# ashispati/ar-vae

Hardware: AMD Instinct MI355X
Metric: training images/sec (dSprites beta-VAE+AR, per-GPU batch 512) (higher is better)
Workload: dtype f32 (conv MFMAs: scaled 2-term fp16 split, 3 products, fp32-accurate)

## Files before the change

ar-vae_amd/csrc/conv32.hip:

```cpp
#include <mutex>
#include "diag.h"
#include "common.h"
#include "conv32_common.h"
#include "reduce.h"
#include "midprep.h"
#include "prep32.h"
#include "regloss.h"
#include "down32p.h"
#include "wgrad32r.h"

#include <type_traits>

namespace arvae {

template <int LO, int STRIDE, int PX = 128>
struct PatchLoader {
    using T = Tile<LO, PX>;
    static constexpr int SZ = STRIDE * LO;
    static constexpr int PR = STRIDE * T::TR + 2, PC = STRIDE * T::TC + 2;
    static constexpr int SLOTS = T::TI * PR * PC * 8;
    static constexpr int ITERS = (SLOTS + 255) / 256;
    float4 r[ITERS];
    unsigned rel[ITERS];
    __amdgpu_buffer_rsrc_t rs_v;
// ... 808 lines not shown
    reg_loss_block(reg, b % reg_bx, b / reg_bx, reg_lds, reg_lds + REG_CHUNK);
}


constexpr int WG32_SLAB = SLAB_C32_FLOATS;


template <int LO, int BIAS>
__device__ __forceinline__ void wgrad32x_body(const float *__restrict__ lo, const float *__restrict__ hi, float *__restrict__ slab, int n_img,
                                              int n_tiles, const unsigned *amax_lo, const unsigned *amax_hi, const int BID, const int NBLK) {
    constexpr int PX = 64, KB = PX / 16;
    using PL = PatchLoader<LO, 2, PX>;
    constexpr int WG_PSB_L = WGRAD_PSB_L, WG_PSB_H = WGRAD_PSB_H;
    constexpr int PC = PL::PC, PR = PL::PR, PLANE = PL::PLANE_DW / PSB * WG_PSB_H, LPLANE = PX * WG_PSB_L;
    extern __shared__ __attribute__((aligned(16))) float lds[];
    unsigned *ldsw = reinterpret_cast<unsigned *>(lds);
    unsigned *lo_w = ldsw + 2 * PLANE;
    const int lane = threadIdx.x & 63, wave = __builtin_amdgcn_readfirstlane(threadIdx.x >> 6);
    const int half = lane >> 5, rc = lane & 31;

    int loff[KB][2], hoff[KB][2];
    {
        const int g16 = lane >> 4, q = (lane & 15) >> 2, pp = lane & 3;
#pragma unroll
        for (int b = 0; b < KB; ++b)
#pragma unroll
            for (int i = 0; i < 2; ++i) {
                const int P = 16 * b + 8 * (g16 >> 1) + 4 * i + q;
                int img, r, c;
                tile_pixel<LO, PX>(P, img, r, c);
                loff[b][i] = P * WG_PSB_L + 8 * (g16 & 1) + 2 * pp;
                hoff[b][i] = ((img * PR + 2 * r + wave) * PC + 2 * c) * WG_PSB_H + 8 * (g16 & 1) + 2 * pp;
            }
    }

    f32x16 acc[4];
#pragma unroll
    for (int kx = 0; kx < 4; ++kx)
#pragma unroll
        for (int i = 0; i < 16; ++i) acc[kx][i] = 0.f;
    float4 bias4 = make_float4(0.f, 0.f, 0.f, 0.f);

    const AmaxLoad al_l = amax_issue(amax_lo), al_h = amax_issue(amax_hi);
    PL pl;
    pl.init(hi, n_img);
    const int64_t lo_bytes = (int64_t)n_img * LO * LO * PIXB;
    const __amdgpu_buffer_rsrc_t rs_lo = make_rsrc(lo, lo_bytes);
    float4 lr[2];
    unsigned lo_base = 0;
    auto set_lo = [&](int i0, int rr0, bool ok) {
        lo_base = ok ? (unsigned)(((i0 * LO + rr0) * LO) * PIXB) + threadIdx.x * 16 : OOB;
    };
    int img0, r0;
    tile_origin<LO, PX>(BID, img0, r0);
    pl.set_tile(img0, r0, BID < n_tiles);
    set_lo(img0, r0, BID < n_tiles);
    pl.issue_all();
#pragma unroll
    for (int it = 0; it < 2; ++it) lr[it] = buf_load4(rs_lo, lo_base + it * 4096);
    const Pow2 sc_lo = amax_scale(al_l), sc_hi = amax_scale(al_h);

    for (int tile = BID; tile < n_tiles; tile += NBLK) {
        __syncthreads();
        pl.template commit_split2<BIAS == 2, WG_PSB_H>(ldsw, sc_hi.s, &bias4);
#pragma unroll
        for (int it = 0; it < 2; ++it) {
            const int idx = threadIdx.x + it * 256, pix = idx >> 3, q = idx & 7;
            uint2 hv, lv;
            split_pair_h2(lr[it].x, lr[it].y, sc_lo.s, hv.x, lv.x);
            split_pair_h2(lr[it].z, lr[it].w, sc_lo.s, hv.y, lv.y);
            *reinterpret_cast<uint2 *>(lo_w + pix * WG_PSB_L + q * 2) = hv;
            *reinterpret_cast<uint2 *>(lo_w + LPLANE + pix * WG_PSB_L + q * 2) = lv;
            if (BIAS == 1) { bias4.x += lr[it].x; bias4.y += lr[it].y; bias4.z += lr[it].z; bias4.w += lr[it].w; }
        }
        __syncthreads();
        {
            int ni, nr;
            tile_origin<LO, PX>(tile + NBLK, ni, nr);
            pl.set_tile(ni, nr, tile + NBLK < n_tiles);
            set_lo(ni, nr, tile + NBLK < n_tiles);
        }
        static_for<0, KB>([&](auto bc) __attribute__((always_inline)) {
            constexpr int b = decltype(bc)::value;
            f16x8 b2[2];
#pragma unroll
            for (int t = 0; t < 2; ++t) b2[t] = lds_tr_f16x8(lo_w + t * LPLANE + loff[b][0], lo_w + t * LPLANE + loff[b][1]);
            pl.template issue_step<KB, b>();
            if constexpr (b < 2) lr[b] = buf_load4(rs_lo, lo_base + b * 4096);
#pragma unroll
            for (int kx = 0; kx < 4; ++kx) {
                f16x8 a2[2];
#pragma unroll
                for (int t = 0; t < 2; ++t)
                    a2[t] = lds_tr_f16x8(ldsw + t * PLANE + hoff[b][0] + kx * WG_PSB_H, ldsw + t * PLANE + hoff[b][1] + kx * WG_PSB_H);
                MFMA_H(acc[kx], a2[1], b2[0]);
                MFMA_H(acc[kx], a2[0], b2[1]);
                MFMA_H(acc[kx], a2[0], b2[0]);
            }
        });
    }

    float *out = slab + (int64_t)BID * WG32_SLAB;
    const float inv = sc_lo.inv * sc_hi.inv;
#pragma unroll
    for (int kx = 0; kx < 4; ++kx)
#pragma unroll
        for (int g = 0; g < 4; ++g)
            *reinterpret_cast<float4 *>(out + ((wave * 4 + kx) * C32 + rc) * C32 + 8 * g + 4 * half) =
                make_float4(acc[kx][4 * g] * inv, acc[kx][4 * g + 1] * inv, acc[kx][4 * g + 2] * inv, acc[kx][4 * g + 3] * inv);
    if (BIAS != 0) {
        __syncthreads();
        *reinterpret_cast<float4 *>(lds + threadIdx.x * 4) = bias4;
        __syncthreads();
        if (threadIdx.x < C32) {
            const int q = threadIdx.x >> 2, e = threadIdx.x & 3;
            float tot = 0.f;
            for (int j = 0; j < 32; ++j) tot += lds[(j * 8 + q) * 4 + e];
            out[16 * C32 * C32 + threadIdx.x] = tot;
        }
    }
}
template <int LO, int BIAS>
__global__ __launch_bounds__(256, 1) void wgrad32x_kernel(const float *__restrict__ lo, const float *__restrict__ hi,
                                                          float *__restrict__ slab, int n_img, int n_tiles, const unsigned *amax_lo,
                                                          const unsigned *amax_hi) {
    wgrad32x_body<LO, BIAS>(lo, hi, slab, n_img, n_tiles, amax_lo, amax_hi, blockIdx.x, gridDim.x);
}

template <int MODE, int BIAS>
__global__ __launch_bounds__(256, 1) void pair4_down_kernel(const float *__restrict__ g_hi, Ep32 ep,
                                                           const float *__restrict__ w_lo, const float *__restrict__ w_hi,
                                                           float *__restrict__ slab, int n_img, int tiles_a, int tiles_b, int grid_a,
                                                           const unsigned *amax_lo, const unsigned *amax_hi) {
    if ((int)blockIdx.x < grid_a) down32s_body<4, MODE>(g_hi, ep, n_img, tiles_a, blockIdx.x, grid_a);
    else wgrad32x_body<4, BIAS>(w_lo, w_hi, slab, n_img, tiles_b, amax_lo, amax_hi, blockIdx.x - grid_a, gridDim.x - grid_a);
}
template <int MODE, int BIAS>
__global__ __launch_bounds__(256, 1) void pair4_up_kernel(const float *__restrict__ g_lo, Ep32 ep,
                                                         const float *__restrict__ w_lo, const float *__restrict__ w_hi,
                                                         float *__restrict__ slab, int n_img, int tiles_a, int tiles_b, int grid_a,
                                                         const unsigned *amax_lo, const unsigned *amax_hi) {
    if ((int)blockIdx.x < grid_a) up32x_body<4, MODE, 32>(g_lo, ep, n_img, tiles_a, blockIdx.x, grid_a);
    else wgrad32x_body<4, BIAS>(w_lo, w_hi, slab, n_img, tiles_b, amax_lo, amax_hi, blockIdx.x - grid_a, gridDim.x - grid_a);
}


template <int LO, int MODE, int BIAS>
__global__ __launch_bounds__(512) __attribute__((amdgpu_waves_per_eu(2, 2))) void pair_down_wgrad_kernel(
    const float *__restrict__ g_hi, Ep32 ep, int n_img, int tiles_a, int grid_a, const float *__restrict__ w_lo, const float *__restrict__ w_hi,
    float *__restrict__ slab, int total_steps, int steps_per_wg, const unsigned *amax_lo, const unsigned *amax_hi) {
    if ((int)blockIdx.x < grid_a) down32p_body<LO, MODE>(g_hi, ep, n_img, tiles_a, blockIdx.x, grid_a);
    else wgrad32r_body<LO, BIAS>(w_lo, w_hi, slab, n_img, total_steps, steps_per_wg, amax_lo, amax_hi, blockIdx.x - grid_a);
}
template <int MODE, int BIAS, bool C1W = false>
__global__ __launch_bounds__(512) __attribute__((amdgpu_waves_per_eu(2, 2))) void pair_up16_wgrad_kernel(
    const float *__restrict__ g_lo, Ep32 ep, int n_img, int tiles_a, int grid_a, const float *__restrict__ w_lo, const float *__restrict__ w_hi,
    float *__restrict__ slab, int total_steps, int steps_per_wg, const unsigned *amax_lo, const unsigned *amax_hi, C1Wgrad c1) {
    if ((int)blockIdx.x < grid_a) up32p_body<MODE, C1W>(g_lo, ep, n_img, tiles_a, blockIdx.x, grid_a, c1);
    else wgrad32r_body<16, BIAS>(w_lo, w_hi, slab, n_img, total_steps, steps_per_wg, amax_lo, amax_hi, blockIdx.x - grid_a);
}
template <int MODE, int BIAS>
__global__ __launch_bounds__(512) __attribute__((amdgpu_waves_per_eu(2, 2))) void pair_up8_wgrad_kernel(
    const float *__restrict__ g_lo, Ep32 ep, int n_img, int tiles_a, int grid_a, const float *__restrict__ w_lo, const float *__restrict__ w_hi,
    float *__restrict__ slab, int total_steps, int steps_per_wg, const unsigned *amax_lo, const unsigned *amax_hi) {
    if ((int)blockIdx.x < grid_a) {
        if (threadIdx.x >= 256) return;
        up32x_body<8, MODE, 32>(g_lo, ep, n_img, tiles_a, blockIdx.x, grid_a);
    } else wgrad32r_body<8, BIAS>(w_lo, w_hi, slab, n_img, total_steps, steps_per_wg, amax_lo, amax_hi, blockIdx.x - grid_a);
}

static int cu_count() { return device_cu_count(); }

template <int LO, int PX = 128> static constexpr int tiles_for(int n) {
    using T = Tile<LO, PX>;
    return T::TI == 1 ? n * (LO / T::TR) : (n + T::TI - 1) / T::TI;
}
static int grid_for_tiles(int tiles) {
    const int cap = cu_count() < AMAX_N / 4 ? cu_count() : AMAX_N / 4;
    return tiles < cap ? tiles : cap;
}

bool conv32_fits(const arvae_link_t *l) {
    return l->chi == 32 && l->clo == 32 && l->kh == 4 && l->kw == 4 && l->stride == 2 && l->pad == 1 &&
           l->hh == l->hw && l->lh == l->lw && (l->lh == 16 || l->lh == 8 || l->lh == 4) && l->hi_perm_c == 0 &&
           l->lo_perm_c == 0 && (int64_t)l->n * l->hh * l->hw * PIXB < (1ll << 31) - (1ll << 20);
}

template <class K> static void allow_lds(K kernel, int bytes) {
    (void)hipFuncSetAttribute((const void *)kernel, hipFuncAttributeMaxDynamicSharedMemorySize, bytes);
}

template <int A, int B> struct MaxOf { static constexpr int value = A > B ? A : B; };

constexpr int LDS_DOWN_S = (PatchLoader<4, 2, 32>::BUF2_DW + 4 * 16 * 64) * 4;
static int down_small_grid(int tiles) {
    int g = tiles < 2 * cu_count() ? tiles : 2 * cu_count();
    return g < AMAX_N ? g : AMAX_N;
}

template <int MODE> static void launch_down_small(const Operand &hi, const Ep32 &ep, int n, hipStream_t s) {
    const int tiles = tiles_for<4, 32>(n);
    static std::once_flag attr;
    std::call_once(attr, [&] { allow_lds(down32s_kernel<4, MODE>, LDS_DOWN_S); });
    ARVAE_LAUNCH((down32s_kernel<4, MODE>), dim3(down_small_grid(tiles)), dim3(256), LDS_DOWN_S, s, hi.v, ep, n, tiles);
}
template <int LO, int MODE, int PX>
static void launch_up_px(const Operand &lo, const Ep32 &ep, int n, hipStream_t s) {
    const int tiles = tiles_for<LO, PX>(n), grid = grid_for_tiles(tiles);
    if constexpr (LO == 16 && PX == 128 && MODE != EP_GATE_F) {
        constexpr int LDSP = (2 * 2 * PatchLoader<16, 1, 128>::PLANE_DW) * 4 + 4 * 4 * 4 * 64 * 16;
        static std::once_flag attrp;
        std::call_once(attrp, [&] { allow_lds(up32p_kernel<MODE>, LDSP); });
        ARVAE_LAUNCH((up32p_kernel<MODE>), dim3(grid), dim3(512), LDSP, s, lo.v, ep, n, tiles);
    } else {
        constexpr int LDSX = 2 * PatchLoader<LO, 1, PX>::PLANE_DW * 4;
        static std::once_flag attrx;
        std::call_once(attrx, [&] { allow_lds(up32x_kernel<LO, MODE, PX>, LDSX); });
        ARVAE_LAUNCH((up32x_kernel<LO, MODE, PX>), dim3(grid), dim3(256), LDSX, s, lo.v, ep, n, tiles);
    }
}
template <int LO, int MODE>
static void launch_up_v(const Operand &lo, const Ep32 &ep, int n, hipStream_t s) {
    if (LO == 4 && 2 * tiles_for<LO, 128>(n) <= cu_count()) launch_up_px<4, MODE, 32>(lo, ep, n, s);
    else if (LO == 8 && tiles_for<LO, 128>(n) <= cu_count()) launch_up_px<8, MODE, 32>(lo, ep, n, s);
    else launch_up_px<LO, MODE, 128>(lo, ep, n, s);
}

static int ep_mode(const Ep32 &ep, int relu) {
    return ep.gate_bits != nullptr ? EP_GATE_B : ep.gate != nullptr ? EP_GATE_F : relu ? EP_RELU : EP_PLAIN;
}

template <int LO, int MODE> static void launch_down_p(const float *hi, const Ep32 &ep, int n, hipStream_t s) {
    constexpr int LDS = DownK<LO>::LDS_DW * 4;
    static std::once_flag attr;
    std::call_once(attr, [&] { allow_lds(down32p_kernel<LO, MODE>, LDS); });
    const int tiles = n * DownK<LO>::TILES_PER_IMG;
    ARVAE_LAUNCH((down32p_kernel<LO, MODE>), dim3(grid_for_tiles(tiles)), dim3(512), LDS, s, hi, ep, n, tiles);
}
template <int LO> static void launch_down_p_mode(const float *hi, const Ep32 &ep, int mode, int n, hipStream_t s) {
    switch (mode) {
        case EP_GATE_B: launch_down_p<LO, EP_GATE_B>(hi, ep, n, s); break;
        case EP_GATE_F: launch_down_p<LO, EP_GATE_F>(hi, ep, n, s); break;
        case EP_RELU: launch_down_p<LO, EP_RELU>(hi, ep, n, s); break;
        default: launch_down_p<LO, EP_PLAIN>(hi, ep, n, s); break;
    }
}
static void conv32_down_ksplit(const arvae_link_t *l, const float *hi, const Ep32 &ep, int mode, hipStream_t s) {
    if (l->lh == 16) launch_down_p_mode<16>(hi, ep, mode, l->n, s);
    else launch_down_p_mode<8>(hi, ep, mode, l->n, s);
}

int conv32_down(const arvae_link_t *l, const Operand &hi, const float *bias, int relu, const float *gate, const uint16_t *gate_bits,
                uint16_t *bits_out, float *out, hipStream_t s, const float *wprep, const unsigned *amax_in, unsigned *amax_out) {
    ARVAE_REQUIRE(wprep != nullptr && amax_in != nullptr, "conv32_down: prepared weights and the input's maxima are needed");
    Ep32 ep{bias, gate, gate_bits, bits_out, out, reinterpret_cast<const uint4 *>(wprep), amax_in, amax_out};
    const int mode = ep_mode(ep, relu);
    if (l->lh != 4) {
        conv32_down_ksplit(l, hi.v, ep, mode, s);
        return check_launch(l->lh == 16 ? "down32_kernel<16>" : "down32_kernel<8>");
    }
    switch (mode) {
        case EP_GATE_B: launch_down_small<EP_GATE_B>(hi, ep, l->n, s); break;
        case EP_GATE_F: launch_down_small<EP_GATE_F>(hi, ep, l->n, s); break;
        case EP_RELU: launch_down_small<EP_RELU>(hi, ep, l->n, s); break;
        default: launch_down_small<EP_PLAIN>(hi, ep, l->n, s); break;
    }
    return check_launch("down32_kernel<4>");
}

template <int MODE>
__global__ __launch_bounds__(512) __attribute__((amdgpu_waves_per_eu(2, 2))) void chain_down_kernel(const float *__restrict__ hi, Ep32 ep_a, Ep32 ep_b,
                                                                                                    int n_img, int tiles_a, int tiles_b) {
    extern __shared__ __attribute__((aligned(16))) unsigned chain_lds[];
    constexpr int BODY_DW = MaxOf<DownK<16>::LDS_DW, DownK<8>::LDS_DW>::value;
    float *chain_max = reinterpret_cast<float *>(chain_lds + BODY_DW);
    down32p_body<16, MODE, 1>(hi, ep_a, n_img, tiles_a, blockIdx.x, gridDim.x, chain_max);
    __syncthreads();
    down32p_body<8, MODE, 2>(ep_a.out, ep_b, n_img, tiles_b, blockIdx.x, gridDim.x, chain_max);
}
static int chain_grid(const arvae_link_t *a, const arvae_link_t *b) {
    if (a->n != b->n || a->n < 1) return 0;
    const int tiles_a = a->n * DownK<16>::TILES_PER_IMG, tiles_b = b->n * DownK<8>::TILES_PER_IMG;
    const int grid = grid_for_tiles(tiles_a);
    const int run_a = (tiles_a + grid - 1) / grid, run_b = (tiles_b + grid - 1) / grid;
    return (run_a * DownK<8>::TILES_PER_IMG == run_b * DownK<16>::TILES_PER_IMG) ? grid : 0;
}
bool conv32_down_chain_fits(const arvae_link_t *a, const arvae_link_t *b) {
    static const bool off = diag_env("ARVAE_NO_DOWN_CHAIN") != nullptr;
    return !off && conv32_fits(a) && conv32_fits(b) && a->lh == 16 && b->lh == 8 && b->hh == a->lh && chain_grid(a, b) > 0;
}
int conv32_down_chain(const arvae_link_t *a, const arvae_link_t *b, const float *hi, const unsigned *amax_in, const float *bias_a,
                      uint16_t *bits_a, float *out_a, const float *wprep_a, unsigned *amax_a, const float *bias_b, uint16_t *bits_b,
                      float *out_b, const float *wprep_b, unsigned *amax_b, hipStream_t s) {
    ARVAE_REQUIRE(conv32_down_chain_fits(a, b), "conv32_down_chain: these two layers do not chain");
    ARVAE_REQUIRE(hi && amax_in && out_a && out_b && wprep_a && wprep_b, "conv32_down_chain: null pointer");
    Ep32 ep_a{bias_a, nullptr, nullptr, bits_a, out_a, reinterpret_cast<const uint4 *>(wprep_a), amax_in, amax_a};
    Ep32 ep_b{bias_b, nullptr, nullptr, bits_b, out_b, reinterpret_cast<const uint4 *>(wprep_b), nullptr, amax_b};
    constexpr int LDS = (MaxOf<DownK<16>::LDS_DW, DownK<8>::LDS_DW>::value + 4) * 4;
    static std::once_flag attr;
    std::call_once(attr, [&] { allow_lds(chain_down_kernel<EP_RELU>, LDS); });
    ARVAE_LAUNCH((chain_down_kernel<EP_RELU>), dim3(chain_grid(a, b)), dim3(512), LDS, s, hi, ep_a, ep_b, a->n, a->n * DownK<16>::TILES_PER_IMG,
                 b->n * DownK<8>::TILES_PER_IMG);
    return check_launch("chain(down32<16> + down32<8>)");
}

template <int LO> static int launch_up(const arvae_link_t *l, const Operand &lo, const Ep32 &ep, int relu, hipStream_t s) {
// ... 110 lines not shown
static int conv32_wgrad_stream(const arvae_link_t *l, const Operand &lo, const Operand &hi, float *slab, int bias_mode, const unsigned *amax_lo,
                               const unsigned *amax_hi, hipStream_t s) {
    return l->lh == 16 ? launch_stream<16>(l, lo.v, hi.v, slab, bias_mode, amax_lo, amax_hi, s)
                       : launch_stream<8>(l, lo.v, hi.v, slab, bias_mode, amax_lo, amax_hi, s);
}

int conv32_wgrad_groups(const arvae_link_t *l) {
    if (conv32_wgrad_stream_fits(l)) return conv32_wgrad_stream_groups(l);
    return grid_for_tiles(tiles_for<4, 64>(l->n));
}

int64_t conv32_wgrad_ws_floats(const arvae_link_t *l) {
    return (int64_t)conv32_wgrad_groups(l) * WG32_SLAB;
}

constexpr int LDS_WGRAD_X4 = 2 * (PatchLoader<4, 2, 64>::PLANE_DW / PSB * WGRAD_PSB_H + 64 * WGRAD_PSB_L) * 4;
static int launch_wgrad_x4(const arvae_link_t *l, const Operand &lo, const Operand &hi, float *slab, int bias_mode, int grid,
                           const unsigned *amax_lo, const unsigned *amax_hi, hipStream_t s) {
    const int tiles = tiles_for<4, 64>(l->n);
    static std::once_flag attr;
    std::call_once(attr, [&] {
        allow_lds(wgrad32x_kernel<4, 0>, LDS_WGRAD_X4);
        allow_lds(wgrad32x_kernel<4, 1>, LDS_WGRAD_X4);
        allow_lds(wgrad32x_kernel<4, 2>, LDS_WGRAD_X4);
    });
    if (bias_mode == 1)
        ARVAE_LAUNCH((wgrad32x_kernel<4, 1>), dim3(grid), dim3(256), LDS_WGRAD_X4, s, lo.v, hi.v, slab, l->n, tiles, amax_lo, amax_hi);
    else if (bias_mode == 2)
        ARVAE_LAUNCH((wgrad32x_kernel<4, 2>), dim3(grid), dim3(256), LDS_WGRAD_X4, s, lo.v, hi.v, slab, l->n, tiles, amax_lo, amax_hi);
    else
        ARVAE_LAUNCH((wgrad32x_kernel<4, 0>), dim3(grid), dim3(256), LDS_WGRAD_X4, s, lo.v, hi.v, slab, l->n, tiles, amax_lo, amax_hi);
    return check_launch("wgrad32_kernel<4>");
}

int conv32_wgrad_partial(const arvae_link_t *l, const Operand &lo, const Operand &hi, float *dwt, float *dbias, int bias_mode,
                         float *slab, hipStream_t s, SlabJob *job, const unsigned *amax_lo, const unsigned *amax_hi) {
    ARVAE_REQUIRE(amax_lo != nullptr && amax_hi != nullptr, "conv32_wgrad: the operands' maxima are needed");
    const int grid = conv32_wgrad_groups(l);
    const int rc = conv32_wgrad_stream_fits(l) ? conv32_wgrad_stream(l, lo, hi, slab, bias_mode, amax_lo, amax_hi, s)
                                               : launch_wgrad_x4(l, lo, hi, slab, bias_mode, grid, amax_lo, amax_hi, s);
    *job = SlabJob{slab, dwt, bias_mode ? dbias : nullptr, grid, SLAB_C32, bias_mode};
    return rc;
}

constexpr int PAIR_SPLIT_C1_PERCENT = 62;
constexpr int PAIR_SPLIT_PERCENT = 50;
bool conv32_pair_fits(const arvae_link_t *l, bool up, const float *gate, const uint16_t *gate_bits, int bias_mode) {
    static const bool off4 = diag_env("ARVAE_NO_PAIR4") != nullptr;
    static const bool off = diag_env("ARVAE_NO_PAIR32") != nullptr;
    if ((gate == nullptr && gate_bits == nullptr) || bias_mode != (up ? 2 : 1)) return false;
    if (l->lh == 4) {
        const int wg_tiles = tiles_for<4, 64>(l->n), dg_tiles = tiles_for<4, 32>(l->n);
        return !off4 && wg_tiles >= 8 && wg_tiles + (dg_tiles + 1) / 2 <= cu_count() && conv32_wgrad_groups(l) == wg_tiles;
    }
    if (off || gate_bits == nullptr || !conv32_wgrad_stream_fits(l)) return false;
    if (l->n * (l->lh * l->lh / 32) < 4 * cu_count()) return false;
    if (!up && l->lh == 8 && tiles_for<8, 128>(l->n) > cu_count()) return false;
    return true;
}

template <int LO> static int launch_pair_big(const arvae_link_t *l, bool up, const float *g, const float *x_in, const Ep32 &ep, float *slab,
                                             const unsigned *amax_g, const unsigned *amax_x, hipStream_t s, int *grid_b_out,
                                             const C1Wgrad *c1 = nullptr, int *grid_a_out = nullptr) {
    const int cus = cu_count() < AMAX_N / 4 ? cu_count() : AMAX_N / 4;
    int grid_a = cus * (c1 != nullptr ? PAIR_SPLIT_C1_PERCENT : PAIR_SPLIT_PERCENT) / 100;
    if (grid_a < 1) grid_a = 1;
    const int tiles_a = up ? l->n * DownK<LO>::TILES_PER_IMG : (LO == 16 ? tiles_for<16, 128>(l->n) : tiles_for<8, 32>(l->n));
    {
        const int run = (tiles_a + grid_a - 1) / grid_a;
        grid_a = (tiles_a + run - 1) / run;
    }
    if (grid_a_out != nullptr) *grid_a_out = grid_a;
    ARVAE_REQUIRE(c1 == nullptr || grid_a <= 256, "pair_up16_wgrad: %d workgroups of the Up half exceed the first layer's 256 weight-gradient slabs", grid_a);
    int total, spw, grid_b;
    stream_geometry(l, cus - grid_a, total, spw, grid_b);
    *grid_b_out = grid_b;
    constexpr int LDS_W = RowStream<LO>::LDS_DW * 4;
    const dim3 grid(grid_a + grid_b);
    if (up) {
        constexpr int LDS = MaxOf<LDS_W, DownK<LO>::LDS_DW * 4>::value;
        static std::once_flag attr;
        std::call_once(attr, [&] { allow_lds(pair_down_wgrad_kernel<LO, EP_GATE_B, 2>, LDS); });
        ARVAE_LAUNCH((pair_down_wgrad_kernel<LO, EP_GATE_B, 2>), grid, dim3(512), LDS, s, g, ep, l->n, tiles_a, grid_a, x_in, g, slab, total, spw,
                     amax_x, amax_g);
        return check_launch(LO == 16 ? "pair(down32<16> + wgrad32<16>)" : "pair(down32<8> + wgrad32<8>)");
    }
    if constexpr (LO == 16) {
        constexpr int LDS_U = (2 * 2 * PatchLoader<16, 1, 128>::PLANE_DW) * 4 + 4 * 4 * 4 * 64 * 16;
        constexpr int LDS = MaxOf<LDS_W, LDS_U>::value;
        static std::once_flag attr;
        if (c1 != nullptr) {
            constexpr int LDS_C = MaxOf<LDS_W, LDS_U + 4 * C1W_WAVE_DW * 4>::value;
            static std::once_flag attr_c;
            std::call_once(attr_c, [&] { allow_lds(pair_up16_wgrad_kernel<EP_GATE_B, 1, true>, LDS_C); });
            ARVAE_LAUNCH((pair_up16_wgrad_kernel<EP_GATE_B, 1, true>), grid, dim3(512), LDS_C, s, g, ep, l->n, tiles_a, grid_a, g, x_in,
                         slab, total, spw, amax_g, amax_x, *c1);
            return check_launch("pair(up32<16> + wgrad32<16> + wgrad_c1)");
        }
        std::call_once(attr, [&] { allow_lds(pair_up16_wgrad_kernel<EP_GATE_B, 1>, LDS); });
        ARVAE_LAUNCH((pair_up16_wgrad_kernel<EP_GATE_B, 1>), grid, dim3(512), LDS, s, g, ep, l->n, tiles_a, grid_a, g, x_in, slab,
                     total, spw, amax_g, amax_x, C1Wgrad{nullptr, nullptr});
        return check_launch("pair(up32<16> + wgrad32<16>)");
    } else {
        constexpr int LDS = MaxOf<LDS_W, 2 * PatchLoader<8, 1, 32>::PLANE_DW * 4>::value;
        static std::once_flag attr;
        std::call_once(attr, [&] { allow_lds(pair_up8_wgrad_kernel<EP_GATE_B, 1>, LDS); });
        ARVAE_LAUNCH((pair_up8_wgrad_kernel<EP_GATE_B, 1>), grid, dim3(512), LDS, s, g, ep, l->n, tiles_a, grid_a, g, x_in, slab, total,
                     spw, amax_g, amax_x);
        return check_launch("pair(up32<8> + wgrad32<8>)");
    }
}

bool conv32_pair_c1_fits(const arvae_link_t *l, bool up, const uint16_t *gate_bits) {
    return !up && l->lh == 16 && gate_bits != nullptr;
}
int conv32_pair(const arvae_link_t *l, bool up, const float *g, const float *x_in, const float *gate, const uint16_t *gate_bits,
                float *d_in, const float *wprep, float *dwt, float *dbias, float *slab, hipStream_t s, SlabJob *job,
                const unsigned *amax_g, const unsigned *amax_x, unsigned *amax_out, const float *c1_img, float *c1_slab, SlabJob *c1_job) {
    ARVAE_REQUIRE(wprep != nullptr && amax_g != nullptr && amax_x != nullptr, "conv32_pair: prepared weights and the operands' maxima are needed");
    Ep32 ep{nullptr, gate_bits ? nullptr : gate, gate_bits, nullptr, d_in, reinterpret_cast<const uint4 *>(wprep), amax_g, amax_out};
    if (l->lh != 4) {
        int grid_b = 0, grid_a = 0;
        C1Wgrad c1{c1_img, c1_slab};
        const bool fuse = c1_img != nullptr && c1_slab != nullptr && c1_job != nullptr && conv32_pair_c1_fits(l, up, gate_bits);
        ARVAE_REQUIRE(fuse || c1_img == nullptr, "conv32_pair: this layer cannot carry the first layer's weight gradient");
        const int rc = l->lh == 16 ? launch_pair_big<16>(l, up, g, x_in, ep, slab, amax_g, amax_x, s, &grid_b, fuse ? &c1 : nullptr, &grid_a)
                                   : launch_pair_big<8>(l, up, g, x_in, ep, slab, amax_g, amax_x, s, &grid_b);
        *job = SlabJob{slab, dwt, dbias, grid_b, SLAB_C32, up ? 2 : 1};
        if (fuse) *c1_job = SlabJob{c1_slab, nullptr, nullptr, grid_a, SLAB_C1, 1};
        return rc;
    }
    constexpr int LDS_U = 2 * PatchLoader<4, 1, 32>::PLANE_DW * 4;
    constexpr int LDS = MaxOf<LDS_WGRAD_X4, MaxOf<LDS_DOWN_S, LDS_U>::value>::value;
    const int wg_tiles = tiles_for<4, 64>(l->n), dg_tiles = tiles_for<4, 32>(l->n), grid_a = (dg_tiles + 1) / 2;
    static std::once_flag attr;
    std::call_once(attr, [&] {
        allow_lds(pair4_down_kernel<EP_GATE_F, 2>, LDS);
        allow_lds(pair4_down_kernel<EP_GATE_B, 2>, LDS);
        allow_lds(pair4_up_kernel<EP_GATE_F, 1>, LDS);
        allow_lds(pair4_up_kernel<EP_GATE_B, 1>, LDS);
    });
    const dim3 grid(grid_a + wg_tiles);
    if (up) {
        if (gate_bits) ARVAE_LAUNCH((pair4_down_kernel<EP_GATE_B, 2>), grid, dim3(256), LDS, s, g, ep, x_in, g, slab, l->n, dg_tiles, wg_tiles, grid_a, amax_x, amax_g);
        else ARVAE_LAUNCH((pair4_down_kernel<EP_GATE_F, 2>), grid, dim3(256), LDS, s, g, ep, x_in, g, slab, l->n, dg_tiles, wg_tiles, grid_a, amax_x, amax_g);
    } else {
        if (gate_bits) ARVAE_LAUNCH((pair4_up_kernel<EP_GATE_B, 1>), grid, dim3(256), LDS, s, g, ep, g, x_in, slab, l->n, dg_tiles, wg_tiles, grid_a, amax_g, amax_x);
        else ARVAE_LAUNCH((pair4_up_kernel<EP_GATE_F, 1>), grid, dim3(256), LDS, s, g, ep, g, x_in, slab, l->n, dg_tiles, wg_tiles, grid_a, amax_g, amax_x);
    }
    *job = SlabJob{slab, dwt, dbias, wg_tiles, SLAB_C32, up ? 2 : 1};
    return check_launch(up ? "pair4(down32 + wgrad32)" : "pair4(up32 + wgrad32)");
}

int conv32_wgrad(const arvae_link_t *l, const Operand &lo, const Operand &hi, float *dwt, float *dbias, int bias_mode,
                 float *slab, hipStream_t s, const unsigned *amax_lo, const unsigned *amax_hi) {
    SlabJob job;
    if (int rc = conv32_wgrad_partial(l, lo, hi, dwt, dbias, bias_mode, slab, s, &job, amax_lo, amax_hi)) return rc;
    return slab_reduce(job, s);
}

}

#ifdef ARVAE_STAMPS
extern "C" int arvae_debug_stamps(unsigned long long *out, int count) {
    return (int)hipMemcpyFromSymbol(out, HIP_SYMBOL(arvae::g_stamps), sizeof(unsigned long long) * count);
}
#endif
#ifdef D32K_STAMPS
extern "C" int arvae_debug_d32k_stamps(unsigned long long *out, int count) {
    return (int)hipMemcpyFromSymbol(out, HIP_SYMBOL(arvae::g_d32k_stamps), sizeof(unsigned long long) * count);
}
#endif
#ifdef WGR_STAMPS
extern "C" int arvae_debug_wgr_stamps(unsigned long long *out, int count) {
    return (int)hipMemcpyFromSymbol(out, HIP_SYMBOL(arvae::g_wgr_stamps), sizeof(unsigned long long) * count);
}
#endif
```

ar-vae_amd/csrc/conv_c1.hip:

```cpp
#include <mutex>
#include "diag.h"
#include "common.h"
#include "reduce.h"
#include "prep32.h"
#include "wgrad_c1s.h"
#include "vae_finish.h"

namespace arvae {

constexpr int PS1 = 36;

struct Ep1 {
    const float *bias;
    const float *gate;
    const uint16_t *gate_bits;
    uint16_t *bits_out;
    float *out;
    int relu;
    unsigned *amax_out = nullptr;
};

template <int GATE, int WAVES>
__device__ __forceinline__ void down_c1s_body(Operand img, const float *__restrict__ wt, Ep1 ep, int n_rows, const int BID,
                                              const int NBLK, float *stage) {
// ... 55 lines not shown
                bits |= (o[j] > 0.f ? 1u : 0u) << (4 * g + j);
            }
            const float4 ov = make_float4(o[0], o[1], o[2], o[3]);
            amax_run = fmaxf(amax_run, amax4(ov));
            *reinterpret_cast<float4 *>(tile + rc * PS1 + 8 * g + 4 * half) = ov;
        }
        if (ep.bits_out != nullptr) ep.bits_out[pix * 2 + half] = (uint16_t)bits;
        __builtin_amdgcn_fence(__ATOMIC_RELEASE, "wavefront");
        __builtin_amdgcn_wave_barrier();
        float4 *dst = reinterpret_cast<float4 *>(ep.out + (int64_t)row * LO1 * CC);
#pragma unroll
        for (int i = 0; i < 4; ++i)
            dst[64 * i + lane] = *reinterpret_cast<const float4 *>(tile + (8 * i + (lane >> 3)) * PS1 + 4 * (lane & 7));
        __builtin_amdgcn_fence(__ATOMIC_RELEASE, "wavefront");
        __builtin_amdgcn_wave_barrier();
        v[0] = vn[0]; v[1] = vn[1];
    }
    if (ep.amax_out != nullptr) {
        __shared__ float wmax[WAVES];
        amax_run = wave_max(amax_run);
        if (lane == 0) wmax[threadIdx.x >> 6] = amax_run;
        __syncthreads();
        if (threadIdx.x < 64) {
            float m = 0.f;
#pragma unroll
            for (int w = 0; w < WAVES; ++w) m = fmaxf(m, wmax[w]);
            amax_publish(ep.amax_out, BID, NBLK, m);
        }
    }
}
template <int GATE>
__global__ __launch_bounds__(256) void down_c1s_kernel(Operand img, const float *__restrict__ wt, Ep1 ep, int n_rows) {
    __shared__ __attribute__((aligned(16))) float stage[4 * LO1 * PS1];
    down_c1s_body<GATE, 4>(img, wt, ep, n_rows, blockIdx.x, gridDim.x, stage);
}

__global__ __launch_bounds__(256) void down_c1s_prep_kernel(Operand img, const float *__restrict__ wt, Ep1 ep, int n_rows, PrepArgs prep,
                                                             MidPrepArgs mid, int conv_blocks, int prep_blocks) {
    __shared__ __attribute__((aligned(16))) float stage[4 * LO1 * PS1];
    if ((int)blockIdx.x < prep_blocks) {
        prep_all_block(prep, mid, conv_blocks, blockIdx.x);
        return;
    }
    down_c1s_body<0, 4>(img, wt, ep, n_rows, blockIdx.x - prep_blocks, gridDim.x - prep_blocks, stage);
}


typedef int i32x4 __attribute__((ext_vector_type(4)));
constexpr int TRU = 16;
constexpr int UG_PER_WAVE = (TRU + 2) * 2 / 4;
constexpr int TS1 = 17;
constexpr int T_FLOATS = (TRU + 2) * LO1 * TS1;

template <int DIST, bool LOSS>
__global__ __launch_bounds__(256, 2) void up_c1_kernel(const float *__restrict__ lo, const float *__restrict__ wt,
                                                        const float *__restrict__ bias_p, float *__restrict__ out,
                                                        const float *__restrict__ x, float inv_b,
                                                        float *__restrict__ partial, float *__restrict__ dlogits, int n_img,
                                                        int n_tiles, VaeFinishArgs fin = VaeFinishArgs{},
                                                        VaeFinishArgs *__restrict__ fin_dst = nullptr) {
    extern __shared__ __attribute__((aligned(16))) float lds[];
    __shared__ float red[4];
    if (fin_dst != nullptr && blockIdx.x == 0) {
        if (threadIdx.x == 0) *fin_dst = fin;
        if (threadIdx.x < 8 && fin.scalars != nullptr) fin.scalars[threadIdx.x] = __builtin_nanf("");
    }
    const int lane = threadIdx.x & 63, wave = threadIdx.x >> 6, g = lane >> 4, li = lane & 15;
    float wreg[2][4];
#pragma unroll
    for (int s = 0; s < 2; ++s)
#pragma unroll
        for (int j = 0; j < 4; ++j) wreg[s][j] = wt[(16 * s + 4 * g + j) * 16 + li];
    const float bias = bias_p != nullptr ? bias_p[0] : 0.f;
    const __amdgpu_buffer_rsrc_t rs =
        __builtin_amdgcn_make_buffer_rsrc(const_cast<float *>(lo), 0, n_img * LO1 * LO1 * CC * 4, 0x00020000);
    auto load4 = [&](unsigned off) {
        const f32x4 v = __builtin_bit_cast(f32x4, __builtin_amdgcn_raw_buffer_load_b128(rs, (int)off, 0, 0));
        return v;
    };
    f32x4 v[UG_PER_WAVE][2];
    auto issue = [&](int tile, int i) {
        const int gidx = wave + 4 * i, prow = gidx >> 1, col0 = (gidx & 1) * 16;
        const int n = tile >> 1, gy = (tile & 1) * TRU - 1 + prow;
        const bool ok = tile < n_tiles && (unsigned)gy < (unsigned)LO1;
        const unsigned off = ok ? (unsigned)((((n * LO1 + gy) * LO1 + col0 + li) * CC + g * 4) * 4) : 0x7fffffffu;
        v[i][0] = load4(off);
        v[i][1] = load4(off + 64);
    };
#pragma unroll
    for (int i = 0; i < UG_PER_WAVE; ++i) issue(blockIdx.x, i);

    float loss = 0.f, corr = 0.f;
    int buf = 0;
    for (int tile = blockIdx.x; tile < n_tiles; tile += gridDim.x, buf ^= 1) {
        float *T = lds + buf * T_FLOATS;
        const int n = tile >> 1, r0 = (tile & 1) * TRU;
        float xv[8];
        if (LOSS) {
#pragma unroll
            for (int i = 0; i < 8; ++i)
                xv[i] = x[((int64_t)n * HI1 + 2 * r0 + (threadIdx.x >> 6) + 4 * i) * HI1 + (threadIdx.x & 63)];
        }
#pragma unroll
        for (int i = 0; i < UG_PER_WAVE; ++i) {
            f32x4 acc = {0.f, 0.f, 0.f, 0.f};
#pragma unroll
            for (int s = 0; s < 2; ++s)
#pragma unroll
                for (int j = 0; j < 4; ++j) acc = __builtin_amdgcn_mfma_f32_16x16x4f32(v[i][s][j], wreg[s][j], acc, 0, 0, 0);
            issue(tile + gridDim.x, i);
            const int gidx = wave + 4 * i, prow = gidx >> 1, col0 = (gidx & 1) * 16;
#pragma unroll
            for (int r = 0; r < 4; ++r) T[(prow * LO1 + col0 + 4 * g + r) * TS1 + li] = acc[r];
        }
        __syncthreads();
        const int hx = threadIdx.x & 63, px = hx & 1, xq = hx >> 1;
#pragma unroll
        for (int i = 0; i < 8; ++i) {
            const int hy = (threadIdx.x >> 6) + 4 * i, py = hy & 1, y = hy >> 1;
            float sum = bias;
#pragma unroll
            for (int ty = 0; ty < 2; ++ty)
#pragma unroll
                for (int tx = 0; tx < 2; ++tx) {
                    const int col = xq + px - tx;
                    const bool ok = (unsigned)col < (unsigned)LO1;
                    const int tap = (1 - py + 2 * ty) * 4 + 1 - px + 2 * tx;
                    const float t = T[((y + py - ty + 1) * LO1 + (ok ? col : 0)) * TS1 + tap];
                    sum += ok ? t : 0.f;
                }
            const int64_t o = ((int64_t)n * HI1 + 2 * r0 + hy) * HI1 + hx;
            out[o] = sum;
            if (LOSS) {
                float d;
                recon_elem<DIST>(sum, xv[i], inv_b, loss, corr, d);
                if (dlogits != nullptr) dlogits[o] = d;
            }
        }
    }
    if (LOSS) {
        const float tl = block_sum_256(loss, red);
        const float tc = block_sum_256(corr, red);
        if (threadIdx.x == 0) {
            partial[2 * blockIdx.x] = tl;
            partial[2 * blockIdx.x + 1] = tc;
        }
    }
}

__global__ __launch_bounds__(64 * WGS_WAVES) void wgrad_c1s_kernel(Operand lo, Operand img, float *__restrict__ slab, int n_rows) {
    __shared__ __attribute__((aligned(16))) float lo_s[WGS_WAVES * LO1 * WS1];
    __shared__ __attribute__((aligned(16))) float im_s[WGS_WAVES * 4 * IMS];
    wgrad_c1s_body(lo, img, slab, n_rows, blockIdx.x, gridDim.x, lo_s, im_s);
}

template <int GATE>
__global__ __launch_bounds__(64 * WGS_WAVES) void pair_c1_kernel(Operand d_img, const float *__restrict__ wt, Ep1 ep, int n_rows_d,
                                                                 Operand w_lo, Operand w_img, float *__restrict__ slab, int n_rows_w, int grid_a,
                                                                 int rider, const VaeFinishArgs *__restrict__ fin) {
    __shared__ __attribute__((aligned(16))) float raw[WGS_WAVES * LO1 * WS1 + WGS_WAVES * 4 * IMS];
    if (rider && blockIdx.x == 0) {
        static_assert(64 * WGS_WAVES == 512, "the finishing body is instantiated for this kernel's 512 threads");
        const VaeFinishArgs args = *fin;
        vae_finish_body<512>(args, reinterpret_cast<float4 *>(raw));
        return;
    }
    const int bid = (int)blockIdx.x - rider, nblk = (int)gridDim.x - rider;
    if (bid < grid_a) down_c1s_body<GATE, WGS_WAVES>(d_img, wt, ep, n_rows_d, bid, grid_a, raw);
    else wgrad_c1s_body(w_lo, w_img, slab, n_rows_w, bid - grid_a, nblk - grid_a, raw, raw + WGS_WAVES * LO1 * WS1);
}
static_assert(WGS_WAVES * LO1 * PS1 <= WGS_WAVES * LO1 * WS1, "pair_c1_kernel: the down body's row tiles fit the shared allocation");

static_assert(WGS_WAVES == 8, "the reduce step gives one of the 8 accumulator registers to each wave");

constexpr int W1_CH = 64, W1_SLOTS = 28;
constexpr int W1_PS = 80;
constexpr int W1_IMS = 32;
constexpr int W1_WAVES = 8;
constexpr int W1_LO_LOADS = (W1_SLOTS * W1_CH / 4 + 63) / 64;

__global__ __launch_bounds__(64 * W1_WAVES) void wgrad_c1w_kernel(Operand lo, Operand img, float *__restrict__ slab, int n_img, int lh,
                                                                 int lw, int hw) {
    __shared__ __attribute__((aligned(16))) float lo_s[W1_WAVES][W1_SLOTS * W1_PS];
    __shared__ float im_s[W1_WAVES][4 * W1_IMS];
    const int lane = threadIdx.x & 63, wave = threadIdx.x >> 6, g = lane >> 4, li = lane & 15;
    const int ky = li >> 2, kx = li & 3;
    float *lw_s = lo_s[wave], *iw = im_s[wave];
    for (int i = lane; i < W1_SLOTS * W1_PS; i += 64) lw_s[i] = 0.f;
    for (int i = lane; i < 4 * W1_IMS; i += 64) iw[i] = 0.f;
    f32x4 acc[4];
#pragma unroll
    for (int ct = 0; ct < 4; ++ct) acc[ct] = f32x4{0.f, 0.f, 0.f, 0.f};
    float lo_sum[4] = {0.f, 0.f, 0.f, 0.f}, img_sum = 0.f;
    const float gs = img.scale != nullptr ? img.scale[0] : 1.f;
    const int n_rows = n_img * lh, hh = lh + 3;
    const int wave0 = blockIdx.x * W1_WAVES + wave, n_waves = gridDim.x * W1_WAVES;
    const int row_f4 = lw * (W1_CH / 4);
    float4 lr[W1_LO_LOADS];
    float ir[2];
    auto issue = [&](int row) __attribute__((always_inline)) {
        const bool in = row < n_rows;
        const int n = row / lh, r = row - n * lh;
#pragma unroll
        for (int i = 0; i < W1_LO_LOADS; ++i) {
            const int e = 64 * i + lane;
            const bool ok = in && e < row_f4;
            const float4 v = lo.at4(ok ? (int64_t)row * lw * W1_CH + 4 * e : 0);
            lr[i] = ok ? v : make_float4(0.f, 0.f, 0.f, 0.f);
        }
#pragma unroll
        for (int i = 0; i < 2; ++i) {
            const int e = 64 * i + lane, pr = e / hw, px = e - pr * hw;
            const bool ok = in && pr < 4;
            const float v = img.at(ok ? ((int64_t)n * hh + r + pr) * hw + px : 0);
            ir[i] = ok ? gs * v : 0.f;
        }
    };
    issue(wave0);
    for (int row = wave0; row < n_rows; row += n_waves) {
        const int r = row % lh;
#pragma unroll
        for (int i = 0; i < W1_LO_LOADS; ++i) {
            const int e = 64 * i + lane;
            if (e < row_f4) *reinterpret_cast<float4 *>(lw_s + (e >> 4) * W1_PS + 4 * (e & 15)) = lr[i];
        }
#pragma unroll
        for (int i = 0; i < 2; ++i) {
            const int e = 64 * i + lane, pr = e / hw, px = e - pr * hw;
            if (pr < 4) {
                iw[pr * W1_IMS + px] = ir[i];
                if (pr == 0 || r == lh - 1) img_sum += ir[i];
            }
        }
        __builtin_amdgcn_fence(__ATOMIC_RELEASE, "wavefront");
        __builtin_amdgcn_wave_barrier();
        issue(row + n_waves);
#pragma unroll
        for (int q = 0; q < W1_SLOTS / 4; ++q) {
            const int c = 4 * q + g;
            const float b = iw[ky * W1_IMS + c + kx];
#pragma unroll
            for (int ct = 0; ct < 4; ++ct) {
                const float a = lw_s[c * W1_PS + 16 * ct + li];
                lo_sum[ct] += a;
                acc[ct] = __builtin_amdgcn_mfma_f32_16x16x4f32(a, b, acc[ct], 0, 0, 0);
            }
        }
        __builtin_amdgcn_fence(__ATOMIC_RELEASE, "wavefront");
        __builtin_amdgcn_wave_barrier();
    }
    float *red = &lo_s[0][0];
    __syncthreads();
#pragma unroll
    for (int ct = 0; ct < 4; ++ct)
#pragma unroll
        for (int r = 0; r < 4; ++r) red[(wave * 16 + ct * 4 + r) * 64 + lane] = acc[ct][r];
    __syncthreads();
    float *out = slab + (int64_t)blockIdx.x * SLAB_C1W_FLOATS;
#pragma unroll
    for (int e = 0; e < 2; ++e) {
        const int reg = 2 * wave + e, ct = reg >> 2, r = reg & 3;
        float tot = 0.f;
#pragma unroll
        for (int w = 0; w < W1_WAVES; ++w) tot += red[(w * 16 + reg) * 64 + lane];
        out[(16 * ct + 4 * g + r) * 16 + li] = tot;
    }
    __syncthreads();
    constexpr int T = 64 * W1_WAVES;
#pragma unroll
    for (int ct = 0; ct < 4; ++ct) red[ct * T + threadIdx.x] = lo_sum[ct];
    red[4 * T + threadIdx.x] = img_sum;
    __syncthreads();
    if (threadIdx.x < W1_CH) {
        const int ct = threadIdx.x >> 4, i = threadIdx.x & 15;
        float tot = 0.f;
        for (int j = 0; j < T / 16; ++j) tot += red[ct * T + j * 16 + i];
        out[W1_CH * 16 + threadIdx.x] = tot;
    } else if (threadIdx.x < 128) {
        float tot = 0.f;
        for (int j = lane; j < T; j += 64) tot += red[4 * T + j];
#pragma unroll
        for (int o = 32; o > 0; o >>= 1) tot += __shfl_xor(tot, o);
        if (lane == 0) out[W1_CH * 16 + W1_CH] = tot;
    }
}
static_assert(W1_WAVES == 8 && W1_WAVES * W1_SLOTS * W1_PS >= W1_WAVES * 16 * 64, "wgrad_c1w_kernel: the row buffers hold the reduce tiles");

bool conv_c1_fits(const arvae_link_t *l) {
    return l->chi == 1 && l->clo == CC && l->kh == 4 && l->kw == 4 && l->stride == 2 && l->pad == 1 && l->hh == HI1 &&
           l->hw == HI1 && l->lh == LO1 && l->lw == LO1 && l->hi_perm_c == 0 && l->lo_perm_c == 0;
}

int conv_c1_down_with_prep(const arvae_link_t *l, const Operand &img, const float *wt, const float *bias, int relu, uint16_t *bits_out,
                           float *out, const float *const *prep_wts, float *const *preps, int n_prep, const MidPrepArgs &mid,
                           hipStream_t s, unsigned *amax_out) {
    ARVAE_REQUIRE(n_prep > 0 && n_prep <= PREP_MAX_LAYERS && mid.count > 0, "conv_c1_down_with_prep: nothing to prepare");
    Ep1 ep{bias, nullptr, nullptr, bits_out, out, relu, amax_out};
    PrepArgs p{};
    for (int i = 0; i < n_prep; ++i) {
        p.wt[i] = prep_wts[i];
        p.out[i] = reinterpret_cast<uint4 *>(preps[i]);
    }
    const int conv_blocks = 16 * n_prep, prep_blocks = conv_blocks + mid_prep_blocks(mid);
    const int n_rows = l->n * LO1;
    int grid = 256 * 16 / 4;
    if (grid > (n_rows + 3) / 4) grid = (n_rows + 3) / 4;
    if (grid > AMAX_N) grid = AMAX_N;
    ARVAE_LAUNCH(down_c1s_prep_kernel, dim3(prep_blocks + grid), dim3(256), 0, s, img, wt, ep, n_rows, p, mid, conv_blocks, prep_blocks);
    return check_launch("down_c1_kernel(+ weight prep)");
}

int conv_c1_down(const arvae_link_t *l, const Operand &img, const float *wt, const float *bias, int relu,
                 const float *gate, const uint16_t *gate_bits, uint16_t *bits_out, float *out, hipStream_t s, unsigned *amax_out) {
    Ep1 ep{bias, gate, gate_bits, bits_out, out, relu, amax_out};
    const int n_rows = l->n * LO1;
    int grid = 256 * 16 / 4;
    if (grid > (n_rows + 3) / 4) grid = (n_rows + 3) / 4;
    if (amax_out != nullptr && grid > AMAX_N) grid = AMAX_N;
    if (gate_bits != nullptr) ARVAE_LAUNCH(down_c1s_kernel<1>, dim3(grid), dim3(256), 0, s, img, wt, ep, n_rows);
    else if (gate != nullptr) ARVAE_LAUNCH(down_c1s_kernel<2>, dim3(grid), dim3(256), 0, s, img, wt, ep, n_rows);
    else ARVAE_LAUNCH(down_c1s_kernel<0>, dim3(grid), dim3(256), 0, s, img, wt, ep, n_rows);
    return check_launch("down_c1_kernel");
}

static int up_c1_grid(int tiles) {
    int dev = 0, cus = 256;
    hipDeviceProp_t prop;
    static int cached = 0;
    if (cached == 0) {
        if (hipGetDevice(&dev) == hipSuccess && hipGetDeviceProperties(&prop, dev) == hipSuccess) cus = prop.multiProcessorCount;
        cached = cus > 0 ? cus : 256;
    }
    return tiles < 2 * cached ? tiles : 2 * cached;
}

template <class K> static void up_c1_lds(K kernel) {
    (void)hipFuncSetAttribute((const void *)kernel, hipFuncAttributeMaxDynamicSharedMemorySize, 2 * T_FLOATS * 4);
}

int conv_c1_up(const arvae_link_t *l, const float *lo, const float *wt, const float *bias, float *out, hipStream_t s) {
    const int tiles = l->n * (LO1 / TRU);
    static std::once_flag attr;
    std::call_once(attr, [&] { up_c1_lds(up_c1_kernel<ARVAE_RECON_BERNOULLI, false>); });
    ARVAE_LAUNCH((up_c1_kernel<ARVAE_RECON_BERNOULLI, false>), dim3(up_c1_grid(tiles)), dim3(256), 2 * T_FLOATS * 4, s, lo,
                       wt, bias, out, nullptr, 0.f, nullptr, nullptr, l->n, tiles);
    return check_launch("up_c1_kernel");
}

int conv_c1_up_recon_blocks(const arvae_link_t *l) { return up_c1_grid(l->n * (LO1 / TRU)); }

int conv_c1_up_recon(const arvae_link_t *l, const float *lo, const float *wt, const float *bias, float *out, const float *x,
                     int dist, float *partial, float *dlogits, hipStream_t s, int *nb_out, const VaeFinishArgs *fin, VaeFinishArgs *fin_dst) {
    const int tiles = l->n * (LO1 / TRU), grid = up_c1_grid(tiles);
    const float inv_b = 1.f / (float)l->n;
    const VaeFinishArgs fa = fin != nullptr ? *fin : VaeFinishArgs{};
    if (fin == nullptr) fin_dst = nullptr;
    static std::once_flag attr;
    std::call_once(attr, [&] {
        up_c1_lds(up_c1_kernel<ARVAE_RECON_BERNOULLI, true>);
        up_c1_lds(up_c1_kernel<ARVAE_RECON_GAUSSIAN, true>);
    });
    if (dist == ARVAE_RECON_BERNOULLI)
        ARVAE_LAUNCH((up_c1_kernel<ARVAE_RECON_BERNOULLI, true>), dim3(grid), dim3(256), 2 * T_FLOATS * 4, s, lo, wt, bias,
                           out, x, inv_b, partial, dlogits, l->n, tiles, fa, fin_dst);
    else
        ARVAE_LAUNCH((up_c1_kernel<ARVAE_RECON_GAUSSIAN, true>), dim3(grid), dim3(256), 2 * T_FLOATS * 4, s, lo, wt, bias,
                           out, x, inv_b, partial, dlogits, l->n, tiles, fa, fin_dst);
    *nb_out = grid;
    return check_launch("up_c1_kernel(recon)");
}

int wgrad_c1_groups(const arvae_link_t *l) {
    constexpr int cap = 256;
    const int units = (l->n * LO1 + WGS_WAVES - 1) / WGS_WAVES;
    return units < cap ? units : cap;
}

int64_t conv_c1_wgrad_ws_floats(const arvae_link_t *l) { return (int64_t)wgrad_c1_groups(l) * WG1_SLAB; }

int conv_c1_wgrad_partial(const arvae_link_t *l, const Operand &lo, const Operand &img, float *dwt, float *dbias,
                          int bias_mode, float *slab, hipStream_t s, SlabJob *job) {
    const int grid = wgrad_c1_groups(l);
    ARVAE_LAUNCH(wgrad_c1s_kernel, dim3(grid), dim3(64 * WGS_WAVES), 0, s, lo, img, slab, l->n * LO1);
    *job = SlabJob{slab, dwt, dbias, grid, SLAB_C1, bias_mode};
    return check_launch("wgrad_c1_kernel");
}

__global__ __launch_bounds__(512) void vae_finish_deferred_kernel(const VaeFinishArgs *__restrict__ fin) {
    __shared__ float4 red4[8];
    const VaeFinishArgs args = *fin;
    vae_finish_body<512>(args, red4);
}
int vae_finish_deferred(const VaeFinishArgs *fin_dev, hipStream_t s) {
    ARVAE_LAUNCH(vae_finish_deferred_kernel, dim3(1), dim3(512), 0, s, fin_dev);
    return check_launch("image_vae_backward(finish)");
}

bool conv_c1_pair_fits(const arvae_link_t *l) {
    static const bool off = diag_env("ARVAE_NO_PAIR_C1") != nullptr;
    return !off && conv_c1_fits(l) && l->n * LO1 >= 8 * 256 && wgrad_c1_groups(l) == 256;
}
int conv_c1_pair(const arvae_link_t *l, const Operand &g_img, const float *wt, const float *gate, const uint16_t *gate_bits, float *d_lo,
                 const Operand &w_lo, float *dwt, float *dbias, int bias_mode, float *slab, hipStream_t s, SlabJob *job,
                 unsigned *amax_out, const VaeFinishArgs *finish) {
    Ep1 ep{nullptr, gate, gate_bits, nullptr, d_lo, 0, amax_out};
    const int rider = finish != nullptr ? 1 : 0;
    const int n_rows = l->n * LO1, grid_a = 256, grid_b = wgrad_c1_groups(l) - rider;
    const dim3 grid(rider + grid_a + grid_b);
    if (gate_bits != nullptr) ARVAE_LAUNCH(pair_c1_kernel<1>, grid, dim3(64 * WGS_WAVES), 0, s, g_img, wt, ep, n_rows, w_lo, g_img, slab, n_rows, grid_a, rider, finish);
    else if (gate != nullptr) ARVAE_LAUNCH(pair_c1_kernel<2>, grid, dim3(64 * WGS_WAVES), 0, s, g_img, wt, ep, n_rows, w_lo, g_img, slab, n_rows, grid_a, rider, finish);
    else ARVAE_LAUNCH(pair_c1_kernel<0>, grid, dim3(64 * WGS_WAVES), 0, s, g_img, wt, ep, n_rows, w_lo, g_img, slab, n_rows, grid_a, rider, finish);
    *job = SlabJob{slab, dwt, dbias, grid_b, SLAB_C1, bias_mode};
    return check_launch("pair_c1(down_c1 + wgrad_c1)");
}

int conv_c1_wgrad(const arvae_link_t *l, const Operand &lo, const Operand &img, float *dwt, float *dbias, int bias_mode,
                  float *slab, hipStream_t s) {
    SlabJob job;
    if (int rc = conv_c1_wgrad_partial(l, lo, img, dwt, dbias, bias_mode, slab, s, &job)) return rc;
    return slab_reduce(job, s);
}

bool conv_c1w_fits(const arvae_link_t *l) {
    return l->chi == 1 && l->clo == W1_CH && l->kh == 4 && l->kw == 4 && l->stride == 1 && l->pad == 0 && l->lw <= W1_SLOTS &&
           l->hw == l->lw + 3 && l->hh == l->lh + 3 && l->hw < W1_IMS && 4 * l->hw <= 128 && l->hi_perm_c == 0 && l->lo_perm_c == 0;
}
static int wgrad_c1w_groups(const arvae_link_t *l) {
    const int units = (l->n * l->lh + W1_WAVES - 1) / W1_WAVES;
    return units < 256 ? units : 256;
}
int64_t conv_c1w_wgrad_ws_floats(const arvae_link_t *l) { return (int64_t)wgrad_c1w_groups(l) * SLAB_C1W_FLOATS; }

int conv_c1w_wgrad(const arvae_link_t *l, const Operand &lo, const Operand &img, float *dwt, float *dbias, int bias_mode,
                   float *slab, hipStream_t s) {
    const int grid = wgrad_c1w_groups(l);
    ARVAE_LAUNCH(wgrad_c1w_kernel, dim3(grid), dim3(64 * W1_WAVES), 0, s, lo, img, slab, l->n, l->lh, l->lw, l->hw);
    if (int rc = check_launch("wgrad_c1w_kernel")) return rc;
    return slab_reduce(SlabJob{slab, dwt, dbias, grid, SLAB_C1W, bias_mode}, s);
}

}
```

ar-vae_amd/csrc/down32p.h:

```cpp
#pragma once
#include "common.h"
#include "conv32_common.h"

namespace arvae {

#ifdef D32K_STAMPS
__device__ unsigned long long g_d32k_stamps[64 * 64];
#define DSTAMP(role, slot) do { if (LO == 16 && threadIdx.x == 256 * (role) && BID < 32 && (slot) < 64) g_d32k_stamps[(BID + 32 * (role)) * 64 + (slot)] = wall_clock64(); } while (0)
#else
#define DSTAMP(role, slot)
#endif

template <int LO> struct DownK {
    using T = Tile<LO, 64>;
    static constexpr int HW = 2 * LO;
    static constexpr int PR = 2 * T::TR + 2;
    static constexpr int PIX = PR * HW;
    static constexpr int BUF = (PIX + 1) * PSB2;
    static constexpr int SLOTS = (PIX * 8 + 255) / 256;
    static constexpr int XCH = 4 * 3 * 2 * 64 * 4;
    static constexpr int LDS_DW = 2 * BUF + XCH;
    static constexpr int TILES_PER_IMG = LO / T::TR;
};

template <int LO, int MODE, int CHAIN = 0>
__device__ __forceinline__ void down32p_body(const float *__restrict__ hi, Ep32 ep, int n_img, int n_tiles, const int BID, const int NBLK,
                                             float *chain_max = nullptr) {
    using K = DownK<LO>;
    constexpr int HW = K::HW, PIX = K::PIX, SLOTS = K::SLOTS, HI = 2 * LO;
    extern __shared__ __attribute__((aligned(16))) unsigned ldsd[];
    unsigned *xch = ldsd + 2 * K::BUF;
    const int lane = threadIdx.x & 63, wave = __builtin_amdgcn_readfirstlane(threadIdx.x >> 6);
    const int per_wg = (n_tiles + NBLK - 1) / NBLK, t_first = BID * per_wg;
    const int t_end = min(n_tiles, t_first + per_wg);
    using S0 = std::integral_constant<int, 0>;
    using S1 = std::integral_constant<int, 1>;
    auto chain_scale = [&]() __attribute__((always_inline)) -> Pow2 {
        const float m = fmaxf(fmaxf(chain_max[0], chain_max[1]), fmaxf(chain_max[2], chain_max[3]));
        return pow2_for((unsigned)__builtin_amdgcn_readfirstlane(__builtin_bit_cast(int, m)));
    };

    if (wave >= 4) {
        DSTAMP(1, 0);
        int pst = 0;
        (void)pst;
        const int pt = threadIdx.x - 256;
        const __amdgpu_buffer_rsrc_t rs_hi = make_rsrc(hi, (int64_t)n_img * HI * HI * PIXB);
        int q = pt & 7, pix0 = pt >> 3;
        float4 lv[2][SLOTS];
        float sc_in = 1.f;
        AmaxLoad al{};
        if constexpr (CHAIN != 2) al = amax_issue(ep.amax_in);
        auto issue = [&](auto set_, int s, int tile) __attribute__((always_inline)) {
            constexpr int set = decltype(set_)::value;
            int img0, r0;
            tile_origin<LO, 64>(tile, img0, r0);
            const int pix = pix0 + 32 * s, pr = pix / HW, px = pix - pr * HW;
            const int gy = 2 * r0 - 1 + pr;
            const bool ok = tile < t_end && pix < PIX && (unsigned)gy < (unsigned)HI;
            lv[set][s] = buf_load4(rs_hi, ok ? (unsigned)((((img0 * HI + gy) * HI + px) * C32 + 4 * q) * 4) : OOB);
        };
        auto commit = [&](auto set_, int s, unsigned *buf) __attribute__((always_inline)) {
            constexpr int set = decltype(set_)::value;
            const int pix = pix0 + 32 * s;
            if (SLOTS * 32 > PIX && pix >= PIX) return;
            uint2 hv, lw;
            split_pair_h2(lv[set][s].x, lv[set][s].y, sc_in, hv.x, lw.x);
            split_pair_h2(lv[set][s].z, lv[set][s].w, sc_in, hv.y, lw.y);
            unsigned *d = buf + pix * PSB2 + q * 2;
            *reinterpret_cast<uint2 *>(d) = hv;
            *reinterpret_cast<uint2 *>(d + 16) = lw;
        };
#pragma unroll
        for (int s = 0; s < SLOTS; ++s) issue(S0{}, s, t_first);
#pragma unroll
        for (int s = 0; s < SLOTS; ++s) issue(S1{}, s, t_first + 1);
        if (pt < 2 * PSB2) ldsd[(pt / PSB2) * K::BUF + PIX * PSB2 + pt % PSB2] = 0u;
        if constexpr (CHAIN != 2) sc_in = amax_scale(al).s;
        else sc_in = chain_scale().s;
        __syncthreads();
#pragma unroll
        for (int s = 0; s < SLOTS; ++s) commit(S0{}, s, ldsd);
#pragma unroll
        for (int s = 0; s < SLOTS; ++s) issue(S0{}, s, t_first + 2);
        __syncthreads();
        const unsigned rel0 = (unsigned)(pix0 * PIXB + q * 16);
        unsigned first_row = 0, last_row = 0, no_slot = 0;
#pragma unroll
        for (int s = 0; s < SLOTS; ++s) {
            const int pix = pix0 + 32 * s, pr = pix / HW;
            if (pr == 0) first_row |= 1u << s;
            if (pr == PIX / HW - 1) last_row |= 1u << s;
            if (pix >= PIX) no_slot |= 1u << s;
        }
        auto do_tile = [&](auto set_, int tile, int cur) __attribute__((always_inline)) {
            constexpr int set = decltype(set_)::value;
            asm volatile("" : "+v"(q), "+v"(pix0));
            DSTAMP(1, 4 + 5 * pst);
            unsigned *nb = ldsd + (cur ^ 1) * K::BUF;
            unsigned n_base, n_bad;
            {
                const int nt = tile + 3;
                int ni, nr;
                tile_origin<LO, 64>(nt, ni, nr);
                const int gy0 = 2 * nr - 1;
                n_base = nt < t_end ? (unsigned)(((ni * HI + gy0) * HI) * PIXB) + rel0 : OOB;
                n_bad = (gy0 < 0 ? first_row : 0u) | (gy0 + PIX / HW - 1 >= HI ? last_row : 0u) | no_slot;
            }
#pragma unroll
            for (int s = 0; s < SLOTS; ++s) {
                commit(set_, s, nb);
                lv[set][s] = buf_load4(rs_hi, (n_bad & (1u << s)) != 0 ? OOB : n_base + 4096u * s);
            }
            DSTAMP(1, 5 + 5 * pst);
            __syncthreads();
            DSTAMP(1, 6 + 5 * pst);
            __syncthreads();
            DSTAMP(1, 7 + 5 * pst);
            ++pst;
        };
        for (int tile = t_first; tile < t_end; tile += 2) {
            do_tile(S1{}, tile, 0);
            do_tile(S0{}, tile + 1, 1);
        }
        return;
    }

    DSTAMP(0, 0);
    int cst = 0;
    (void)cst;
    const int half = lane >> 5, rc = lane & 31;
    AmaxLoad al{};
    if constexpr (CHAIN != 2) al = amax_issue(ep.amax_in);
    int xoff[2][4];
#pragma unroll
    for (int mt = 0; mt < 2; ++mt) {
        int img, r, c;
        tile_pixel<LO, 64>(mt * 32 + rc, img, r, c);
#pragma unroll
        for (int kx = 0; kx < 4; ++kx) {
            const int col = 2 * c - 1 + kx;
            xoff[mt][kx] = ((unsigned)col < (unsigned)HW ? (2 * r + wave) * HW + col : PIX) * PSB2 + half * 4;
        }
    }
    const int om = wave & 1, og = wave >> 1;
    float4 b4[2];
#pragma unroll
    for (int e = 0; e < 2; ++e)
        b4[e] = ep.bias != nullptr ? *reinterpret_cast<const float4 *>(ep.bias + 8 * (2 * og + e) + 4 * half) : make_float4(0.f, 0.f, 0.f, 0.f);
    const int64_t out_bytes = (int64_t)n_img * LO * LO * PIXB;
    const __amdgpu_buffer_rsrc_t rs_out = make_rsrc(ep.out, out_bytes);
    const __amdgpu_buffer_rsrc_t rs_gate = make_rsrc(MODE == EP_GATE_F ? ep.gate : ep.out, out_bytes);
    const bool want_bits = MODE == EP_RELU && ep.bits_out != nullptr;
    const __amdgpu_buffer_rsrc_t rs_bits =
        make_rsrc(MODE == EP_GATE_B ? (const void *)ep.gate_bits : want_bits ? (const void *)ep.bits_out : (const void *)ep.out,
                  (int64_t)n_img * LO * LO * 4);
    const unsigned out_lane = (unsigned)((om * 32 + rc) * PIXB + (2 * og) * 32 + half * 16);
    f16x8 w2[8][2];
    {
        const uint4 *wp = ep.wprep + ((wave >> 1) * PREP_DOWN_SLOTS + ((wave & 1) * 4) * 2 * 2) * 64 + lane;
#pragma unroll
        for (int st = 0; st < 8; ++st)
#pragma unroll
            for (int t = 0; t < 2; ++t) w2[st][t] = __builtin_bit_cast(f16x8, wp[(st * 2 + t) * 64]);
    }
    float inv;
    if constexpr (CHAIN != 2) inv = amax_scale(al).inv * prep_inv_scale(ep.wprep);
    else inv = chain_scale().inv * prep_inv_scale(ep.wprep);
    float amax_run = 0.f;
    __syncthreads();
    __syncthreads();
    DSTAMP(0, 1);

    float4 own[2] = {make_float4(0.f, 0.f, 0.f, 0.f), make_float4(0.f, 0.f, 0.f, 0.f)};
    float4 gq_prev[2] = {own[0], own[0]};
    unsigned obase_prev = OOB, gb_prev = 0;
    const float4 *xq_own = reinterpret_cast<const float4 *>(xch) + (wave * 3) * 2 * 64 + lane;
    unsigned bits_acc = 0;
    float4 part[2][3];
    auto load_parts = [&]() __attribute__((always_inline)) {
#pragma unroll
        for (int e = 0; e < 2; ++e)
#pragma unroll
            for (int k = 0; k < 3; ++k) part[e][k] = xq_own[(k * 2 + e) * 64];
    };
    auto epi_item = [&](auto ic) __attribute__((always_inline)) {
        constexpr int i = decltype(ic)::value;
        if constexpr (i < 8) {
            constexpr int e = i / 4, k = i % 4;
            if constexpr (k < 3) {
                const float4 p = part[e][k];
                own[e].x += p.x; own[e].y += p.y; own[e].z += p.z; own[e].w += p.w;
            } else {
                float o4[4] = {fmaf(own[e].x, inv, b4[e].x), fmaf(own[e].y, inv, b4[e].y), fmaf(own[e].z, inv, b4[e].z), fmaf(own[e].w, inv, b4[e].w)};
                const float gf[4] = {gq_prev[e].x, gq_prev[e].y, gq_prev[e].z, gq_prev[e].w};
#pragma unroll
                for (int j = 0; j < 4; ++j) {
                    if (MODE == EP_RELU) {
                        o4[j] = fmaxf(o4[j], 0.f);
                        bits_acc |= (o4[j] > 0.f ? 1u : 0u) << (4 * e + j);
                    }
                    if (MODE == EP_GATE_F) o4[j] = gf[j] > 0.f ? o4[j] : 0.f;
                    if (MODE == EP_GATE_B) o4[j] = ((gb_prev >> (8 * og + 4 * e + j)) & 1u) ? o4[j] : 0.f;
                }
                const float4 ov = make_float4(o4[0], o4[1], o4[2], o4[3]);
                amax_run = obase_prev != OOB ? fmaxf(amax_run, amax4(ov)) : amax_run;
                buf_store4(ov, rs_out, obase_prev + e * 32);
            }
        } else if constexpr (i == 8) {
            if (MODE == EP_RELU)
                __builtin_amdgcn_raw_buffer_store_b8((unsigned char)bits_acc, rs_bits,
                                                     (int)((obase_prev == OOB || !want_bits) ? OOB : bits_off(obase_prev, half) + og), 0, 0);
            bits_acc = 0;
        }
    };
    auto do_tile = [&](int tile, int cur) __attribute__((always_inline)) {
        DSTAMP(0, 4 + 5 * cst);
        const unsigned *xb = ldsd + cur * K::BUF;
        f32x16 acc[2], accb[2];
#pragma unroll
        for (int mt = 0; mt < 2; ++mt)
#pragma unroll
            for (int i = 0; i < 16; ++i) { acc[mt][i] = 0.f; accb[mt][i] = 0.f; }
        f16x8 x2[2][2][2];
#pragma unroll
        for (int mt = 0; mt < 2; ++mt)
#pragma unroll
            for (int t = 0; t < 2; ++t)
                x2[0][mt][t] = __builtin_bit_cast(f16x8, *reinterpret_cast<const i32x4v *>(xb + xoff[mt][0] + t * 16));
        load_parts();
        int img0, r0;
        tile_origin<LO, 64>(tile, img0, r0);
        const unsigned obase = tile < t_end ? (unsigned)(((img0 * LO + r0) * LO) * PIXB) + out_lane : OOB;
        float4 gq[2];
        unsigned gb = 0;
        if (MODE == EP_GATE_F) {
            gq[0] = buf_load4(rs_gate, obase);
            gq[1] = buf_load4(rs_gate, obase + 32);
        }
        if (MODE == EP_GATE_B) gb = buf_load_u16(rs_bits, bits_off(obase, half));
        static_for<0, 8>([&](auto kc) __attribute__((always_inline)) {
            constexpr int step = decltype(kc)::value, cu = step & 1, nx = cu ^ 1;
            constexpr int e_lo = step >= 1 ? 2 * (step - 1) : 0, e_hi = step >= 1 ? (2 * step < 9 ? 2 * step : 9) : 0;
            constexpr int n_epi = e_hi > e_lo ? e_hi - e_lo : 0, n_items = 4 + n_epi;
            auto item = [&](auto ic) __attribute__((always_inline)) {
                constexpr int i = decltype(ic)::value;
                if constexpr (i < 4) {
                    if constexpr (step + 1 < 8) {
                        constexpr int nkx = (step + 1) >> 1, nc = (step + 1) & 1, mt = i / 2, t = i % 2;
                        x2[nx][mt][t] = __builtin_bit_cast(f16x8, *reinterpret_cast<const i32x4v *>(xb + xoff[mt][nkx] + t * 16 + nc * 8));
                    }
                } else {
                    epi_item(std::integral_constant<int, e_lo + (i - 4)>{});
                }
            };
            __builtin_amdgcn_sched_barrier(0);
            static_for<0, 6>([&](auto mc) __attribute__((always_inline)) {
                constexpr int m = decltype(mc)::value, prod = m >> 1, mt = m & 1;
                constexpr int tw = prod == 0 ? 1 : 0;
                constexpr int tx = prod == 1 ? 1 : 0;
                if constexpr ((prod == 1) == ((step & 1) == 0)) MFMA_H(accb[mt], w2[step][tw], x2[cu][mt][tx]);
                else MFMA_H(acc[mt], w2[step][tw], x2[cu][mt][tx]);
                __builtin_amdgcn_sched_barrier(0);
                static_for<m * n_items / 6, (m + 1) * n_items / 6>(item);
                __builtin_amdgcn_sched_barrier(0);
            });
        });
#pragma unroll
        for (int mt = 0; mt < 2; ++mt)
#pragma unroll
            for (int i = 0; i < 16; ++i) acc[mt][i] += accb[mt][i];
        DSTAMP(0, 5 + 5 * cst);
        __syncthreads();
        DSTAMP(0, 6 + 5 * cst);
        float4 *xq = reinterpret_cast<float4 *>(xch);
        auto piece = [&](auto m_, auto g_, int e) __attribute__((always_inline)) -> float4 {
            constexpr int M = decltype(m_)::value, G = decltype(g_)::value;
            return e == 0 ? make_float4(acc[M][8 * G], acc[M][8 * G + 1], acc[M][8 * G + 2], acc[M][8 * G + 3])
                          : make_float4(acc[M][8 * G + 4], acc[M][8 * G + 5], acc[M][8 * G + 6], acc[M][8 * G + 7]);
        };
        static_for<0, 4>([&](auto oc) __attribute__((always_inline)) {
            constexpr int ow = decltype(oc)::value;
            if (ow != wave) {
                const int src = (wave - ow - 1) & 3;
#pragma unroll
                for (int e = 0; e < 2; ++e)
                    xq[((ow * 3 + src) * 2 + e) * 64 + lane] = piece(std::integral_constant<int, (ow & 1)>{}, std::integral_constant<int, (ow >> 1)>{}, e);
            }
        });
#pragma unroll
        for (int e = 0; e < 2; ++e)
            own[e] = wave == 0 ? piece(std::integral_constant<int, 0>{}, std::integral_constant<int, 0>{}, e)
                   : wave == 1 ? piece(std::integral_constant<int, 1>{}, std::integral_constant<int, 0>{}, e)
                   : wave == 2 ? piece(std::integral_constant<int, 0>{}, std::integral_constant<int, 1>{}, e)
                               : piece(std::integral_constant<int, 1>{}, std::integral_constant<int, 1>{}, e);
        obase_prev = obase;
        gb_prev = gb;
        if (MODE == EP_GATE_F) { gq_prev[0] = gq[0]; gq_prev[1] = gq[1]; }
        __syncthreads();
        DSTAMP(0, 7 + 5 * cst);
        DSTAMP(0, 8 + 5 * cst);
        ++cst;
    };
    for (int tile = t_first; tile < t_end; tile += 2) {
        do_tile(tile, 0);
        do_tile(tile + 1, 1);
    }
    load_parts();
    static_for<0, 9>(epi_item);
    amax_publish(ep.amax_out, BID * 4 + wave, NBLK * 4, amax_run);
    if constexpr (CHAIN == 1) {
        const float m = wave_max(amax_run);
        if (lane == 0) chain_max[wave] = m;
    }
}
template <int LO, int MODE>
__global__ __launch_bounds__(512) __attribute__((amdgpu_waves_per_eu(2, 2))) void down32p_kernel(const float *__restrict__ hi, Ep32 ep,
                                                                                                 int n_img, int n_tiles) {
    down32p_body<LO, MODE>(hi, ep, n_img, n_tiles, blockIdx.x, gridDim.x);
}
// ... 3 lines not shown
```

ar-vae_amd/csrc/plan.hip:

```cpp
#include "diag.h"
#include "common.h"
#include "dense.h"
#include "reduce.h"
#include "midprep.h"
#include "regloss.h"
#include "vae_finish.h"
#include "conv32_common.h"

namespace arvae {

bool conv32_fits(const arvae_link_t *l);
bool conv_c1_fits(const arvae_link_t *l);
bool conv64_fits(const arvae_link_t *l, bool up);
bool conv64s_fits(const arvae_link_t *l, bool up);
int64_t conv64s_ws_floats();
int conv64s_prep_batch(const float *const *wts, float *const *outs, const int *transposed, const int *q, int count, hipStream_t s);
bool conv64_wgrad_fits(const arvae_link_t *l);
int link_wgrad_conv64(const arvae_link_t *link, const Operand &lo, const Operand &hi, float *dwt, float *dbias, int bias_side, float *ws,
                      hipStream_t st, const unsigned *amax_lo, const unsigned *amax_hi);
bool single_channel_down_gated_fits(const arvae_link_t *l);
int single_channel_down_gated(const arvae_link_t *link, const Operand &hi, const float *wt, const GateOp *gate, float *lo, hipStream_t s,
                              unsigned *amax_out);
bool single_channel_down_fits(const arvae_link_t *l);
int single_channel_down(const arvae_link_t *link, const Operand &hi, const float *wt, const float *bias, int act, const uint8_t *mask,
                        float *lo, hipStream_t s, unsigned *amax_out);
int conv64_down(const arvae_link_t *l, const Operand &hi, const float *wt, const float *bias, int act, const uint8_t *mask,
                float *lo, float *ws, hipStream_t s, const GateOp *gate, const unsigned *amax_in = nullptr, unsigned *amax_out = nullptr,
                float *prepped = nullptr);
int conv64_up(const arvae_link_t *l, const Operand &lo, const float *wt, const float *bias, int act, const uint8_t *mask,
              float *hi, float *ws, hipStream_t s, const GateOp *gate, const unsigned *amax_in = nullptr, unsigned *amax_out = nullptr,
              float *prepped = nullptr);
int conv32_down(const arvae_link_t *l, const Operand &hi, const float *bias, int relu, const float *gate, const uint16_t *gate_bits,
                uint16_t *bits_out, float *out, hipStream_t s, const float *wprep, const unsigned *amax_in, unsigned *amax_out);
int conv32_up(const arvae_link_t *l, const Operand &lo, const float *bias, int relu, const float *gate, const uint16_t *gate_bits,
              uint16_t *bits_out, float *out, hipStream_t s, const float *wprep, const unsigned *amax_in, unsigned *amax_out);
int conv32_amax(const float *x, int64_t count, unsigned *out, hipStream_t s);
int conv_c1_up_recon(const arvae_link_t *l, const float *lo, const float *wt, const float *bias, float *out, const float *x,
                     int dist, float *partial, float *dlogits, hipStream_t s, int *nb_out, const VaeFinishArgs *fin = nullptr,
                     VaeFinishArgs *fin_dst = nullptr);
int vae_finish_deferred(const VaeFinishArgs *fin_dev, hipStream_t s);
VaeFinishArgs vae_finish_args(const float *rec_partial, int nb, int64_t batch, int64_t pix, const float *mu, const float *sigma,
                              int64_t zdim, float beta, const float *cap, const float *reg_ws, int64_t n_cols, int64_t ldz,
                              const int32_t *dims, int32_t r, float gamma, float delta, float reg_scale, float *dz, float *rec_out,
                              float *kld_out, float *reg_out, float *scalars, int64_t rec_rows);
bool conv32_up_reg_fits(const arvae_link_t *l);
bool conv32_down_chain_fits(const arvae_link_t *a, const arvae_link_t *b);
int conv32_down_chain(const arvae_link_t *a, const arvae_link_t *b, const float *hi, const unsigned *amax_in, const float *bias_a,
                      uint16_t *bits_a, float *out_a, const float *wprep_a, unsigned *amax_a, const float *bias_b, uint16_t *bits_b,
                      float *out_b, const float *wprep_b, unsigned *amax_b, hipStream_t s);
int conv32_up_reg(const arvae_link_t *l, const Operand &lo, const float *bias, uint16_t *bits_out, float *out, const float *wprep,
                  const unsigned *amax_in, unsigned *amax_out, const RegArgs &reg, int r, hipStream_t s);
int conv_c1_up_recon_blocks(const arvae_link_t *l);
int recon_partial_blocks(int64_t count);
int64_t conv32_prep_floats();
int conv32_weight_prep(const float *const *wts, float *const *preps, int n_layers, hipStream_t s);
int conv32_weight_prep_with_mid(const float *const *wts, float *const *preps, int n_layers, const MidPrepArgs &mid, hipStream_t s);
void mid_prep_args(const arvae_image_vae_t *m, const float *params, float *prep_ws, MidPrepArgs *out, int batch);
bool conv32_pair_fits(const arvae_link_t *l, bool up, const float *gate, const uint16_t *gate_bits, int bias_mode);
int conv32_pair(const arvae_link_t *l, bool up, const float *g, const float *x_in, const float *gate, const uint16_t *gate_bits,
                 float *d_in, const float *wprep, float *dwt, float *dbias, float *slab, hipStream_t s, SlabJob *job,
                 const unsigned *amax_g, const unsigned *amax_x, unsigned *amax_out, const float *c1_img, float *c1_slab, SlabJob *c1_job);
bool conv32_pair_c1_fits(const arvae_link_t *l, bool up, const uint16_t *gate_bits);
int conv32_wgrad_partial(const arvae_link_t *l, const Operand &lo, const Operand &hi, float *dwt, float *dbias, int bias_mode,
                         float *slab, hipStream_t s, SlabJob *job, const unsigned *amax_lo, const unsigned *amax_hi);
bool conv_c1_pair_fits(const arvae_link_t *l);
int conv_c1_pair(const arvae_link_t *l, const Operand &g_img, const float *wt, const float *gate, const uint16_t *gate_bits, float *d_lo,
                 const Operand &w_lo, float *dwt, float *dbias, int bias_mode, float *slab, hipStream_t s, SlabJob *job,
                 unsigned *amax_out, const VaeFinishArgs *finish = nullptr);
int conv_c1_wgrad_partial(const arvae_link_t *l, const Operand &lo, const Operand &img, float *dwt, float *dbias,
                          int bias_mode, float *slab, hipStream_t s, SlabJob *job);
bool dense_wgrad_c1_fits(const DenseWgradBatch *b);
int dense_wgrad_flush_with_c1(DenseWgradBatch *b, const arvae_link_t *l, const Operand &lo, const Operand &img, float *dwt, float *dbias,
                              int bias_mode, float *slab, hipStream_t s, SlabJob *job);
int conv_c1_down(const arvae_link_t *l, const Operand &img, const float *wt, const float *bias, int relu,
                 const float *gate, const uint16_t *gate_bits, uint16_t *bits_out, float *out, hipStream_t s, unsigned *amax_out);
int conv_c1_down_with_prep(const arvae_link_t *l, const Operand &img, const float *wt, const float *bias, int relu, uint16_t *bits_out,
                           float *out, const float *const *prep_wts, float *const *preps, int n_prep, const MidPrepArgs &mid,
                           hipStream_t s, unsigned *amax_out);

bool heads_fusable(const arvae_layer_t *hm, const arvae_layer_t *hl, int zdim);
int heads_latent_fwd(const arvae_layer_t *hm, const arvae_layer_t *hl, int batch, int zdim, const float *params,
                     const float *hidden, const float *eps, float *mu, float *log_std, float *sigma, float *z, hipStream_t s,
                     const arvae_image_vae_t *rng_model = nullptr, const arvae_layer_t *next = nullptr, float *next_out = nullptr);
bool heads_next_fusable(const arvae_layer_t *l, int zdim);
int heads_latent_bwd(const arvae_layer_t *hm, const arvae_layer_t *hl, int batch, int zdim, const float *params,
                     const float *g_z, const float *dz_reg, const float *dz_extra, const float *mu, const float *sigma,
                     const float *eps, const float *g_loss, const float *kl, const float *cap, float beta, float reg_scale,
                     const float *gate, float *d_mu, float *d_ls, float *d_hidden, hipStream_t s, const arvae_layer_t *next = nullptr,
                     const float *next_g = nullptr);

bool mid_fusable(const arvae_image_vae_t *m, int *ne_out, int *nd_out);
int64_t mid_prep_floats(const arvae_image_vae_t *m);
int mid_forward(const arvae_image_vae_t *m, int batch, const float *params, float *prep_ws, const float *x0, float *const *enc_y,
                float *const *dec_y, const float *eps, float *mu, float *log_std, float *sigma, float *z, hipStream_t s, bool prep_done,
                unsigned *amax_out, const MidFold *fold, float *wide_ws);
int64_t mid_wide_ws_floats(const arvae_image_vae_t *m, int batch);
int mid_wide_wgrad(const arvae_image_vae_t *m, int batch, const float *params, float *prep_ws, float *wide_ws, const float *x0,
                   const float *g_last_pre, float *grads, hipStream_t s, int *took);
bool mid_fold_fits(const arvae_image_vae_t *m, int batch);
int64_t mid_fold_slab_floats(const arvae_image_vae_t *m, int batch);
int mid_backward(const arvae_image_vae_t *m, int batch, const float *params, float *prep_ws, float *const *enc_y, float *const *dec_y,
                 float *const *enc_g, float *const *dec_g, const float *g_out, int g_is_pre, const float *gate0, float *d_x0,
                 const float *eps, const float *mu, const float *sigma, const float *dz_reg, const float *dz_extra, const float *g_loss,
                 const float *kl, const float *cap, float beta, float reg_scale, float *d_mu, float *d_ls, hipStream_t s,
                 unsigned *amax_out, const MidFold *fold, float *wide_ws);

int recon_partials(const float *logits, const float *x, int64_t count, int64_t batch, int32_t dist, float *ws,
                   float *dlogits, hipStream_t s, int *nb_out);
int reg_partials(const float *z_rows, const float *lab_rows, int64_t n_rows, const float *z_cols, const float *lab_cols,
                 int64_t n_cols, int64_t ldz, int64_t ldl, const RegDims &rd, int32_t r, float delta, float *ws,
                 hipStream_t s, const VaeFinishArgs *park = nullptr, VaeFinishArgs *park_dst = nullptr);
int vae_finish(const float *rec_partial, int nb, int64_t batch, int64_t pix, const float *mu, const float *sigma,
               int64_t zdim, float beta, const float *cap, const float *reg_ws, int64_t n_cols, int64_t ldz,
               const int32_t *dims, int32_t r, float gamma, float delta, float reg_scale, float *dz, float *rec_out,
               float *kld_out, float *reg_out, float *scalars, hipStream_t s, int64_t rec_rows = 0);

__global__ __launch_bounds__(256) void latent_bwd_full_kernel(const float *__restrict__ g_z, const float *__restrict__ dz_reg,
                                                               const float *__restrict__ dz_extra, const float *__restrict__ mu,
                                                               const float *__restrict__ sigma, const float *__restrict__ eps,
                                                               const float *__restrict__ g_loss, const float *__restrict__ kl,
                                                               const float *__restrict__ cap, float beta, float inv_batch,
                                                               float reg_scale, int64_t count, float *__restrict__ d_mu,
                                                               float *__restrict__ d_ls) {
    const float g = g_loss[0];
    const float diff = kl[0] - (cap != nullptr ? cap[0] : 0.f);
    const float k = g * beta * (diff > 0.f ? 1.f : (diff < 0.f ? -1.f : 0.f)) * inv_batch;
    for (int64_t i = (int64_t)blockIdx.x * 256 + threadIdx.x; i < count; i += (int64_t)gridDim.x * 256) {
        float gz = g_z[i];
        if (dz_reg != nullptr) gz += g * reg_scale * dz_reg[i];
        if (dz_extra != nullptr) gz += dz_extra[i];
        const float s = sigma[i];
        d_mu[i] = gz + k * mu[i];
        d_ls[i] = (gz * eps[i] + k * (s - 1.f / s)) * s;
    }
}

__global__ __launch_bounds__(256) void add_inplace_kernel(float *__restrict__ a, const float *__restrict__ b,
                                                           const float *__restrict__ gate, int64_t count) {
    for (int64_t i = (int64_t)blockIdx.x * 256 + threadIdx.x; i < count; i += (int64_t)gridDim.x * 256) {
        const float v = a[i] + b[i];
        a[i] = (gate == nullptr || gate[i] > 0.f) ? v : 0.f;
    }
}

static inline int64_t up4(int64_t v) { return (v + 3) / 4 * 4; }

static inline int64_t out_elems(const arvae_layer_t &l, int64_t n) {
    return l.is_up ? n * l.link.hh * l.link.hw * l.link.chi : n * l.link.lh * l.link.lw * l.link.clo;
}
static inline int64_t in_elems(const arvae_layer_t &l, int64_t n) {
    return l.is_up ? n * l.link.lh * l.link.lw * l.link.clo : n * l.link.hh * l.link.hw * l.link.chi;
}

struct Layout {
    int64_t enc_out[ARVAE_MAX_LAYERS], dec_out[ARVAE_MAX_LAYERS];
    int64_t enc_keep[ARVAE_MAX_LAYERS], dec_keep[ARVAE_MAX_LAYERS];
    int64_t enc_slab[ARVAE_MAX_LAYERS], dec_slab[ARVAE_MAX_LAYERS];
    int64_t enc_bits[ARVAE_MAX_LAYERS], dec_bits[ARVAE_MAX_LAYERS];
    int64_t enc_wprep[ARVAE_MAX_LAYERS], dec_wprep[ARVAE_MAX_LAYERS];
    int64_t enc_wide[ARVAE_MAX_LAYERS][2], dec_wide[ARVAE_MAX_LAYERS][2];
    int64_t enc_amax[ARVAE_MAX_LAYERS], dec_amax[ARVAE_MAX_LAYERS], enc_gamax[ARVAE_MAX_LAYERS], dec_gamax[ARVAE_MAX_LAYERS];
    int64_t ga_amax, gb_amax, tmp_amax, tmp2_amax;
    int64_t log_std, dlogits, dz_reg, d_mu, d_ls, g_a, g_b, slab, link_ws, mid_prep, mid_wide, fin_args, rec_ws, reg_ws, rec_out, kld_out, reg_out, total;
    int64_t slab_floats;
};

static int make_layout(const arvae_image_vae_t *m, int64_t n, int64_t n_cols, Layout &L) {
    ARVAE_REQUIRE(m != nullptr && n > 0, "image_vae: null model or empty batch");
    ARVAE_REQUIRE(m->n_enc >= 1 && m->n_enc <= ARVAE_MAX_LAYERS && m->n_dec >= 1 && m->n_dec <= ARVAE_MAX_LAYERS,
                  "image_vae: layer counts out of range");
    ARVAE_REQUIRE(m->zdim > 0 && m->n_reg >= 0 && m->n_reg <= 16, "image_vae: bad zdim / n_reg");
    int64_t off = 0, gmax = 0, slab = 0, lws = 0;
    auto take = [&](int64_t count) { const int64_t o = off; off += up4(count); return o; };
    auto visit = [&](const arvae_layer_t &l) {
        arvae_link_t lk = l.link;
        lk.n = (int32_t)n;
        const int64_t s = arvae_link_wgrad_ws_floats(&lk);
        if (s > slab) slab = s;
        if (arvae_link_ws_floats(&lk) > lws) lws = arvae_link_ws_floats(&lk);
        if (out_elems(l, n) > gmax) gmax = out_elems(l, n);
        if (in_elems(l, n) > gmax) gmax = in_elems(l, n);
    };
    auto wide = [&](const arvae_layer_t &l, int64_t (&slot)[2]) {
        arvae_link_t lk = l.link;
        lk.n = (int32_t)n;
        const bool other = dense_fits(&lk) || conv32_fits(&lk) || conv_c1_fits(&lk);
        for (int t = 0; t < 2; ++t) slot[t] = (!other && conv64_fits(&lk, t == 1) && conv64s_fits(&lk, t == 1)) ? take(conv64s_ws_floats()) : -1;
    };
    for (int i = 0; i < ARVAE_MAX_LAYERS; ++i) L.enc_wide[i][0] = L.enc_wide[i][1] = L.dec_wide[i][0] = L.dec_wide[i][1] = -1;
    for (int i = 0; i < m->n_enc; ++i) wide(m->enc[i], L.enc_wide[i]);
    for (int i = 0; i < m->n_dec; ++i) wide(m->dec[i], L.dec_wide[i]);
    for (int i = 0; i < m->n_enc; ++i) { L.enc_out[i] = take(out_elems(m->enc[i], n)); visit(m->enc[i]); }
    for (int i = 0; i < m->n_dec; ++i) {
        L.dec_out[i] = (i + 1 < m->n_dec) ? take(out_elems(m->dec[i], n)) : -1;
        visit(m->dec[i]);
    }
    visit(m->head_mu);
    visit(m->head_log_std);
    const int64_t fold_slab = mid_fold_slab_floats(m, (int)n);
    auto own_slab = [&](const arvae_layer_t &l) -> int64_t {
        arvae_link_t lk = l.link;
        lk.n = (int32_t)n;
        if (!(conv32_fits(&lk) || conv_c1_fits(&lk))) return -1;
        const int64_t need = arvae_link_wgrad_ws_floats(&lk);
        return take((conv32_fits(&lk) && lk.lh == 4 && fold_slab > need) ? fold_slab : need);
    };
    auto own_bits = [&](const arvae_layer_t &l, int64_t wprep) -> int64_t {
        arvae_link_t lk = l.link;
        lk.n = (int32_t)n;
        const bool fast = (conv32_fits(&lk) && wprep >= 0) || (conv_c1_fits(&lk) && !l.is_up);
        return (fast && l.act == ARVAE_ACT_RELU && !l.dropout) ? take(out_elems(l, n) / 32) : -1;
    };
    int n_prep = 0;
    auto own_prep = [&](const arvae_layer_t &l) -> int64_t {
        arvae_link_t lk = l.link;
        lk.n = (int32_t)n;
        return (conv32_fits(&lk) && n_prep++ < 8) ? take(conv32_prep_floats()) : -1;
    };
    for (int i = 0; i < m->n_enc; ++i) L.enc_wprep[i] = own_prep(m->enc[i]);
    for (int i = 0; i < m->n_dec; ++i) L.dec_wprep[i] = own_prep(m->dec[i]);
    for (int i = 0; i < m->n_enc; ++i) L.enc_bits[i] = own_bits(m->enc[i], L.enc_wprep[i]);
    for (int i = 0; i < m->n_dec; ++i) L.dec_bits[i] = own_bits(m->dec[i], L.dec_wprep[i]);
    for (int i = 0; i < m->n_enc; ++i) L.enc_slab[i] = own_slab(m->enc[i]);
    for (int i = 0; i < m->n_dec; ++i) L.dec_slab[i] = own_slab(m->dec[i]);
    for (int i = 0; i < m->n_enc; ++i) L.enc_keep[i] = take(out_elems(m->enc[i], n));
    for (int i = 0; i < m->n_dec; ++i) L.dec_keep[i] = take(out_elems(m->dec[i], n));
    for (int i = 0; i < m->n_enc; ++i) { L.enc_amax[i] = take(AMAX_N); L.enc_gamax[i] = take(AMAX_N); }
    for (int i = 0; i < m->n_dec; ++i) { L.dec_amax[i] = take(AMAX_N); L.dec_gamax[i] = take(AMAX_N); }
    L.ga_amax = take(AMAX_N);
    L.gb_amax = take(AMAX_N);
    L.tmp_amax = take(AMAX_N);
    L.tmp2_amax = take(AMAX_N);
    const int64_t bz = n * m->zdim;
    L.log_std = take(bz);
    L.dlogits = take(out_elems(m->dec[m->n_dec - 1], n));
    L.dz_reg = take(bz);
    L.d_mu = take(bz);
    L.d_ls = take(bz);
    L.g_a = take(gmax);
    L.g_b = take(gmax);
    L.slab_floats = slab;
    L.slab = take(slab);
    L.link_ws = take(lws);
    L.mid_prep = take(mid_prep_floats(m));
    {
        const int64_t w = mid_wide_ws_floats(m, (int)n);
        L.mid_wide = w > 0 ? take(w) : -1;
    }
    static_assert(sizeof(VaeFinishArgs) <= 64 * sizeof(float), "the parked finishing step's arguments fit their workspace slot");
    L.fin_args = take(64);
    L.rec_ws = take(arvae_recon_ws_floats(out_elems(m->dec[m->n_dec - 1], n)));
    L.reg_ws = take(arvae_reg_loss_ws_floats(n, m->n_reg > 0 ? m->n_reg : 1));
    L.rec_out = take(4);
    L.kld_out = take(4);
    L.reg_out = take(4);
    L.total = off;
    (void)n_cols;
    return ARVAE_OK;
}

static inline void mark(void *event, hipStream_t st) {
    if (event != nullptr) (void)hipEventRecord(reinterpret_cast<hipEvent_t>(event), st);
}

static bool recon_is_fused(const arvae_image_vae_t *m) {
    const arvae_layer_t &last = m->dec[m->n_dec - 1];
    return last.is_up && last.act == ARVAE_ACT_NONE && last.dropout == 0 && conv_c1_fits(&last.link) && arvae_recon_ws_floats(0) >= 2 * 1024;
}
static bool finish_deferred(const arvae_image_vae_t *m) { return (m->flags & ARVAE_VAE_DEFER_FINISH) != 0 && recon_is_fused(m); }

static arvae_operand_t plain(const float *v) { return arvae_operand_t{v, nullptr, nullptr, ARVAE_ACT_NONE}; }

static int layer_forward(const arvae_layer_t &l, int32_t n, const float *params, const float *in, const uint8_t *mask,
                         float *out, uint16_t *bits_out, float *link_ws, arvae_stream_t st, const float *wprep,
                         const unsigned *in_amax, unsigned *tmp_amax, unsigned *out_amax, bool *out_has, float *wide_prep = nullptr) {
    arvae_link_t lk = l.link;
    lk.n = n;
    const arvae_operand_t op = plain(in);
    const float *w = params + l.w_off, *b = l.b_off >= 0 ? params + l.b_off : nullptr;
    *out_has = false;
    if (bits_out != nullptr) {
        hipStream_t hs = as_stream(st);
        *out_has = true;
        if (conv32_fits(&lk)) {
            if (in_amax == nullptr) {
                if (int rc = conv32_amax(in, in_elems(l, n), tmp_amax, hs)) return rc;
                in_amax = tmp_amax;
            }
            return l.is_up ? conv32_up(&lk, make_operand(&op), b, 1, nullptr, nullptr, bits_out, out, hs, wprep, in_amax, out_amax)
                           : conv32_down(&lk, make_operand(&op), b, 1, nullptr, nullptr, bits_out, out, hs, wprep, in_amax, out_amax);
        }
        return conv_c1_down(&lk, make_operand(&op), w, b, 1, nullptr, nullptr, bits_out, out, hs, out_amax);
    }
    if (conv64_fits(&lk, l.is_up != 0) && tmp_amax != nullptr && !dense_fits(&lk) && !conv32_fits(&lk) && !conv_c1_fits(&lk)) {
        hipStream_t hs = as_stream(st);
        if (in_amax == nullptr && conv64s_fits(&lk, l.is_up != 0)) {
            if (int rc = conv32_amax(in, in_elems(l, n), tmp_amax, hs)) return rc;
            in_amax = tmp_amax;
        }
        *out_has = out_amax != nullptr;
        return l.is_up ? conv64_up(&lk, make_operand(&op), w, b, l.act, mask, out, link_ws, hs, nullptr, in_amax, *out_has ? out_amax : nullptr, wide_prep)
                       : conv64_down(&lk, make_operand(&op), w, b, l.act, mask, out, link_ws, hs, nullptr, in_amax, *out_has ? out_amax : nullptr,
                                     wide_prep);
    }
    if (!l.is_up && out_amax != nullptr && !dense_fits(&lk) && !conv32_fits(&lk) && !conv_c1_fits(&lk) && !conv64_fits(&lk, false) &&
        single_channel_down_fits(&lk)) {
        *out_has = true;
        return single_channel_down(&lk, make_operand(&op), w, b, l.act, mask, out, as_stream(st), out_amax);
    }
    return l.is_up ? arvae_link_up(&lk, &op, w, b, l.act, mask, out, link_ws, st)
                   : arvae_link_down(&lk, &op, w, b, l.act, mask, out, link_ws, st);
}

static int layer_backward(const arvae_layer_t &l, int32_t n, const float *params, float *grads, const float *in,
                          const float *out, const uint8_t *mask, const float *g, bool g_is_pre, const float *gate,
                          float *d_in, bool *gated, float *slab, float *link_ws, DenseWgradBatch *defer, float *own_slab,
                          SlabReduceBatch *rdefer, arvae_stream_t st, const float *g_scale = nullptr,
                          const uint16_t *gate_bits = nullptr, const float *wprep = nullptr, const GateOp *gate_op = nullptr,
                          const unsigned *g_amax = nullptr, const unsigned *in_amax = nullptr, unsigned *tmp_amax = nullptr,
                          unsigned *tmp2_amax = nullptr, unsigned *din_amax = nullptr, bool *din_has = nullptr, float *wide_prep = nullptr,
                          const float *c1_img = nullptr, float *c1_slab = nullptr, SlabJob *c1_job = nullptr,
                          const VaeFinishArgs *finish = nullptr, bool *finish_taken = nullptr) {
    arvae_link_t lk = l.link;
    lk.n = n;
    bool din_has_local = false;
    if (din_has == nullptr) din_has = &din_has_local;
    *din_has = false;
    const bool c32 = conv32_fits(&lk) && wprep != nullptr && tmp_amax != nullptr && tmp2_amax != nullptr;
    auto need_g = [&]() -> int {
        if (g_amax != nullptr) return ARVAE_OK;
        g_amax = tmp_amax;
        return conv32_amax(g, out_elems(l, n), tmp_amax, as_stream(st));
    };
    auto need_in = [&]() -> int {
        if (in_amax != nullptr) return ARVAE_OK;
        in_amax = tmp2_amax;
        return conv32_amax(in, in_elems(l, n), tmp2_amax, as_stream(st));
    };
    arvae_operand_t gop = g_is_pre ? plain(g) : arvae_operand_t{g, out, mask, l.act};
    if (!g_is_pre && (mask != nullptr || l.act != ARVAE_ACT_NONE) && (conv64_fits(&lk, false) || conv64_fits(&lk, true))) {
        const int64_t count = (int64_t)n * (l.is_up ? (int64_t)lk.hh * lk.hw * lk.chi : (int64_t)lk.lh * lk.lw * lk.clo);
        if (int rc = arvae_operand_apply(&gop, count, const_cast<float *>(g), st)) return rc;
        gop = plain(g);
        g_amax = nullptr;
    }
    const arvae_operand_t xin = plain(in);
    const float *w = params + l.w_off;
    float *dw = grads + l.w_off, *db = l.b_off >= 0 ? grads + l.b_off : nullptr;
    hipStream_t hs = as_stream(st);
    const arvae_stream_t wst = st;
    hipStream_t whs = hs;
    if (gated != nullptr) *gated = false;
    if (d_in != nullptr && gated != nullptr && rdefer != nullptr && own_slab != nullptr && gop.y == nullptr && g_scale == nullptr &&
        rdefer->count < SLAB_BATCH_MAX && c32 &&
        conv32_pair_fits(&lk, l.is_up != 0, gate, gate_bits, db ? (l.is_up ? 2 : 1) : 0)) {
        SlabJob job;
        if (int rc = need_g()) return rc;
        if (int rc = need_in()) return rc;
        const bool c1 = c1_img != nullptr && c1_slab != nullptr && c1_job != nullptr && conv32_pair_c1_fits(&lk, l.is_up != 0, gate_bits);
        if (int rc = conv32_pair(&lk, l.is_up != 0, gop.v, in, gate, gate_bits, d_in, wprep, dw, db, own_slab, hs, &job, g_amax, in_amax,
                                  c1 ? nullptr : din_amax, c1 ? c1_img : nullptr, c1 ? c1_slab : nullptr, c1 ? c1_job : nullptr))
            return rc;
        slab_reduce_defer(rdefer, job);
        if (c1) { *gated = true; *din_has = false; return ARVAE_OK; }
        *gated = true;
        *din_has = din_amax != nullptr;
        return ARVAE_OK;
    }
    const bool simple = gop.mask == nullptr && gop.act != ARVAE_ACT_SELU;
    if (d_in != nullptr && gated != nullptr && l.is_up && gate != nullptr && simple && gop.y == nullptr && rdefer != nullptr &&
        own_slab != nullptr && rdefer->count < SLAB_BATCH_MAX && conv_c1_pair_fits(&lk)) {
        Operand g_op = make_operand(&gop);
        g_op.scale = g_scale;
        SlabJob job;
        if (int rc = conv_c1_pair(&lk, g_op, w, gate_bits ? nullptr : gate, gate_bits, d_in, make_operand(&xin), dw, db, db ? 2 : 0, own_slab,
                                  hs, &job, din_amax, finish))
            return rc;
        if (finish != nullptr && finish_taken != nullptr) *finish_taken = true;
        slab_reduce_defer(rdefer, job);
        *gated = true;
        *din_has = din_amax != nullptr;
        return ARVAE_OK;
    }
    if (d_in != nullptr) {
        int rc;
        if (l.is_up) {
            if (gate != nullptr && gop.y == nullptr && c32) {
                if (int rc2 = need_g()) return rc2;
                rc = conv32_down(&lk, make_operand(&gop), nullptr, 0, gate_bits ? nullptr : gate, gate_bits, nullptr, d_in, hs, wprep,
                                 g_amax, din_amax);
                *gated = true;
                *din_has = din_amax != nullptr;
            } else if (gate != nullptr && simple && conv_c1_fits(&lk)) {
                Operand g_op = make_operand(&gop);
                g_op.scale = g_scale;
                rc = conv_c1_down(&lk, g_op, w, nullptr, 0, gate_bits ? nullptr : gate, gate_bits, nullptr, d_in, hs, din_amax);
                *gated = true;
                *din_has = din_amax != nullptr;
            } else if (gate_op != nullptr && !conv64_fits(&lk, false) && !conv_c1_fits(&lk) && single_channel_down_gated_fits(&lk)) {
                rc = single_channel_down_gated(&lk, make_operand(&gop), w, gate_op, d_in, hs, din_amax);
                *gated = true;
                *din_has = din_amax != nullptr && lk.n <= 1024;
            } else if (gate_op != nullptr && conv64s_fits(&lk, false)) {
                if (gop.y == nullptr && tmp_amax != nullptr)
                    if (int rc2 = need_g()) return rc2;
                rc = conv64_down(&lk, make_operand(&gop), w, nullptr, ARVAE_ACT_NONE, nullptr, d_in, link_ws, hs, gate_op,
                                 gop.y == nullptr ? g_amax : nullptr, din_amax, wide_prep);
                *gated = true;
                *din_has = din_amax != nullptr;
            } else {
                rc = arvae_link_down(&lk, &gop, w, nullptr, ARVAE_ACT_NONE, nullptr, d_in, link_ws, st);
            }
        } else {
            if (gate != nullptr && gop.y == nullptr && c32) {
                if (int rc2 = need_g()) return rc2;
                rc = conv32_up(&lk, make_operand(&gop), nullptr, 0, gate_bits ? nullptr : gate, gate_bits, nullptr, d_in, hs, wprep,
                               g_amax, din_amax);
                *gated = true;
                *din_has = din_amax != nullptr;
            } else if (gate != nullptr && dense_fits(&lk)) {
                rc = dense_dgrad(&lk, make_operand(&gop), w, gate, d_in, hs);
                *gated = true;
            } else if (gate_op != nullptr && conv64_fits(&lk, true)) {
                if (gop.y == nullptr && tmp_amax != nullptr)
                    if (int rc2 = need_g()) return rc2;
                rc = conv64_up(&lk, make_operand(&gop), w, nullptr, ARVAE_ACT_NONE, nullptr, d_in, link_ws, hs, gate_op,
                               gop.y == nullptr ? g_amax : nullptr, din_amax, wide_prep);
                *gated = true;
                *din_has = din_amax != nullptr;
            } else {
                rc = arvae_link_up(&lk, &gop, w, nullptr, ARVAE_ACT_NONE, nullptr, d_in, link_ws, st);
            }
        }
        if (rc) return rc;
    }
    if (rdefer != nullptr && own_slab != nullptr && gop.y == nullptr && rdefer->count < SLAB_BATCH_MAX &&
        ((conv32_fits(&lk) && tmp_amax != nullptr && tmp2_amax != nullptr) || conv_c1_fits(&lk))) {
        Operand lo_op = make_operand(l.is_up ? &xin : &gop), hi_op = make_operand(l.is_up ? &gop : &xin);
        (l.is_up ? hi_op : lo_op).scale = g_scale;
        const int bias_mode = db ? (l.is_up ? 2 : 1) : 0;
        SlabJob job;
        if (conv32_fits(&lk)) {
            if (int rc = need_g()) return rc;
            if (int rc = need_in()) return rc;
        }
        const int rc = conv32_fits(&lk) ? conv32_wgrad_partial(&lk, lo_op, hi_op, dw, db, bias_mode, own_slab, whs, &job,
                                                               l.is_up ? in_amax : g_amax, l.is_up ? g_amax : in_amax)
                       : (d_in == nullptr && !l.is_up && dense_wgrad_c1_fits(defer))
                           ? dense_wgrad_flush_with_c1(defer, &lk, lo_op, hi_op, dw, db, bias_mode, own_slab, whs, &job)
                           : conv_c1_wgrad_partial(&lk, lo_op, hi_op, dw, db, bias_mode, own_slab, whs, &job);
        if (rc) return rc;
        slab_reduce_defer(rdefer, job);
        return ARVAE_OK;
    }
    if (conv64_wgrad_fits(&lk) && !dense_fits(&lk) && !conv_c1_fits(&lk) && !conv32_fits(&lk) && tmp_amax != nullptr && tmp2_amax != nullptr) {
        const bool g_plain = gop.y == nullptr;
        if (g_plain)
            if (int rc = need_g()) return rc;
        if (int rc = need_in()) return rc;
        const unsigned *ga = g_plain ? g_amax : nullptr;
        return l.is_up ? link_wgrad_conv64(&lk, make_operand(&xin), make_operand(&gop), dw, db, db ? 2 : 0, slab, whs, in_amax, ga)
                       : link_wgrad_conv64(&lk, make_operand(&gop), make_operand(&xin), dw, db, db ? 1 : 0, slab, whs, ga, in_amax);
    }
    if (l.is_up) return arvae_link_wgrad(&lk, &xin, &gop, dw, db, db ? 2 : 0, slab, wst);
    if (defer != nullptr && dense_fits(&lk) && dense_wgrad_defer(defer, &lk, make_operand(&gop), in, dw, db)) return ARVAE_OK;
    return arvae_link_wgrad(&lk, &gop, &xin, dw, db, db ? 1 : 0, slab, wst);
}

static bool fold_conv_layers(const arvae_image_vae_t *m, const Layout &L, int batch, const uint8_t *const *masks, int mid_ne, int mid_nd) {
    const int e = m->n_enc - mid_ne - 1;
    return masks == nullptr && e >= 1 && mid_nd + 1 < m->n_dec && mid_fold_fits(m, batch) && L.dec_bits[mid_nd] >= 0 &&
           L.enc_slab[e] >= 0 && L.dec_slab[mid_nd] >= 0 && L.dec_wprep[mid_nd + 1] >= 0;
}

static int count_masks(const arvae_image_vae_t *m) {
    int c = 0;
    for (int i = 0; i < m->n_enc; ++i) c += m->enc[i].dropout != 0;
    for (int i = 0; i < m->n_dec; ++i) c += m->dec[i].dropout != 0;
    return c;
}

}

using namespace arvae;

extern "C" int64_t arvae_image_vae_ws_floats(const arvae_image_vae_t *model, int32_t batch, int64_t n_cols) {
    Layout L;
    if (make_layout(model, batch, n_cols, L)) return -1;
    return L.total;
}

extern "C" int arvae_image_vae_forward(const arvae_image_vae_t *m, int32_t batch, const float *params, const float *x,
                                       const float *labels, int64_t ld_labels, const float *eps,
                                       const uint8_t *const *masks, const float *capacity, const float *z_cols,
                                       const float *lab_cols, int64_t n_cols, float reg_scale, float *ws,
                                       float *scalars, float *mu, float *sigma, float *z, float *logits,
                                       arvae_stream_t stream) {
    Layout L;
    if (int rc = make_layout(m, batch, n_cols, L)) return rc;
    ARVAE_REQUIRE(params && x && eps && ws && scalars && mu && sigma && z && logits, "image_vae_forward: null pointer");
    ARVAE_REQUIRE(m->n_reg == 0 || n_cols < 0 || labels != nullptr, "image_vae_forward: labels needed for the reg loss");
    hipStream_t st = as_stream(stream);
    auto U = [&](int64_t off) { return reinterpret_cast<unsigned *>(ws + off); };
    int mi = 0;
    bool mid_prepped = false;
    int mid_ne = 0, mid_nd = 0;
    const bool mid = mid_fusable(m, &mid_ne, &mid_nd);
    int first = 0;
    {
        const float *wts[8];
        float *preps[8];
        int np = 0;
        for (int i = 0; i < m->n_enc; ++i)
            if (L.enc_wprep[i] >= 0) { wts[np] = params + m->enc[i].w_off; preps[np++] = ws + L.enc_wprep[i]; }
        for (int i = 0; i < m->n_dec; ++i)
            if (L.dec_wprep[i] >= 0) { wts[np] = params + m->dec[i].w_off; preps[np++] = ws + L.dec_wprep[i]; }
        if (np > 0 && mid) {
            MidPrepArgs margs;
            mid_prep_args(m, params, ws + L.mid_prep, &margs, batch);
            const arvae_layer_t &l0 = m->enc[0];
            arvae_link_t lk0 = l0.link;
            lk0.n = batch;
            static const bool no_pair = diag_env("ARVAE_NO_PAIR_PREP") != nullptr;
            if (!no_pair && m->n_enc - mid_ne > 1 && L.enc_bits[0] >= 0 && L.enc_wprep[0] < 0 && !l0.is_up && conv_c1_fits(&lk0) &&
                !(masks != nullptr && l0.dropout)) {
                const arvae_operand_t op = plain(x);
                if (int rc = conv_c1_down_with_prep(&lk0, make_operand(&op), params + l0.w_off, l0.b_off >= 0 ? params + l0.b_off : nullptr,
                                                    1, reinterpret_cast<uint16_t *>(ws + L.enc_bits[0]), ws + L.enc_out[0], wts, preps, np,
                                                    margs, st, U(L.enc_amax[0])))
                    return rc;
                first = 1;
            } else if (int rc = conv32_weight_prep_with_mid(wts, preps, np, margs, st)) return rc;
            mid_prepped = true;
        } else if (int rc = conv32_weight_prep(wts, preps, np, st)) return rc;
    }
    {
        const float *wts[4 * ARVAE_MAX_LAYERS];
        float *outs[4 * ARVAE_MAX_LAYERS];
        int tr[4 * ARVAE_MAX_LAYERS], qs[4 * ARVAE_MAX_LAYERS], nj = 0;
        auto add = [&](const arvae_layer_t &l, const int64_t (&slot)[2]) {
            for (int t = 0; t < 2; ++t)
                if (slot[t] >= 0) { wts[nj] = params + l.w_off; outs[nj] = ws + slot[t]; tr[nj] = t; qs[nj] = t ? l.link.chi : l.link.clo; ++nj; }
        };
        for (int i = 0; i < m->n_enc; ++i) add(m->enc[i], L.enc_wide[i]);
        for (int i = 0; i < m->n_dec; ++i) add(m->dec[i], L.dec_wide[i]);
        if (int rc = conv64s_prep_batch(wts, outs, tr, qs, nj, st)) return rc;
    }
    const bool fold = mid && fold_conv_layers(m, L, batch, masks, mid_ne, mid_nd);
    const float *h = first ? ws + L.enc_out[0] : x;
    const unsigned *h_amax = first ? U(L.enc_amax[0]) : nullptr;
    mi += first ? (m->enc[0].dropout != 0) : 0;
    for (int i = first; i < m->n_enc - mid_ne - (fold ? 1 : 0); ++i) {
        const uint8_t *mask = (masks != nullptr && m->enc[i].dropout) ? masks[mi] : nullptr;
        mi += m->enc[i].dropout != 0;
        uint16_t *bits = L.enc_bits[i] >= 0 ? reinterpret_cast<uint16_t *>(ws + L.enc_bits[i]) : nullptr;
        bool has = false;
        if (i + 1 < m->n_enc - mid_ne - (fold ? 1 : 0) && mask == nullptr && !(masks != nullptr && m->enc[i + 1].dropout) && bits != nullptr &&
            L.enc_bits[i + 1] >= 0 && L.enc_wprep[i] >= 0 && L.enc_wprep[i + 1] >= 0 && h_amax != nullptr && !m->enc[i].is_up && !m->enc[i + 1].is_up) {
            arvae_link_t la = m->enc[i].link, lb = m->enc[i + 1].link;
            la.n = lb.n = batch;
            if (conv32_down_chain_fits(&la, &lb)) {
                const arvae_layer_t &a = m->enc[i], &b = m->enc[i + 1];
                if (int rc = conv32_down_chain(&la, &lb, h, h_amax, a.b_off >= 0 ? params + a.b_off : nullptr, bits, ws + L.enc_out[i],
                                               ws + L.enc_wprep[i], U(L.enc_amax[i]), b.b_off >= 0 ? params + b.b_off : nullptr,
                                               reinterpret_cast<uint16_t *>(ws + L.enc_bits[i + 1]), ws + L.enc_out[i + 1],
                                               ws + L.enc_wprep[i + 1], U(L.enc_amax[i + 1]), st))
                    return rc;
                ++i;
                h = ws + L.enc_out[i];
                h_amax = U(L.enc_amax[i]);
                continue;
            }
        }
        if (int rc = layer_forward(m->enc[i], batch, params, h, mask, ws + L.enc_out[i], bits, ws + L.link_ws, stream,
                                   L.enc_wprep[i] >= 0 ? ws + L.enc_wprep[i] : nullptr, h_amax, i > 0 ? U(L.enc_amax[i - 1]) : U(L.tmp_amax),
                                   U(L.enc_amax[i]), &has, L.enc_wide[i][m->enc[i].is_up ? 1 : 0] >= 0 ? ws + L.enc_wide[i][m->enc[i].is_up ? 1 : 0] : nullptr))
            return rc;
        h = ws + L.enc_out[i];
        h_amax = has ? U(L.enc_amax[i]) : nullptr;
    }
    const int64_t bz = (int64_t)batch * m->zdim;
    bool heads_next = false;
    if (mid) {
        float *enc_y[ARVAE_MAX_LAYERS], *dec_y[ARVAE_MAX_LAYERS];
        for (int i = 0; i < mid_ne; ++i) enc_y[i] = ws + L.enc_out[m->n_enc - mid_ne + i];
        for (int i = 0; i < mid_nd; ++i) dec_y[i] = ws + L.dec_out[i];
        MidFold mf{};
        if (fold) {
            mf.hi_e = h;
            mf.hi_d = ws + L.dec_out[mid_nd];
            mf.hi_d_bits = reinterpret_cast<unsigned char *>(ws + L.dec_bits[mid_nd]);
            mf.hi_d_amax = U(L.dec_amax[mid_nd]);
        }
        if (int rc = mid_forward(m, batch, params, ws + L.mid_prep, fold ? ws + L.enc_out[m->n_enc - mid_ne - 1] : h, enc_y, dec_y, eps, mu,
                                 ws + L.log_std, sigma, z, st, mid_prepped, U(L.dec_amax[mid_nd - 1]), fold ? &mf : nullptr,
                                 L.mid_wide >= 0 ? ws + L.mid_wide : nullptr))
            return rc;
        h = fold ? ws + L.dec_out[mid_nd] : dec_y[mid_nd - 1];
        h_amax = fold ? U(L.dec_amax[mid_nd]) : U(L.dec_amax[mid_nd - 1]);
    } else if (heads_fusable(&m->head_mu, &m->head_log_std, m->zdim)) {
        heads_next = m->n_dec > 1 && heads_next_fusable(&m->dec[0], m->zdim) && !(masks != nullptr && m->dec[0].dropout);
        if (int rc = heads_latent_fwd(&m->head_mu, &m->head_log_std, batch, m->zdim, params, h, eps, mu, ws + L.log_std,
                                      sigma, z, st, m, heads_next ? &m->dec[0] : nullptr, heads_next ? ws + L.dec_out[0] : nullptr))
            return rc;
// ... 48 lines not shown
            VaeFinishArgs fa{};
            if (defer_finish) {
                const int64_t nc_d = reg_here ? reg_args.n_cols : (int64_t)batch;
                fa = vae_finish_args(ws + L.rec_ws, conv_c1_up_recon_blocks(&lk), batch, out_elems(m->dec[m->n_dec - 1], batch), mu, sigma,
                                     m->zdim, m->beta, capacity, reg_here ? ws + L.reg_ws : nullptr, nc_d, m->zdim, m->reg_dims, m->n_reg,
                                     m->gamma, m->delta, reg_scale, ws + L.dz_reg, ws + L.rec_out, ws + L.kld_out, ws + L.reg_out, scalars, 0);
            }
            if (int rc = conv_c1_up_recon(&lk, h, params + l.w_off, l.b_off >= 0 ? params + l.b_off : nullptr, logits, x,
                                          m->recon_dist, ws + L.rec_ws, ws + L.dlogits, st, &nb, defer_finish ? &fa : nullptr,
                                          reinterpret_cast<VaeFinishArgs *>(ws + L.fin_args)))
                return rc;
            h_amax = nullptr;
        } else {
            uint16_t *bits = L.dec_bits[i] >= 0 ? reinterpret_cast<uint16_t *>(ws + L.dec_bits[i]) : nullptr;
            bool has = false;
            if (int rc = layer_forward(m->dec[i], batch, params, h, mask, out, bits, ws + L.link_ws, stream,
                                       L.dec_wprep[i] >= 0 ? ws + L.dec_wprep[i] : nullptr, h_amax, i > 0 ? U(L.dec_amax[i - 1]) : U(L.tmp_amax),
                                       U(L.dec_amax[i]), &has, L.dec_wide[i][m->dec[i].is_up ? 1 : 0] >= 0 ? ws + L.dec_wide[i][m->dec[i].is_up ? 1 : 0] : nullptr))
                return rc;
            h_amax = has ? U(L.dec_amax[i]) : nullptr;
        }
        h = out;
    }
    const int64_t pix = out_elems(m->dec[m->n_dec - 1], batch);
    if (!recon_fused)
        if (int rc = recon_partials(logits, x, pix, batch, m->recon_dist, ws + L.rec_ws, ws + L.dlogits, st, &nb)) return rc;
    if (n_cols == -2) return ARVAE_OK;
    const int64_t nc = reg_here ? reg_args.n_cols : (int64_t)batch;
    if (reg_here && !reg_done)
        if (int rc = reg_partials(z, labels, batch, reg_args.zc, reg_args.lc, nc, m->zdim, ld_labels, reg_args.dims, m->n_reg, m->delta,
                                  ws + L.reg_ws, st))
            return rc;
    if (defer_finish) return ARVAE_OK;
    return vae_finish(ws + L.rec_ws, nb, batch, pix, mu, sigma, m->zdim, m->beta, capacity,
                      reg_here ? ws + L.reg_ws : nullptr, nc, m->zdim, m->reg_dims, m->n_reg, m->gamma, m->delta, reg_scale,
                      ws + L.dz_reg, ws + L.rec_out, ws + L.kld_out, ws + L.reg_out, scalars, st);
}

extern "C" int arvae_image_vae_finish(const arvae_image_vae_t *m, int32_t batch, const float *labels, int64_t ld_labels,
                                      const float *capacity, const float *z_cols, const float *lab_cols, int64_t n_cols,
                                      float reg_scale, float *ws, float *scalars, const float *mu, const float *sigma,
                                      const float *z, arvae_stream_t stream) {
    Layout L;
    if (int rc = make_layout(m, batch, n_cols, L)) return rc;
    ARVAE_REQUIRE(ws && scalars && mu && sigma && z, "image_vae_finish: null pointer");
    ARVAE_REQUIRE(m->n_reg == 0 || (labels && z_cols && lab_cols && n_cols >= batch), "image_vae_finish: gathered columns needed");
    hipStream_t st = as_stream(stream);
    const arvae_layer_t &last = m->dec[m->n_dec - 1];
    arvae_link_t lk = last.link;
    lk.n = batch;
    const int64_t pix = out_elems(last, batch);
    const bool recon_fused = last.is_up && last.act == ARVAE_ACT_NONE && last.dropout == 0 && conv_c1_fits(&lk) &&
                             arvae_recon_ws_floats(0) >= 2 * 1024;
    const int nb = recon_fused ? conv_c1_up_recon_blocks(&lk) : recon_partial_blocks(pix);
    const bool reg = m->n_reg > 0;
    if (reg) {
        RegDims rd;
        for (int i = 0; i < 16; ++i) rd.d[i] = i < m->n_reg ? m->reg_dims[i] : 0;
        for (int i = 0; i < m->n_reg; ++i)
            ARVAE_REQUIRE(m->reg_dims[i] >= 0 && m->reg_dims[i] < m->zdim && m->reg_dims[i] < ld_labels,
                          "image_vae_finish: reg dim %d outside z/labels", m->reg_dims[i]);
        if (finish_deferred(m)) {
            const VaeFinishArgs fa = vae_finish_args(ws + L.rec_ws, nb, batch, pix, mu, sigma, m->zdim, m->beta, capacity, ws + L.reg_ws, n_cols, m->zdim,
                                                     m->reg_dims, m->n_reg, m->gamma, m->delta, reg_scale, ws + L.dz_reg, ws + L.rec_out,
                                                     ws + L.kld_out, ws + L.reg_out, scalars, 0);
            return reg_partials(z, labels, batch, z_cols, lab_cols, n_cols, m->zdim, ld_labels, rd, m->n_reg, m->delta, ws + L.reg_ws, st, &fa,
                                reinterpret_cast<VaeFinishArgs *>(ws + L.fin_args));
        }
        if (int rc = reg_partials(z, labels, batch, z_cols, lab_cols, n_cols, m->zdim, ld_labels, rd, m->n_reg, m->delta, ws + L.reg_ws, st))
            return rc;
    }
    return vae_finish(ws + L.rec_ws, nb, batch, pix, mu, sigma, m->zdim, m->beta, capacity, reg ? ws + L.reg_ws : nullptr,
                      reg ? n_cols : (int64_t)batch, m->zdim, m->reg_dims, m->n_reg, m->gamma, m->delta, reg_scale, ws + L.dz_reg,
                      ws + L.rec_out, ws + L.kld_out, ws + L.reg_out, scalars, st);
}

extern "C" int arvae_image_vae_backward(const arvae_image_vae_t *m, int32_t batch, const float *params, float *grads,
                                        const float *x, const float *eps, const uint8_t *const *masks,
                                        const float *capacity, const float *mu, const float *sigma, const float *z,
                                        const float *logits, const float *g_loss, const float *dz_extra,
                                        int32_t reg_fused, float reg_scale, float *ws, arvae_stream_t stream) {
    Layout L;
    if (int rc = make_layout(m, batch, 0, L)) return rc;
    ARVAE_REQUIRE(params && grads && x && eps && mu && sigma && z && logits && g_loss && ws,
                  "image_vae_backward: null pointer");
    hipStream_t st = as_stream(stream);
    auto U = [&](int64_t off) { return reinterpret_cast<unsigned *>(ws + off); };
    auto grad_amax = [&](const float *p) -> unsigned * {
        if (p == nullptr) return nullptr;
        for (int i = 0; i < m->n_enc; ++i) if (p == ws + L.enc_keep[i]) return U(L.enc_gamax[i]);
        for (int i = 0; i < m->n_dec; ++i) if (p == ws + L.dec_keep[i]) return U(L.dec_gamax[i]);
        return p == ws + L.g_a ? U(L.ga_amax) : p == ws + L.g_b ? U(L.gb_amax) : nullptr;
    };
    auto in_amax_of = [&](bool dec, int i) -> const unsigned * {
        if (i == 0) return nullptr;
        const bool fast = (dec ? L.dec_bits[i] : L.enc_bits[i]) >= 0 && (dec ? L.dec_wprep[i] : L.enc_wprep[i]) >= 0;
        const arvae_layer_t &l = dec ? m->dec[i] : m->enc[i];
        arvae_link_t lk = l.link;
        lk.n = batch;
        const bool wide = conv64s_fits(&lk, l.is_up != 0) && !dense_fits(&lk) && !conv32_fits(&lk) && !conv_c1_fits(&lk);
        return (fast || wide) ? U(dec ? L.dec_amax[i - 1] : L.enc_amax[i - 1]) : nullptr;
    };
    const unsigned *cur_amax = nullptr;
    int enc_mask[ARVAE_MAX_LAYERS], dec_mask[ARVAE_MAX_LAYERS], mi = 0;
    for (int i = 0; i < m->n_enc; ++i) enc_mask[i] = m->enc[i].dropout ? mi++ : -1;
    for (int i = 0; i < m->n_dec; ++i) dec_mask[i] = m->dec[i].dropout ? mi++ : -1;
    auto mask_of = [&](int idx) -> const uint8_t * { return (masks != nullptr && idx >= 0) ? masks[idx] : nullptr; };

    float *const pp_a = ws + L.g_a, *const pp_b = ws + L.g_b, *slab = L.slab_floats ? ws + L.slab : nullptr;
    DenseWgradBatch defer;
    defer.count = 0;
    SlabReduceBatch rdefer;
    rdefer.count = 0;
    hipStream_t flush_stream = st;
    auto grad_dst = [&](int64_t keep, const float *busy) -> float * {
        if (keep >= 0) return ws + keep;
        return busy == pp_a ? pp_b : pp_a;
    };
    const int64_t pix = out_elems(m->dec[m->n_dec - 1], batch);
    const int64_t bz = (int64_t)batch * m->zdim;
    float *cur;
    const float *first_scale = nullptr;
    auto relu_gate = [&](const arvae_layer_t &producer, int mask_idx, const float *saved) -> const float * {
        return (producer.act == ARVAE_ACT_RELU && mask_of(mask_idx) == nullptr) ? saved : nullptr;
    };
    auto general_gate = [&](const arvae_layer_t &producer, int mask_idx, const float *saved, GateOp &go) -> const GateOp * {
        if (producer.act == ARVAE_ACT_NONE && mask_of(mask_idx) == nullptr) return nullptr;
        if (producer.act == ARVAE_ACT_RELU && mask_of(mask_idx) == nullptr) return nullptr;
        go.y = saved; go.mask = mask_of(mask_idx); go.act = producer.act;
        return &go;
    };
    bool pre = true;
    {
        const int li = m->n_dec - 1;
        const arvae_layer_t &last = m->dec[li];
        arvae_link_t lk = last.link;
        lk.n = batch;
        const bool fold = last.is_up && conv_c1_fits(&lk) && mask_of(dec_mask[li]) == nullptr && li > 0 &&
                          relu_gate(m->dec[li - 1], dec_mask[li - 1], ws + L.dec_out[li - 1]) != nullptr && L.dec_slab[li] >= 0;
        if (fold) {
            cur = ws + L.dlogits;
            first_scale = g_loss;
        } else {
            cur = grad_dst(L.dec_keep[li], nullptr);
            if (int rc = arvae_scale_by_scalar(g_loss, ws + L.dlogits, pix, cur, stream)) return rc;
        }
    }
    int mid_ne = 0, mid_nd = 0;
    const bool mid = mid_fusable(m, &mid_ne, &mid_nd);
    const bool fold = mid && fold_conv_layers(m, L, batch, masks, mid_ne, mid_nd);
    bool finish_pending = finish_deferred(m);
    const VaeFinishArgs *fin_dev = reinterpret_cast<const VaeFinishArgs *>(ws + L.fin_args);
    const float *heads_next_g = nullptr;
    for (int i = m->n_dec - 1; i >= (mid ? mid_nd + (fold ? 1 : 0) : 0); --i) {
        const float *in = i > 0 ? ws + L.dec_out[i - 1] : z;
        const float *out = (i + 1 < m->n_dec) ? ws + L.dec_out[i] : logits;
        const float *gate = i > 0 ? relu_gate(m->dec[i - 1], dec_mask[i - 1], in) : nullptr;
        GateOp go;
        const GateOp *gate_op = i > 0 ? general_gate(m->dec[i - 1], dec_mask[i - 1], in, go) : nullptr;
        float *dst = grad_dst(i > 0 ? L.dec_keep[i - 1] : -1, cur);
        bool gated = false;
        if (i == 0 && !mid && pre && m->n_dec > 1 && heads_fusable(&m->head_mu, &m->head_log_std, m->zdim) &&
            heads_next_fusable(&m->dec[0], m->zdim) && mask_of(dec_mask[0]) == nullptr) {
            heads_next_g = cur;
            dst = nullptr;
        }
        bool din_has = false;
        const bool carry = finish_pending && i == m->n_dec - 1;
        bool taken = false;
        if (int rc = layer_backward(m->dec[i], batch, params, grads, in, out, mask_of(dec_mask[i]), cur, pre, gate, dst,
                                    &gated, slab, ws + L.link_ws, &defer, L.dec_slab[i] >= 0 ? ws + L.dec_slab[i] : nullptr, &rdefer, stream,
                                    i == m->n_dec - 1 ? first_scale : nullptr,
                                    (gate != nullptr && i > 0 && L.dec_bits[i - 1] >= 0)
                                        ? reinterpret_cast<const uint16_t *>(ws + L.dec_bits[i - 1]) : nullptr,
                                    L.dec_wprep[i] >= 0 ? ws + L.dec_wprep[i] : nullptr, gate_op, cur_amax, in_amax_of(true, i),
                                    U(L.tmp_amax), U(L.tmp2_amax), grad_amax(dst), &din_has,
                                    L.dec_wide[i][m->dec[i].is_up ? 0 : 1] >= 0 ? ws + L.dec_wide[i][m->dec[i].is_up ? 0 : 1] : nullptr,
                                    nullptr, nullptr, nullptr, carry ? fin_dev : nullptr, carry ? &taken : nullptr))
            return rc;
        if (carry) {
            if (!taken)
                if (int rc = vae_finish_deferred(fin_dev, st)) return rc;
            finish_pending = false;
        }
        pre = gated;
        if (heads_next_g == nullptr) { cur = dst; cur_amax = din_has ? grad_amax(dst) : nullptr; }
    }
    const arvae_milestones *ms = m->milestones;
    bool dec_marked = false, lin_marked = false;
    if (ms != nullptr && ms->dec_grads != nullptr && defer.count == 0) {
        if (int rc = slab_reduce_flush(&rdefer, st)) return rc;
        mark(ms->dec_grads, st);
        dec_marked = true;
    }
    const float *hidden = ws + L.enc_out[m->n_enc - 1];
    const float *dz_reg = (reg_fused == 1 && m->n_reg > 0) ? ws + L.dz_reg : reg_fused == 2 ? dz_extra : nullptr;
    if (reg_fused == 2) {
        ARVAE_REQUIRE(dz_extra != nullptr, "image_vae_backward: reg_fused 2 needs the unit regulariser gradient in dz_extra");
        dz_extra = nullptr;
    }
    const float *head_gate = relu_gate(m->enc[m->n_enc - 1], enc_mask[m->n_enc - 1], hidden);
    float *d_hidden = grad_dst(L.enc_keep[m->n_enc - 1], nullptr);
    int enc_from = m->n_enc - 1;
    if (mid) {
        const int e0 = m->n_enc - mid_ne;
        float *enc_y[ARVAE_MAX_LAYERS], *dec_y[ARVAE_MAX_LAYERS], *enc_g[ARVAE_MAX_LAYERS], *dec_g[ARVAE_MAX_LAYERS];
        for (int i = 0; i < mid_ne; ++i) { enc_y[i] = ws + L.enc_out[e0 + i]; enc_g[i] = ws + L.enc_keep[e0 + i]; }
        for (int i = 0; i < mid_nd; ++i) { dec_y[i] = ws + L.dec_out[i]; dec_g[i] = ws + L.dec_keep[i]; }
        const float *x0 = ws + L.enc_out[e0 - 1];
        const float *gate0 = relu_gate(m->enc[e0 - 1], enc_mask[e0 - 1], x0);
        float *d_x0 = ws + L.enc_keep[e0 - 1];
        const float *g_last = cur;
        MidFold mf{};
        if (fold) {
            ARVAE_REQUIRE(pre, "image_vae_backward: the folded conv layer needs a gated upstream gradient");
            mf.hi_e = ws + L.enc_out[e0 - 2];
            mf.g_hi_d = cur;
            mf.d_hi_e = ws + L.enc_keep[e0 - 2];
            mf.d_hi_e_amax = grad_amax(mf.d_hi_e);
            mf.slab_e = ws + L.enc_slab[e0 - 1];
            mf.slab_d = ws + L.dec_slab[mid_nd];
        }
        if (int rc = mid_backward(m, batch, params, ws + L.mid_prep, enc_y, dec_y, enc_g, dec_g, g_last, (pre || fold) ? 1 : 0, gate0, d_x0, eps,
                                  mu, sigma, dz_reg, dz_extra, g_loss, ws + L.kld_out + 1, capacity, m->beta, reg_scale, ws + L.d_mu,
                                  ws + L.d_ls, st, grad_amax(d_x0), fold ? &mf : nullptr, L.mid_wide >= 0 ? ws + L.mid_wide : nullptr))
            return rc;
        if (fold) {
            const int n_wg = (batch + 31) / 32;
            const arvae_layer_t &ce = m->enc[e0 - 1], &cd = m->dec[mid_nd];
            SlabJob je{mf.slab_e, grads + ce.w_off, ce.b_off >= 0 ? grads + ce.b_off : nullptr, n_wg, SLAB_C32T, ce.b_off >= 0 ? 1 : 0};
            SlabJob jd{mf.slab_d, grads + cd.w_off, cd.b_off >= 0 ? grads + cd.b_off : nullptr, n_wg, SLAB_C32T, cd.b_off >= 0 ? 2 : 0};
            ARVAE_REQUIRE(slab_reduce_defer(&rdefer, jd) && slab_reduce_defer(&rdefer, je), "image_vae_backward: too many slab reductions queued");
        }
        auto queue = [&](const arvae_layer_t &l, const float *g, const float *in) -> int {
            arvae_link_t lk = l.link;
            lk.n = batch;
            float *dw = grads + l.w_off, *db = l.b_off >= 0 ? grads + l.b_off : nullptr;
            const arvae_operand_t gop = plain(g), xin = plain(in);
            if (dense_wgrad_defer(&defer, &lk, make_operand(&gop), in, dw, db)) return ARVAE_OK;
            return arvae_link_wgrad(&lk, &gop, &xin, dw, db, db ? 1 : 0, slab, stream);
        };
        int wide_took = 0;
        if (L.mid_wide >= 0)
            if (int rc = mid_wide_wgrad(m, batch, params, ws + L.mid_prep, ws + L.mid_wide, x0, (pre && !fold) ? g_last : dec_g[mid_nd - 1], grads,
                                        st, &wide_took))
                return rc;
        for (int i = mid_nd - 1; i >= 0; --i) {
            if (i == mid_nd - 1 && (wide_took & 2)) continue;
            if (int rc = queue(m->dec[i], (i == mid_nd - 1 && pre && !fold) ? g_last : dec_g[i], i > 0 ? dec_y[i - 1] : z)) return rc;
        }
        if (int rc = queue(m->head_mu, ws + L.d_mu, hidden)) return rc;
        if (int rc = queue(m->head_log_std, ws + L.d_ls, hidden)) return rc;
        for (int i = mid_ne - 1; i >= 0; --i) {
            if (i == 0 && (wide_took & 1)) continue;
            if (int rc = queue(m->enc[e0 + i], enc_g[i], i > 0 ? enc_y[i - 1] : x0)) return rc;
        }
        cur = fold ? mf.d_hi_e : d_x0;
        cur_amax = grad_amax(cur);
        pre = fold ? true : gate0 != nullptr;
        enc_from = fold ? e0 - 2 : e0 - 1;
        if (ms != nullptr && ms->linear_grads != nullptr) {
            if (int rc = dense_wgrad_flush(&defer, st)) return rc;
            mark(ms->linear_grads, st);
            lin_marked = true;
        }
    } else if (heads_fusable(&m->head_mu, &m->head_log_std, m->zdim)) {
        if (int rc = heads_latent_bwd(&m->head_mu, &m->head_log_std, batch, m->zdim, params, heads_next_g != nullptr ? nullptr : cur,
                                      dz_reg, dz_extra, mu, sigma, eps, g_loss, ws + L.kld_out + 1, capacity, m->beta, reg_scale,
                                      head_gate, ws + L.d_mu, ws + L.d_ls, d_hidden, st,
                                      heads_next_g != nullptr ? &m->dec[0] : nullptr, heads_next_g))
            return rc;
        const arvae_layer_t *heads[2] = {&m->head_mu, &m->head_log_std};
        const float *hg[2] = {ws + L.d_mu, ws + L.d_ls};
        for (int k = 0; k < 2; ++k) {
            arvae_link_t lk = heads[k]->link;
            lk.n = batch;
            float *dw = grads + heads[k]->w_off, *db = heads[k]->b_off >= 0 ? grads + heads[k]->b_off : nullptr;
            const arvae_operand_t gop = plain(hg[k]), xin = plain(hidden);
            if (!dense_wgrad_defer(&defer, &lk, make_operand(&gop), hidden, dw, db))
                if (int rc = arvae_link_wgrad(&lk, &gop, &xin, dw, db, db ? 1 : 0, slab, stream)) return rc;
        }
        cur = d_hidden;
        cur_amax = nullptr;
        pre = head_gate != nullptr;
    } else {
        int64_t blocks = (bz + 255) / 256;
        if (blocks > 1024) blocks = 1024;
        ARVAE_LAUNCH(latent_bwd_full_kernel, dim3((unsigned)blocks), dim3(256), 0, st, cur, dz_reg, dz_extra, mu, sigma,
                           eps, g_loss, ws + L.kld_out + 1, capacity, m->beta, 1.f / (float)batch, reg_scale, bz,
                           ws + L.d_mu, ws + L.d_ls);
        if (int rc = check_launch("image_vae_backward(latent)")) return rc;
        cur = d_hidden;
        float *other = grad_dst(-1, cur);
        if (int rc = layer_backward(m->head_mu, batch, params, grads, hidden, nullptr, nullptr, ws + L.d_mu, true, nullptr,
                                    cur, nullptr, slab, ws + L.link_ws, &defer, nullptr, nullptr, stream))
            return rc;
        if (int rc = layer_backward(m->head_log_std, batch, params, grads, hidden, nullptr, nullptr, ws + L.d_ls, true,
                                    nullptr, other, nullptr, slab, ws + L.link_ws, &defer, nullptr, nullptr, stream))
            return rc;
        const int64_t hn = in_elems(m->head_mu, batch);
        int64_t blocks2 = (hn + 255) / 256;
        if (blocks2 > 2048) blocks2 = 2048;
        ARVAE_LAUNCH(add_inplace_kernel, dim3((unsigned)blocks2), dim3(256), 0, st, cur, other, head_gate, hn);
        if (int rc = check_launch("image_vae_backward(add)")) return rc;
        pre = head_gate != nullptr;
        cur_amax = nullptr;
    }
    SlabJob c1_job{};
    bool c1_possible = false;
    if (enc_from >= 1 && masks == nullptr && L.enc_slab[0] >= 0 && L.enc_bits[0] >= 0) {
        arvae_link_t lk0 = m->enc[0].link;
        lk0.n = batch;
        c1_possible = !m->enc[0].is_up && m->enc[0].act == ARVAE_ACT_RELU && m->enc[0].dropout == 0 && conv_c1_fits(&lk0) && lk0.hh == 64 &&
                      lk0.hw == 64 && lk0.clo == 32 && m->enc[0].b_off >= 0;
    }
    for (int i = enc_from; i >= 0; --i) {
        if (i == 0 && c1_job.slab != nullptr) {
            c1_job.dwt = grads + m->enc[0].w_off;
            c1_job.dbias = grads + m->enc[0].b_off;
            ARVAE_REQUIRE(slab_reduce_defer(&rdefer, c1_job), "image_vae_backward: too many slab reductions queued");
            break;
        }
        const float *in = i > 0 ? ws + L.enc_out[i - 1] : x;
        const float *gate = i > 0 ? relu_gate(m->enc[i - 1], enc_mask[i - 1], in) : nullptr;
        GateOp go;
        const GateOp *gate_op = i > 0 ? general_gate(m->enc[i - 1], enc_mask[i - 1], in, go) : nullptr;
        float *dst = i > 0 ? grad_dst(L.enc_keep[i - 1], cur) : nullptr;
        bool gated = false;
        bool din_has = false;
        if (int rc = layer_backward(m->enc[i], batch, params, grads, in, ws + L.enc_out[i], mask_of(enc_mask[i]), cur, pre,
                                    gate, dst, &gated, slab, ws + L.link_ws, &defer, L.enc_slab[i] >= 0 ? ws + L.enc_slab[i] : nullptr, &rdefer,
                                    stream, nullptr,
// ... 20 lines not shown
```

ar-vae_amd/csrc/wgrad32r.h:

```cpp
#pragma once
#include "common.h"
#include "conv32_common.h"
#include "reduce.h"

namespace arvae {

template <int LO> struct RowStream {
    static constexpr int HW = 2 * LO;
    static constexpr int RB = HW * PIXB;
    static constexpr int HN = 16384 / RB;
    static constexpr int TR = 32 / LO;
    static constexpr int RING = 3 * HN;
    static constexpr int PCOLS = HW + 2;
    static constexpr int HP = WGRAD_PSB_H, LP = WGRAD_PSB_L;
    static constexpr int HPLANE = RING * PCOLS * HP;
    static constexpr int LPLANE = 32 * LP, LBUF = 2 * LPLANE;
    static constexpr int LDS_DW = 2 * HPLANE + 2 * LBUF;
    static constexpr int PRO = 2 * RB / 4096;
    static constexpr int STEPS_PER_IMG = LO * LO / 32;
};

#ifdef WGR_STAMPS
__device__ unsigned long long g_wgr_stamps[256 * 2 * 64 * 2];
#define WGR_STAMP(role, slot)                                                                             \
    do {                                                                                                  \
        if ((threadIdx.x & 255) == 0 && BID < 256 && (slot) < 64) {                                \
            g_wgr_stamps[((BID * 2 + (role)) * 64 + (slot)) * 2] = __builtin_readcyclecounter();   \
            g_wgr_stamps[((BID * 2 + (role)) * 64 + (slot)) * 2 + 1] = wall_clock64();             \
        }                                                                                                 \
    } while (0)
#else
#define WGR_STAMP(role, slot)
#endif

constexpr int WGR_DEPTH = 3;

template <int LO, int BIAS>
__device__ __forceinline__ void wgrad32r_body(const float *__restrict__ lo, const float *__restrict__ hi, float *__restrict__ slab,
                                              int n_img, int total_steps, int steps_per_wg, const unsigned *amax_lo,
                                              const unsigned *amax_hi, const int BID) {
    using RS = RowStream<LO>;
    constexpr int HN = RS::HN, RING = RS::RING, PCOLS = RS::PCOLS, HP = RS::HP, LP = RS::LP, RB = RS::RB;
    constexpr int HPLANE = RS::HPLANE, LPLANE = RS::LPLANE, LBUF = RS::LBUF;
    extern __shared__ __attribute__((aligned(16))) unsigned ring[];
    unsigned *lo_w = ring + 2 * HPLANE;
    const int wave = __builtin_amdgcn_readfirstlane(threadIdx.x >> 6);
    const int k0 = BID * steps_per_wg;
    const int k1 = min(k0 + steps_per_wg, total_steps);
    float *out = slab + (int64_t)BID * SLAB_C32_FLOATS;

    if (wave >= 4) {
        const int pt = threadIdx.x - 256, chunk = pt & 7;
        const __amdgpu_buffer_rsrc_t rs_hi = make_rsrc(hi, (int64_t)n_img * RS::HW * RB);
        const __amdgpu_buffer_rsrc_t rs_lo = make_rsrc(lo, (int64_t)n_img * LO * LO * PIXB);
        float4 bias4 = make_float4(0.f, 0.f, 0.f, 0.f);
        float sc_h = 1.f, sc_l = 1.f;
        const AmaxLoad al_h = amax_issue(amax_hi), al_l = amax_issue(amax_lo);
        auto put = [&](unsigned *dst, int plane, const float4 &v, float sc) __attribute__((always_inline)) {
            uint2 hv, lv;
            split_pair_h2(v.x, v.y, sc, hv.x, lv.x);
            split_pair_h2(v.z, v.w, sc, hv.y, lv.y);
            *reinterpret_cast<uint2 *>(dst) = hv;
            *reinterpret_cast<uint2 *>(dst + plane) = lv;
        };
        auto slot_of = [&](int k, int j) { const int s = HN * (k % 3) + j; return s < 0 ? s + RING : (s >= RING ? s - RING : s); };
        auto row_of = [&](int o) { return o / RB; };
        auto px_of = [&](int o) { return (o % RB) / PIXB; };

        float4 pv[RS::PRO];
        {
            const unsigned base = (unsigned)((HN * k0 - 1) * RB);
#pragma unroll
            for (int j = 0; j < RS::PRO; ++j) {
                const int o = j * 4096 + pt * 16;
                const bool ok = k0 < k1 && (HN * k0 - 1 + row_of(o)) >= 0;
                pv[j] = buf_load4(rs_hi, ok ? base + (unsigned)o : OOB);
            }
        }
        float4 hv[WGR_DEPTH][4], lv[WGR_DEPTH];
        auto issue = [&](auto dc, int k) __attribute__((always_inline)) {
            constexpr int d = decltype(dc)::value;
            const bool ok = k < k1;
            const unsigned hb = (unsigned)((HN * k + 1) * RB) + pt * 16, lb = (unsigned)k * 4096u + pt * 16;
#pragma unroll
            for (int j = 0; j < 4; ++j) hv[d][j] = buf_load4(rs_hi, ok ? hb + j * 4096 : OOB);
            lv[d] = buf_load4(rs_lo, ok ? lb : OOB);
        };
        auto commit = [&](auto dc, int k) __attribute__((always_inline)) {
            constexpr int d = decltype(dc)::value;
#pragma unroll
            for (int j = 0; j < 4; ++j) {
                const int o = j * 4096 + pt * 16;
                put(ring + (slot_of(k, row_of(o) + 1) * PCOLS + px_of(o) + 1) * HP + chunk * 2, HPLANE, hv[d][j], sc_h);
                if (BIAS == 2) { bias4.x += hv[d][j].x; bias4.y += hv[d][j].y; bias4.z += hv[d][j].z; bias4.w += hv[d][j].w; }
            }
            put(lo_w + (k & 1) * LBUF + (pt >> 3) * LP + chunk * 2, LPLANE, lv[d], sc_l);
            if (BIAS == 1) { bias4.x += lv[d].x; bias4.y += lv[d].y; bias4.z += lv[d].z; bias4.w += lv[d].w; }
        };
        WGR_STAMP(1, 0);
        static_for<0, WGR_DEPTH>([&](auto dc) __attribute__((always_inline)) { issue(dc, k0 + decltype(dc)::value); });
        sc_h = amax_scale(al_h).s;
        sc_l = amax_scale(al_l).s;
        for (int e = pt; e < 2 * RING * 2 * 16; e += 256) {
            const int dw = e & 15, side = (e >> 4) & 1, row = (e >> 5) % RING, t = (e >> 5) / RING;
            ring[t * HPLANE + (row * PCOLS + side * (PCOLS - 1)) * HP + dw] = 0u;
        }
#pragma unroll
        for (int j = 0; j < RS::PRO; ++j) {
            const int o = j * 4096 + pt * 16;
            put(ring + (slot_of(k0, row_of(o) - 1) * PCOLS + px_of(o) + 1) * HP + chunk * 2, HPLANE, pv[j], sc_h);
            if (BIAS == 2 && k0 == 0) { bias4.x += pv[j].x; bias4.y += pv[j].y; bias4.z += pv[j].z; bias4.w += pv[j].w; }
        }
        commit(std::integral_constant<int, 0>{}, k0);
        WGR_STAMP(1, 1);
        __syncthreads();
#define ARVAE_WGR_PRODUCE(D)                                                          \
        if (k + D >= k1) break;                                                       \
        WGR_STAMP(1, 2 + 2 * (k + D - k0));                                           \
        issue(std::integral_constant<int, D>{}, k + D + WGR_DEPTH);                   \
        commit(std::integral_constant<int, (D + 1) % WGR_DEPTH>{}, k + D + 1);        \
        WGR_STAMP(1, 3 + 2 * (k + D - k0));                                           \
        __syncthreads();
        for (int k = k0;; k += WGR_DEPTH) {
            ARVAE_WGR_PRODUCE(0)
            ARVAE_WGR_PRODUCE(1)
            ARVAE_WGR_PRODUCE(2)
        }
#undef ARVAE_WGR_PRODUCE
        WGR_STAMP(1, 63);
        if (BIAS != 0) {
            float *red = reinterpret_cast<float *>(ring);
            *reinterpret_cast<float4 *>(red + pt * 4) = bias4;
            __builtin_amdgcn_fence(__ATOMIC_RELEASE, "workgroup");
        }
    } else {
        const int lane = threadIdx.x & 63, half = lane >> 5, rc = lane & 31;
        const int g16 = lane >> 4, q = (lane & 15) >> 2, pp = lane & 3;
        const AmaxLoad al_h = amax_issue(amax_hi), al_l = amax_issue(amax_lo);
        int loff[2][2], hcol[2][2], hrow[2];
#pragma unroll
        for (int b = 0; b < 2; ++b) {
            hrow[b] = 2 * ((16 * b + 8 * half) / LO) + wave;
#pragma unroll
            for (int i = 0; i < 2; ++i) {
                const int P = 16 * b + 8 * half + 4 * i + q;
                loff[b][i] = P * LP + 8 * (g16 & 1) + 2 * pp;
                hcol[b][i] = (2 * (P % LO)) * HP + 8 * (g16 & 1) + 2 * pp;
            }
        }
        f32x16 acc[4];
#pragma unroll
        for (int kx = 0; kx < 4; ++kx)
#pragma unroll
            for (int i = 0; i < 16; ++i) acc[kx][i] = 0.f;
        f16x8 a2[2][4][2], b2[2][2];
        const unsigned *lbuf = lo_w, *hrow0 = ring, *hrow1 = ring;
        auto set_step = [&](int k) __attribute__((always_inline)) {
            const int slot0 = (HN * (k % 3) + RING - 1) % RING;
            lbuf = lo_w + (k & 1) * LBUF;
            int s0 = slot0 + hrow[0], s1 = slot0 + hrow[1];
            s0 = s0 >= RING ? s0 - RING : s0;
            s1 = s1 >= RING ? s1 - RING : s1;
            hrow0 = ring + s0 * (PCOLS * HP);
            hrow1 = ring + s1 * (PCOLS * HP);
        };
        auto read_block = [&](auto bc) __attribute__((always_inline)) {
            constexpr int b = decltype(bc)::value;
#pragma unroll
            for (int t = 0; t < 2; ++t) b2[b][t] = lds_tr_f16x8(lbuf + t * LPLANE + loff[b][0], lbuf + t * LPLANE + loff[b][1]);
            const unsigned *hb = b == 0 ? hrow0 : hrow1;
#pragma unroll
            for (int kx = 0; kx < 4; ++kx)
#pragma unroll
                for (int t = 0; t < 2; ++t)
                    a2[b][kx][t] = lds_tr_f16x8(hb + kx * HP + t * HPLANE + hcol[b][0], hb + kx * HP + t * HPLANE + hcol[b][1]);
        };
        auto mask_b = [&](auto bc, int k) __attribute__((always_inline)) {
            constexpr int b = decltype(bc)::value;
            if (wave == 0 || wave == 3) {
                const int rimg = (RS::TR * k + (16 * b + 8 * half) / LO) & (LO - 1);
                const bool outside = wave == 0 ? rimg == 0 : rimg == LO - 1;
                typedef int i32x4q __attribute__((ext_vector_type(4)));
#pragma unroll
                for (int t = 0; t < 2; ++t) {
                    i32x4q v = __builtin_bit_cast(i32x4q, b2[b][t]);
                    v.x = outside ? 0 : v.x; v.y = outside ? 0 : v.y; v.z = outside ? 0 : v.z; v.w = outside ? 0 : v.w;
                    b2[b][t] = __builtin_bit_cast(f16x8, v);
                }
            }
        };
        auto mfma_block = [&](auto bc) __attribute__((always_inline)) {
            constexpr int b = decltype(bc)::value;
#define ARVAE_WGR_PRODUCT(TA, TB)                                                     \
            _Pragma("unroll") for (int kx = 0; kx < 4; ++kx) MFMA_H(acc[kx], a2[b][kx][TA], b2[b][TB]);
            ARVAE_WGR_PRODUCT(1, 0)
            ARVAE_WGR_PRODUCT(0, 1)
            ARVAE_WGR_PRODUCT(0, 0)
#undef ARVAE_WGR_PRODUCT
        };
        const float inv = amax_scale(al_l).inv * amax_scale(al_h).inv;
        WGR_STAMP(0, 0);
        __syncthreads();
        WGR_STAMP(0, 1);
        set_step(k0);
        read_block(std::integral_constant<int, 0>{});
#define ARVAE_WGR_INTERLEAVE                                                                                      \
        { _Pragma("unroll") for (int g_ = 0; g_ < 8; ++g_) {                                                      \
              __builtin_amdgcn_sched_group_barrier(0x008, 1, 0); __builtin_amdgcn_sched_group_barrier(0x100, 4, 0); } \
          _Pragma("unroll") for (int g_ = 0; g_ < 4; ++g_) {                                                      \
              __builtin_amdgcn_sched_group_barrier(0x008, 1, 0); __builtin_amdgcn_sched_group_barrier(0x100, 2, 0); } }
        for (int k = k0; k < k1; ++k) {
            __builtin_amdgcn_sched_barrier(0);
            mask_b(std::integral_constant<int, 0>{}, k);
            read_block(std::integral_constant<int, 1>{});
            mfma_block(std::integral_constant<int, 0>{});
            ARVAE_WGR_INTERLEAVE
            __builtin_amdgcn_sched_barrier(0);
            WGR_STAMP(0, 2 + 2 * (k - k0));
            __syncthreads();
            WGR_STAMP(0, 3 + 2 * (k - k0));
            set_step(k + 1);
            mask_b(std::integral_constant<int, 1>{}, k);
            __builtin_amdgcn_sched_barrier(0);
            read_block(std::integral_constant<int, 0>{});
            mfma_block(std::integral_constant<int, 1>{});
            ARVAE_WGR_INTERLEAVE
            __builtin_amdgcn_sched_barrier(0);
        }
#undef ARVAE_WGR_INTERLEAVE
        WGR_STAMP(0, 62);
#pragma unroll
        for (int kx = 0; kx < 4; ++kx)
#pragma unroll
            for (int g = 0; g < 4; ++g)
                *reinterpret_cast<float4 *>(out + ((wave * 4 + kx) * C32 + rc) * C32 + 8 * g + 4 * half) =
                    make_float4(acc[kx][4 * g] * inv, acc[kx][4 * g + 1] * inv, acc[kx][4 * g + 2] * inv, acc[kx][4 * g + 3] * inv);
        WGR_STAMP(0, 63);
    }
    if (BIAS != 0) {
        __syncthreads();
        if (threadIdx.x < C32) {
            const float *red = reinterpret_cast<const float *>(ring);
            const int qq = threadIdx.x >> 2, e = threadIdx.x & 3;
            float tot = 0.f;
            for (int j = 0; j < 32; ++j) tot += red[(j * 8 + qq) * 4 + e];
            out[16 * C32 * C32 + threadIdx.x] = tot;
        }
    }
}

template <int LO, int BIAS>
__global__ __launch_bounds__(512, 2) void wgrad32r_kernel(const float *__restrict__ lo, const float *__restrict__ hi,
                                                          float *__restrict__ slab, int n_img, int total_steps, int steps_per_wg,
                                                          const unsigned *amax_lo, const unsigned *amax_hi) {
    wgrad32r_body<LO, BIAS>(lo, hi, slab, n_img, total_steps, steps_per_wg, amax_lo, amax_hi, blockIdx.x);
}

}
```

Baseline: 1.414 million.

## Recompute decoder output-layer gradient inside paired down/wgrad conv kernel instead of materializing it

Adds a GD3 path where the paired down-conv and weight-gradient kernel computes the 32x32 gradient on the fly from the upstream 64x64 gradient, the small 4-tap weights and the gate sign bits, rather than reading a precomputed tensor. The intent is to drop a separate kernel plus a write and read of the intermediate gradient, and to derive its scaling maxima locally. It also folds the VAE finishing step into a spare workgroup of the c1 weight-gradient launch. In exchange, both consumers redundantly recompute the gradient rows, and each block does an extra max scan over its input range.

```diff
diff --git a/ar-vae_amd/csrc/conv32.hip b/ar-vae_amd/csrc/conv32.hip
--- a/ar-vae_amd/csrc/conv32.hip
+++ b/ar-vae_amd/csrc/conv32.hip
@@ -984,6 +984,13 @@
     if ((int)blockIdx.x < grid_a) down32p_body<LO, MODE>(g_hi, ep, n_img, tiles_a, blockIdx.x, grid_a);
     else wgrad32r_body<LO, BIAS>(w_lo, w_hi, slab, n_img, total_steps, steps_per_wg, amax_lo, amax_hi, blockIdx.x - grid_a);
 }
+template <int MODE, int BIAS>
+__global__ __launch_bounds__(512) __attribute__((amdgpu_waves_per_eu(2, 2))) void pair_down_wgrad_gd3_kernel(
+    Gd3Src gd3, Ep32 ep, int n_img, int tiles_a, int grid_a, const float *__restrict__ w_lo, float *__restrict__ slab, int total_steps,
+    int steps_per_wg, const unsigned *amax_lo) {
+    if ((int)blockIdx.x < grid_a) down32p_body<16, MODE, 0, true>(nullptr, ep, n_img, tiles_a, blockIdx.x, grid_a, nullptr, gd3);
+    else wgrad32r_body<16, BIAS, true>(w_lo, nullptr, slab, n_img, total_steps, steps_per_wg, amax_lo, nullptr, blockIdx.x - grid_a, gd3);
+}
 template <int MODE, int BIAS, bool C1W = false>
 __global__ __launch_bounds__(512) __attribute__((amdgpu_waves_per_eu(2, 2))) void pair_up16_wgrad_kernel(
     const float *__restrict__ g_lo, Ep32 ep, int n_img, int tiles_a, int grid_a, const float *__restrict__ w_lo, const float *__restrict__ w_hi,
@@ -1400,6 +1407,36 @@
     return check_launch(up ? "pair4(down32 + wgrad32)" : "pair4(up32 + wgrad32)");
 }
 
+bool conv32_pair_gd3_fits(const arvae_link_t *l, const float *gate, const uint16_t *gate_bits, int bias_mode) {
+    static const bool off = diag_env("ARVAE_NO_FUSED_GD3") != nullptr;
+    return !off && conv32_fits(l) && l->lh == 16 && conv32_pair_fits(l, true, gate, gate_bits, bias_mode);
+}
+int conv32_pair_gd3(const arvae_link_t *l, const float *d, const float *d_scale, const float *w4, const uint16_t *g_bits,
+                    const float *x_in, const uint16_t *gate_bits, float *d_in, const float *wprep, float *dwt, float *dbias, float *slab,
+                    hipStream_t s, SlabJob *job, const unsigned *amax_x, unsigned *amax_out) {
+    ARVAE_REQUIRE(wprep != nullptr && amax_x != nullptr && d != nullptr && w4 != nullptr && g_bits != nullptr && gate_bits != nullptr,
+                  "conv32_pair_gd3: prepared weights, the input's maxima, the sources of the gradient and the sign bits are needed");
+    Ep32 ep{nullptr, nullptr, gate_bits, nullptr, d_in, reinterpret_cast<const uint4 *>(wprep), nullptr, amax_out};
+    const Gd3Src src{d, d_scale, w4, g_bits};
+    const int cus = cu_count() < AMAX_N / 4 ? cu_count() : AMAX_N / 4;
+    int grid_a = cus * PAIR_SPLIT_PERCENT / 100;
+    if (grid_a < 1) grid_a = 1;
+    const int tiles_a = l->n * DownK<16>::TILES_PER_IMG;
+    {
+        const int run = (tiles_a + grid_a - 1) / grid_a;
+        grid_a = (tiles_a + run - 1) / run;
+    }
+    int total, spw, grid_b;
+    stream_geometry(l, cus - grid_a, total, spw, grid_b);
+    constexpr int LDS = MaxOf<RowStream<16>::LDS_DW * 4, DownK<16>::LDS_DW * 4>::value;
+    static std::once_flag attr;
+    std::call_once(attr, [&] { allow_lds(pair_down_wgrad_gd3_kernel<EP_GATE_B, 2>, LDS); });
+    ARVAE_LAUNCH((pair_down_wgrad_gd3_kernel<EP_GATE_B, 2>), dim3(grid_a + grid_b), dim3(512), LDS, s, src, ep, l->n, tiles_a, grid_a, x_in, slab,
+                 total, spw, amax_x);
+    *job = SlabJob{slab, dwt, dbias, grid_b, SLAB_C32, 2};
+    return check_launch("pair(down32<16> + wgrad32<16>)");
+}
+
 int conv32_wgrad(const arvae_link_t *l, const Operand &lo, const Operand &hi, float *dwt, float *dbias, int bias_mode,
                  float *slab, hipStream_t s, const unsigned *amax_lo, const unsigned *amax_hi) {
     SlabJob job;
diff --git a/ar-vae_amd/csrc/conv_c1.hip b/ar-vae_amd/csrc/conv_c1.hip
--- a/ar-vae_amd/csrc/conv_c1.hip
+++ b/ar-vae_amd/csrc/conv_c1.hip
@@ -231,6 +231,18 @@
     __shared__ __attribute__((aligned(16))) float lo_s[WGS_WAVES * LO1 * WS1];
     __shared__ __attribute__((aligned(16))) float im_s[WGS_WAVES * 4 * IMS];
     wgrad_c1s_body(lo, img, slab, n_rows, blockIdx.x, gridDim.x, lo_s, im_s);
+}
+
+__global__ __launch_bounds__(64 * WGS_WAVES) void wgrad_c1s_finish_kernel(Operand lo, Operand img, float *__restrict__ slab, int n_rows,
+                                                                         const VaeFinishArgs *__restrict__ fin) {
+    __shared__ __attribute__((aligned(16))) float raw[WGS_WAVES * LO1 * WS1 + WGS_WAVES * 4 * IMS];
+    if (blockIdx.x == 0) {
+        static_assert(64 * WGS_WAVES == 512, "the finishing body is instantiated for this kernel's 512 threads");
+        const VaeFinishArgs args = *fin;
+        vae_finish_body<512>(args, reinterpret_cast<float4 *>(raw));
+        return;
+    }
+    wgrad_c1s_body(lo, img, slab, n_rows, (int)blockIdx.x - 1, (int)gridDim.x - 1, raw, raw + WGS_WAVES * LO1 * WS1);
 }
 
 template <int GATE>
@@ -458,9 +470,15 @@
 int64_t conv_c1_wgrad_ws_floats(const arvae_link_t *l) { return (int64_t)wgrad_c1_groups(l) * WG1_SLAB; }
 
 int conv_c1_wgrad_partial(const arvae_link_t *l, const Operand &lo, const Operand &img, float *dwt, float *dbias,
-                          int bias_mode, float *slab, hipStream_t s, SlabJob *job) {
-    const int grid = wgrad_c1_groups(l);
-    ARVAE_LAUNCH(wgrad_c1s_kernel, dim3(grid), dim3(64 * WGS_WAVES), 0, s, lo, img, slab, l->n * LO1);
+                          int bias_mode, float *slab, hipStream_t s, SlabJob *job, const VaeFinishArgs *finish) {
+    int grid = wgrad_c1_groups(l);
+    if (finish != nullptr && grid > 1) {
+        grid -= 1;
+        ARVAE_LAUNCH(wgrad_c1s_finish_kernel, dim3(grid + 1), dim3(64 * WGS_WAVES), 0, s, lo, img, slab, l->n * LO1, finish);
+    } else {
+        ARVAE_REQUIRE(finish == nullptr, "conv_c1_wgrad_partial: no workgroup to spare for the finishing step");
+        ARVAE_LAUNCH(wgrad_c1s_kernel, dim3(grid), dim3(64 * WGS_WAVES), 0, s, lo, img, slab, l->n * LO1);
+    }
     *job = SlabJob{slab, dwt, dbias, grid, SLAB_C1, bias_mode};
     return check_launch("wgrad_c1_kernel");
 }
@@ -496,7 +514,7 @@
 int conv_c1_wgrad(const arvae_link_t *l, const Operand &lo, const Operand &img, float *dwt, float *dbias, int bias_mode,
                   float *slab, hipStream_t s) {
     SlabJob job;
-    if (int rc = conv_c1_wgrad_partial(l, lo, img, dwt, dbias, bias_mode, slab, s, &job)) return rc;
+    if (int rc = conv_c1_wgrad_partial(l, lo, img, dwt, dbias, bias_mode, slab, s, &job, nullptr)) return rc;
     return slab_reduce(job, s);
 }
 
diff --git a/ar-vae_amd/csrc/down32p.h b/ar-vae_amd/csrc/down32p.h
--- a/ar-vae_amd/csrc/down32p.h
+++ b/ar-vae_amd/csrc/down32p.h
@@ -1,6 +1,7 @@
 #pragma once
 #include "common.h"
 #include "conv32_common.h"
+#include "gd3.h"
 
 namespace arvae {
 
@@ -23,9 +24,10 @@
     static constexpr int TILES_PER_IMG = LO / T::TR;
 };
 
-template <int LO, int MODE, int CHAIN = 0>
+template <int LO, int MODE, int CHAIN = 0, bool GD3 = false>
 __device__ __forceinline__ void down32p_body(const float *__restrict__ hi, Ep32 ep, int n_img, int n_tiles, const int BID, const int NBLK,
-                                             float *chain_max = nullptr) {
+                                             float *chain_max = nullptr, const Gd3Src gd3 = Gd3Src{}) {
+    static_assert(!GD3 || (LO == 16 && CHAIN == 0), "the computed input is the 32 x 32 gradient of the dSprites decoder");
     using K = DownK<LO>;
     constexpr int HW = K::HW, PIX = K::PIX, SLOTS = K::SLOTS, HI = 2 * LO;
     extern __shared__ __attribute__((aligned(16))) unsigned ldsd[];
@@ -35,6 +37,11 @@
     const int t_end = min(n_tiles, t_first + per_wg);
     using S0 = std::integral_constant<int, 0>;
     using S1 = std::integral_constant<int, 1>;
+    Gd3Ctx gc{};
+    if constexpr (GD3) {
+        constexpr int RPT = 2 * K::T::TR;
+        gc = gd3_setup(gd3, n_img, t_first * RPT - 1, t_end * RPT + 1);
+    }
     auto chain_scale = [&]() __attribute__((always_inline)) -> Pow2 {
         const float m = fmaxf(fmaxf(chain_max[0], chain_max[1]), fmaxf(chain_max[2], chain_max[3]));
         return pow2_for((unsigned)__builtin_amdgcn_readfirstlane(__builtin_bit_cast(int, m)));
@@ -47,14 +54,22 @@
         const int pt = threadIdx.x - 256;
         const __amdgpu_buffer_rsrc_t rs_hi = make_rsrc(hi, (int64_t)n_img * HI * HI * PIXB);
         int q = pt & 7, pix0 = pt >> 3;
-        float4 lv[2][SLOTS];
+        constexpr int GROWS = GD3 ? (K::PR + 3) / 4 : 1;
+        float4 lv[2][GD3 ? 1 : SLOTS];
+        Gd3Row gv[2][GROWS];
+        (void)lv; (void)gv;
         float sc_in = 1.f;
         AmaxLoad al{};
-        if constexpr (CHAIN != 2) al = amax_issue(ep.amax_in);
+        if constexpr (CHAIN != 2 && !GD3) al = amax_issue(ep.amax_in);
         auto issue = [&](auto set_, int s, int tile) __attribute__((always_inline)) {
             constexpr int set = decltype(set_)::value;
             int img0, r0;
             tile_origin<LO, 64>(tile, img0, r0);
+            if constexpr (GD3) {
+                const int pr = (wave - 4) + 4 * s, gy = 2 * r0 - 1 + pr;
+                gv[set][s] = gd3_issue(gc, tile < t_end && pr < K::PR && (unsigned)gy < (unsigned)HI, img0 * HI + gy);
+                return;
+            }
             const int pix = pix0 + 32 * s, pr = pix / HW, px = pix - pr * HW;
             const int gy = 2 * r0 - 1 + pr;
             const bool ok = tile < t_end && pix < PIX && (unsigned)gy < (unsigned)HI;
@@ -62,6 +77,20 @@
         };
         auto commit = [&](auto set_, int s, unsigned *buf) __attribute__((always_inline)) {
             constexpr int set = decltype(set_)::value;
+            if constexpr (GD3) {
+                const int pr = (wave - 4) + 4 * s;
+                if (pr >= K::PR) return;
+                const f32x16 acc = gd3_row(gc, gv[set][s]);
+                unsigned *d = buf + (pr * HW + (lane & 31)) * PSB2 + (lane >> 5) * 2;
+#pragma unroll
+                for (int g = 0; g < 4; ++g) {
+                    uint2 hv, lw;
+                    gd3_split(gc, acc, g, hv, lw);
+                    *reinterpret_cast<uint2 *>(d + 4 * g) = hv;
+                    *reinterpret_cast<uint2 *>(d + 4 * g + 16) = lw;
+                }
+                return;
+            }
             const int pix = pix0 + 32 * s;
             if (SLOTS * 32 > PIX && pix >= PIX) return;
             uint2 hv, lw;
@@ -71,18 +100,20 @@
             *reinterpret_cast<uint2 *>(d) = hv;
             *reinterpret_cast<uint2 *>(d + 16) = lw;
         };
-#pragma unroll
-        for (int s = 0; s < SLOTS; ++s) issue(S0{}, s, t_first);
-#pragma unroll
-        for (int s = 0; s < SLOTS; ++s) issue(S1{}, s, t_first + 1);
+        constexpr int NS = GD3 ? GROWS : SLOTS;
+#pragma unroll
+        for (int s = 0; s < NS; ++s) issue(S0{}, s, t_first);
+#pragma unroll
+        for (int s = 0; s < NS; ++s) issue(S1{}, s, t_first + 1);
         if (pt < 2 * PSB2) ldsd[(pt / PSB2) * K::BUF + PIX * PSB2 + pt % PSB2] = 0u;
-        if constexpr (CHAIN != 2) sc_in = amax_scale(al).s;
+        if constexpr (GD3) sc_in = gc.in.s;
+        else if constexpr (CHAIN != 2) sc_in = amax_scale(al).s;
         else sc_in = chain_scale().s;
         __syncthreads();
 #pragma unroll
-        for (int s = 0; s < SLOTS; ++s) commit(S0{}, s, ldsd);
-#pragma unroll
-        for (int s = 0; s < SLOTS; ++s) issue(S0{}, s, t_first + 2);
+        for (int s = 0; s < NS; ++s) commit(S0{}, s, ldsd);
+#pragma unroll
+        for (int s = 0; s < NS; ++s) issue(S0{}, s, t_first + 2);
         __syncthreads();
         const unsigned rel0 = (unsigned)(pix0 * PIXB + q * 16);
         unsigned first_row = 0, last_row = 0, no_slot = 0;
@@ -107,10 +138,18 @@
                 n_base = nt < t_end ? (unsigned)(((ni * HI + gy0) * HI) * PIXB) + rel0 : OOB;
                 n_bad = (gy0 < 0 ? first_row : 0u) | (gy0 + PIX / HW - 1 >= HI ? last_row : 0u) | no_slot;
             }
-#pragma unroll
-            for (int s = 0; s < SLOTS; ++s) {
-                commit(set_, s, nb);
-                lv[set][s] = buf_load4(rs_hi, (n_bad & (1u << s)) != 0 ? OOB : n_base + 4096u * s);
+            if constexpr (GD3) {
+#pragma unroll
+                for (int s = 0; s < NS; ++s) {
+                    commit(set_, s, nb);
+                    issue(set_, s, tile + 3);
+                }
+            } else {
+#pragma unroll
+                for (int s = 0; s < SLOTS; ++s) {
+                    commit(set_, s, nb);
+                    lv[set][s] = buf_load4(rs_hi, (n_bad & (1u << s)) != 0 ? OOB : n_base + 4096u * s);
+                }
             }
             DSTAMP(1, 5 + 5 * pst);
             __syncthreads();
@@ -131,7 +170,7 @@
     (void)cst;
     const int half = lane >> 5, rc = lane & 31;
     AmaxLoad al{};
-    if constexpr (CHAIN != 2) al = amax_issue(ep.amax_in);
+    if constexpr (CHAIN != 2 && !GD3) al = amax_issue(ep.amax_in);
     int xoff[2][4];
 #pragma unroll
     for (int mt = 0; mt < 2; ++mt) {
@@ -165,7 +204,8 @@
             for (int t = 0; t < 2; ++t) w2[st][t] = __builtin_bit_cast(f16x8, wp[(st * 2 + t) * 64]);
     }
     float inv;
-    if constexpr (CHAIN != 2) inv = amax_scale(al).inv * prep_inv_scale(ep.wprep);
+    if constexpr (GD3) inv = gc.in.inv * prep_inv_scale(ep.wprep);
+    else if constexpr (CHAIN != 2) inv = amax_scale(al).inv * prep_inv_scale(ep.wprep);
     else inv = chain_scale().inv * prep_inv_scale(ep.wprep);
     float amax_run = 0.f;
     __syncthreads();
diff --git a/ar-vae_amd/csrc/gd3.h b/ar-vae_amd/csrc/gd3.h
--- /dev/null
+++ b/ar-vae_amd/csrc/gd3.h
@@ -0,0 +1,128 @@
+#pragma once
+#include "common.h"
+#include "conv32_common.h"
+
+namespace arvae {
+
+struct Gd3Src {
+    const float *d = nullptr;
+    const float *scale = nullptr;
+    const float *w4 = nullptr;
+    const uint16_t *bits = nullptr;
+};
+
+constexpr int GD3_H = 32, GD3_DH = 64;
+
+struct Gd3Ctx {
+    __amdgpu_buffer_rsrc_t rs_d, rs_bits;
+    f16x8 wa[2];
+    float gs;
+    float sd;
+    float c;
+    float inv_acc;
+    Pow2 in;
+    int n_rows;
+};
+
+typedef float gd3_f2 __attribute__((ext_vector_type(2)));
+struct Gd3Row { gd3_f2 v0, v1; unsigned gb; };
+
+__device__ __forceinline__ Gd3Ctx gd3_setup(const Gd3Src &src, int n_img, int g0, int g1) {
+    __shared__ float gd3_max[8];
+    const int lane = threadIdx.x & 63, half = lane >> 5, rc = lane & 31;
+    Gd3Ctx c;
+    c.n_rows = n_img * GD3_H;
+    c.rs_d = make_rsrc(src.d, (int64_t)n_img * GD3_DH * GD3_DH * 4);
+    c.rs_bits = make_rsrc(src.bits, (int64_t)n_img * GD3_H * GD3_H * 4);
+    c.gs = src.scale != nullptr ? src.scale[0] : 1.f;
+    float m = 0.f;
+    {
+        const int r0 = max(0, 2 * g0 - 1), r1 = min(n_img * GD3_DH, 2 * g1 + 1);
+        const float4 *p = reinterpret_cast<const float4 *>(src.d) + (int64_t)r0 * (GD3_DH / 4);
+        const int nf4 = (r1 - r0) * (GD3_DH / 4);
+        for (int i = threadIdx.x; i < nf4; i += 512) m = fmaxf(m, amax4(p[i]));
+    }
+    m = wave_max(m);
+    if (lane == 0) gd3_max[threadIdx.x >> 6] = m;
+    const float4 wa4 = *reinterpret_cast<const float4 *>(src.w4 + rc * 16 + 8 * half);
+    const float4 wb4 = *reinterpret_cast<const float4 *>(src.w4 + rc * 16 + 8 * half + 4);
+    const float w[8] = {wa4.x, wa4.y, wa4.z, wa4.w, wb4.x, wb4.y, wb4.z, wb4.w};
+    float wm = 0.f, ws = 0.f;
+#pragma unroll
+    for (int i = 0; i < 8; ++i) { wm = fmaxf(wm, fabsf(w[i])); ws += fabsf(w[i]); }
+    ws += __shfl_xor(ws, 32);
+    wm = wave_max(wm);
+    ws = wave_max(ws);
+    const Pow2 pw = pow2_for((unsigned)__builtin_amdgcn_readfirstlane(__builtin_bit_cast(int, wm)));
+    {
+        uint4 h, l;
+        split_pair_h2(w[0], w[1], pw.s, h.x, l.x);
+        split_pair_h2(w[2], w[3], pw.s, h.y, l.y);
+        split_pair_h2(w[4], w[5], pw.s, h.z, l.z);
+        split_pair_h2(w[6], w[7], pw.s, h.w, l.w);
+        c.wa[0] = __builtin_bit_cast(f16x8, h);
+        c.wa[1] = __builtin_bit_cast(f16x8, l);
+    }
+    __syncthreads();
+    float md = 0.f;
+#pragma unroll
+    for (int i = 0; i < 8; ++i) md = fmaxf(md, gd3_max[i]);
+    md *= fabsf(c.gs);
+    const Pow2 pd = pow2_for((unsigned)__builtin_amdgcn_readfirstlane(__builtin_bit_cast(int, md)));
+    c.sd = pd.s;
+    c.in = pow2_for((unsigned)__builtin_amdgcn_readfirstlane(__builtin_bit_cast(int, md * ws)));
+    c.inv_acc = pd.inv * pw.inv;
+    c.c = (c.in.s * pd.inv) * pw.inv;
+    return c;
+}
+
+__device__ __forceinline__ Gd3Row gd3_issue(const Gd3Ctx &c, bool ok, int g) {
+    const int lane = threadIdx.x & 63, half = lane >> 5, rc = lane & 31;
+    ok = ok && (unsigned)g < (unsigned)c.n_rows;
+    const int n = g >> 5, y = g & (GD3_H - 1);
+    Gd3Row r;
+    auto row = [&](int q) __attribute__((always_inline)) -> gd3_f2 {
+        const int dy = 2 * y - 1 + 2 * half + q;
+        const bool okq = ok && (unsigned)dy < (unsigned)GD3_DH;
+        const unsigned off = okq ? (unsigned)((((n * GD3_DH + dy) * GD3_DH) + 2 * rc) * 4) : OOB;
+        return __builtin_bit_cast(gd3_f2, __builtin_amdgcn_raw_buffer_load_b64(c.rs_d, (int)off, 0, 0));
+    };
+    r.v0 = row(0);
+    r.v1 = row(1);
+    r.gb = buf_load_u16(c.rs_bits, ok ? (unsigned)(((g * GD3_H + rc) * 2 + half) * 2) : OOB);
+    return r;
+}
+
+__device__ __forceinline__ f32x16 gd3_row(const Gd3Ctx &c, const Gd3Row &r) {
+    const int rc = threadIdx.x & 31;
+    uint4 xh, xl;
+    {
+        const float a = c.gs * r.v0.x, b = c.gs * r.v0.y;
+        const float left = __shfl_up(b, 1, 32), right = __shfl_down(a, 1, 32);
+        split_pair_h2(rc == 0 ? 0.f : left, a, c.sd, xh.x, xl.x);
+        split_pair_h2(b, rc == 31 ? 0.f : right, c.sd, xh.y, xl.y);
+    }
+    {
+        const float a = c.gs * r.v1.x, b = c.gs * r.v1.y;
+        const float left = __shfl_up(b, 1, 32), right = __shfl_down(a, 1, 32);
+        split_pair_h2(rc == 0 ? 0.f : left, a, c.sd, xh.z, xl.z);
+        split_pair_h2(b, rc == 31 ? 0.f : right, c.sd, xh.w, xl.w);
+    }
+    const f16x8 bh = __builtin_bit_cast(f16x8, xh), bl = __builtin_bit_cast(f16x8, xl);
+    f32x16 acc;
+#pragma unroll
+    for (int i = 0; i < 16; ++i) acc[i] = 0.f;
+    MFMA_H(acc, c.wa[1], bh);
+    MFMA_H(acc, c.wa[0], bl);
+    MFMA_H(acc, c.wa[0], bh);
+#pragma unroll
+    for (int i = 0; i < 16; ++i) acc[i] = ((r.gb >> i) & 1u) ? acc[i] : 0.f;
+    return acc;
+}
+
+__device__ __forceinline__ void gd3_split(const Gd3Ctx &c, const f32x16 &acc, int g, uint2 &hv, uint2 &lw) {
+    split_pair_h2(acc[4 * g], acc[4 * g + 1], c.c, hv.x, lw.x);
+    split_pair_h2(acc[4 * g + 2], acc[4 * g + 3], c.c, hv.y, lw.y);
+}
+
+}
diff --git a/ar-vae_amd/csrc/plan.hip b/ar-vae_amd/csrc/plan.hip
--- a/ar-vae_amd/csrc/plan.hip
+++ b/ar-vae_amd/csrc/plan.hip
@@ -68,7 +68,15 @@
                  const Operand &w_lo, float *dwt, float *dbias, int bias_mode, float *slab, hipStream_t s, SlabJob *job,
                  unsigned *amax_out, const VaeFinishArgs *finish = nullptr);
 int conv_c1_wgrad_partial(const arvae_link_t *l, const Operand &lo, const Operand &img, float *dwt, float *dbias,
-                          int bias_mode, float *slab, hipStream_t s, SlabJob *job);
+                          int bias_mode, float *slab, hipStream_t s, SlabJob *job, const VaeFinishArgs *finish = nullptr);
+bool conv32_pair_gd3_fits(const arvae_link_t *l, const float *gate, const uint16_t *gate_bits, int bias_mode);
+int conv32_pair_gd3(const arvae_link_t *l, const float *d, const float *d_scale, const float *w4, const uint16_t *g_bits,
+                    const float *x_in, const uint16_t *gate_bits, float *d_in, const float *wprep, float *dwt, float *dbias, float *slab,
+                    hipStream_t s, SlabJob *job, const unsigned *amax_x, unsigned *amax_out);
+struct Gd3Plan {
+    const float *d, *d_scale, *w4;
+    const uint16_t *bits;
+};
 bool dense_wgrad_c1_fits(const DenseWgradBatch *b);
 int dense_wgrad_flush_with_c1(DenseWgradBatch *b, const arvae_link_t *l, const Operand &lo, const Operand &img, float *dwt, float *dbias,
                               int bias_mode, float *slab, hipStream_t s, SlabJob *job);
@@ -320,7 +328,7 @@
                           const unsigned *g_amax = nullptr, const unsigned *in_amax = nullptr, unsigned *tmp_amax = nullptr,
                           unsigned *tmp2_amax = nullptr, unsigned *din_amax = nullptr, bool *din_has = nullptr, float *wide_prep = nullptr,
                           const float *c1_img = nullptr, float *c1_slab = nullptr, SlabJob *c1_job = nullptr,
-                          const VaeFinishArgs *finish = nullptr, bool *finish_taken = nullptr) {
+                          const VaeFinishArgs *finish = nullptr, bool *finish_taken = nullptr, const Gd3Plan *gd3 = nullptr) {
     arvae_link_t lk = l.link;
     lk.n = n;
     bool din_has_local = false;
@@ -351,6 +359,19 @@
     const arvae_stream_t wst = st;
     hipStream_t whs = hs;
     if (gated != nullptr) *gated = false;
+    if (gd3 != nullptr) {
+        ARVAE_REQUIRE(d_in != nullptr && gated != nullptr && rdefer != nullptr && own_slab != nullptr && c32 && l.is_up && db != nullptr &&
+                          gate_bits != nullptr && g_is_pre && in_amax != nullptr && rdefer->count < SLAB_BATCH_MAX,
+                      "layer_backward: this layer cannot compute its incoming gradient");
+        SlabJob job;
+        if (int rc = conv32_pair_gd3(&lk, gd3->d, gd3->d_scale, gd3->w4, gd3->bits, in, gate_bits, d_in, wprep, dw, db, own_slab, hs, &job,
+                                      in_amax, din_amax))
+            return rc;
+        slab_reduce_defer(rdefer, job);
+        *gated = true;
+        *din_has = din_amax != nullptr;
+        return ARVAE_OK;
+    }
     if (d_in != nullptr && gated != nullptr && rdefer != nullptr && own_slab != nullptr && gop.y == nullptr && g_scale == nullptr &&
         rdefer->count < SLAB_BATCH_MAX && c32 &&
         conv32_pair_fits(&lk, l.is_up != 0, gate, gate_bits, db ? (l.is_up ? 2 : 1) : 0)) {
@@ -448,8 +469,10 @@
                                                                l.is_up ? in_amax : g_amax, l.is_up ? g_amax : in_amax)
                        : (d_in == nullptr && !l.is_up && dense_wgrad_c1_fits(defer))
                            ? dense_wgrad_flush_with_c1(defer, &lk, lo_op, hi_op, dw, db, bias_mode, own_slab, whs, &job)
-                           : conv_c1_wgrad_partial(&lk, lo_op, hi_op, dw, db, bias_mode, own_slab, whs, &job);
+                           : conv_c1_wgrad_partial(&lk, lo_op, hi_op, dw, db, bias_mode, own_slab, whs, &job,
+                                                   (d_in == nullptr && l.is_up && finish_taken != nullptr) ? finish : nullptr);
         if (rc) return rc;
+        if (!conv32_fits(&lk) && d_in == nullptr && l.is_up && finish != nullptr && finish_taken != nullptr) *finish_taken = true;
         slab_reduce_defer(rdefer, job);
         return ARVAE_OK;
     }
@@ -804,7 +827,23 @@
     bool finish_pending = finish_deferred(m);
     const VaeFinishArgs *fin_dev = reinterpret_cast<const VaeFinishArgs *>(ws + L.fin_args);
     const float *heads_next_g = nullptr;
-    for (int i = m->n_dec - 1; i >= (mid ? mid_nd + (fold ? 1 : 0) : 0); --i) {
+    const int dec_stop = mid ? mid_nd + (fold ? 1 : 0) : 0;
+    bool gd3_on = false;
+    Gd3Plan gd3_plan{};
+    auto gd3_fits = [&](int li) -> bool {
+        if (li < 2 || li - 1 < dec_stop || cur != ws + L.dlogits || first_scale == nullptr || !pre) return false;
+        const arvae_layer_t &a = m->dec[li], &b = m->dec[li - 1];
+        arvae_link_t la = a.link, lb = b.link;
+        la.n = lb.n = batch;
+        if (!a.is_up || !conv_c1_pair_fits(&la) || L.dec_bits[li - 1] < 0 || L.dec_slab[li] < 0 || rdefer.count + 2 > SLAB_BATCH_MAX) return false;
+        if (relu_gate(b, dec_mask[li - 1], ws + L.dec_out[li - 1]) == nullptr) return false;
+        const float *gate_b = relu_gate(m->dec[li - 2], dec_mask[li - 2], ws + L.dec_out[li - 2]);
+        if (!b.is_up || gate_b == nullptr || L.dec_bits[li - 2] < 0 || L.dec_wprep[li - 1] < 0 || L.dec_slab[li - 1] < 0 || b.b_off < 0 ||
+            in_amax_of(true, li - 1) == nullptr)
+            return false;
+        return conv32_pair_gd3_fits(&lb, gate_b, reinterpret_cast<const uint16_t *>(ws + L.dec_bits[li - 2]), 2);
+    };
+    for (int i = m->n_dec - 1; i >= dec_stop; --i) {
         const float *in = i > 0 ? ws + L.dec_out[i - 1] : z;
         const float *out = (i + 1 < m->n_dec) ? ws + L.dec_out[i] : logits;
         const float *gate = i > 0 ? relu_gate(m->dec[i - 1], dec_mask[i - 1], in) : nullptr;
@@ -818,9 +857,14 @@
             dst = nullptr;
         }
         bool din_has = false;
+        if (i == m->n_dec - 1) gd3_on = gd3_fits(i);
+        const bool gd3_first = gd3_on && i == m->n_dec - 1, gd3_second = gd3_on && i == m->n_dec - 2;
+        if (gd3_first) {
+            gd3_plan = Gd3Plan{cur, first_scale, params + m->dec[i].w_off, reinterpret_cast<const uint16_t *>(ws + L.dec_bits[i - 1])};
+        }
         const bool carry = finish_pending && i == m->n_dec - 1;
         bool taken = false;
-        if (int rc = layer_backward(m->dec[i], batch, params, grads, in, out, mask_of(dec_mask[i]), cur, pre, gate, dst,
+        if (int rc = layer_backward(m->dec[i], batch, params, grads, in, out, mask_of(dec_mask[i]), cur, pre, gate, gd3_first ? nullptr : dst,
                                     &gated, slab, ws + L.link_ws, &defer, L.dec_slab[i] >= 0 ? ws + L.dec_slab[i] : nullptr, &rdefer, stream,
                                     i == m->n_dec - 1 ? first_scale : nullptr,
                                     (gate != nullptr && i > 0 && L.dec_bits[i - 1] >= 0)
@@ -828,8 +872,10 @@
                                     L.dec_wprep[i] >= 0 ? ws + L.dec_wprep[i] : nullptr, gate_op, cur_amax, in_amax_of(true, i),
                                     U(L.tmp_amax), U(L.tmp2_amax), grad_amax(dst), &din_has,
                                     L.dec_wide[i][m->dec[i].is_up ? 0 : 1] >= 0 ? ws + L.dec_wide[i][m->dec[i].is_up ? 0 : 1] : nullptr,
-                                    nullptr, nullptr, nullptr, carry ? fin_dev : nullptr, carry ? &taken : nullptr))
-            return rc;
+                                    nullptr, nullptr, nullptr, carry ? fin_dev : nullptr, carry ? &taken : nullptr,
+                                    gd3_second ? &gd3_plan : nullptr))
+            return rc;
+        if (gd3_first) gated = true;
         if (carry) {
             if (!taken)
                 if (int rc = vae_finish_deferred(fin_dev, st)) return rc;
diff --git a/ar-vae_amd/csrc/wgrad32r.h b/ar-vae_amd/csrc/wgrad32r.h
--- a/ar-vae_amd/csrc/wgrad32r.h
+++ b/ar-vae_amd/csrc/wgrad32r.h
@@ -2,6 +2,7 @@
 #include "common.h"
 #include "conv32_common.h"
 #include "reduce.h"
+#include "gd3.h"
 
 namespace arvae {
 
@@ -35,10 +36,11 @@
 
 constexpr int WGR_DEPTH = 3;
 
-template <int LO, int BIAS>
+template <int LO, int BIAS, bool GD3 = false>
 __device__ __forceinline__ void wgrad32r_body(const float *__restrict__ lo, const float *__restrict__ hi, float *__restrict__ slab,
                                               int n_img, int total_steps, int steps_per_wg, const unsigned *amax_lo,
-                                              const unsigned *amax_hi, const int BID) {
+                                              const unsigned *amax_hi, const int BID, const Gd3Src gd3 = Gd3Src{}) {
+    static_assert(!GD3 || LO == 16, "the computed input is the 32 x 32 gradient of the dSprites decoder");
     using RS = RowStream<LO>;
     constexpr int HN = RS::HN, RING = RS::RING, PCOLS = RS::PCOLS, HP = RS::HP, LP = RS::LP, RB = RS::RB;
     constexpr int HPLANE = RS::HPLANE, LPLANE = RS::LPLANE, LBUF = RS::LBUF;
@@ -48,6 +50,8 @@
     const int k0 = BID * steps_per_wg;
     const int k1 = min(k0 + steps_per_wg, total_steps);
     float *out = slab + (int64_t)BID * SLAB_C32_FLOATS;
+    Gd3Ctx gc{};
+    if constexpr (GD3) gc = gd3_setup(gd3, n_img, HN * k0 - 1, k0 < k1 ? HN * k1 + 1 : HN * k0 - 1);
 
     if (wave >= 4) {
         const int pt = threadIdx.x - 256, chunk = pt & 7;
@@ -55,7 +59,29 @@
         const __amdgpu_buffer_rsrc_t rs_lo = make_rsrc(lo, (int64_t)n_img * LO * LO * PIXB);
         float4 bias4 = make_float4(0.f, 0.f, 0.f, 0.f);
         float sc_h = 1.f, sc_l = 1.f;
-        const AmaxLoad al_h = amax_issue(amax_hi), al_l = amax_issue(amax_lo);
+        AmaxLoad al_h{};
+        if constexpr (!GD3) al_h = amax_issue(amax_hi);
+        const AmaxLoad al_l = amax_issue(amax_lo);
+        const int pw = wave - 4;
+        float4 gbias[4];
+#pragma unroll
+        for (int g = 0; g < 4; ++g) gbias[g] = make_float4(0.f, 0.f, 0.f, 0.f);
+        (void)gbias;
+        auto put_row = [&](const Gd3Row &r, int slot, bool sum) __attribute__((always_inline)) {
+            const f32x16 acc = gd3_row(gc, r);
+            const int ln = threadIdx.x & 63;
+            unsigned *dst = ring + (slot * PCOLS + (ln & 31) + 1) * HP + (ln >> 5) * 2;
+#pragma unroll
+            for (int g = 0; g < 4; ++g) {
+                uint2 hv, lw;
+                gd3_split(gc, acc, g, hv, lw);
+                *reinterpret_cast<uint2 *>(dst + 4 * g) = hv;
+                *reinterpret_cast<uint2 *>(dst + 4 * g + HPLANE) = lw;
+                if (BIAS == 2 && sum) {
+                    gbias[g].x += acc[4 * g]; gbias[g].y += acc[4 * g + 1]; gbias[g].z += acc[4 * g + 2]; gbias[g].w += acc[4 * g + 3];
+                }
+            }
+        };
         auto put = [&](unsigned *dst, int plane, const float4 &v, float sc) __attribute__((always_inline)) {
             uint2 hv, lv;
             split_pair_h2(v.x, v.y, sc, hv.x, lv.x);
@@ -68,7 +94,11 @@
         auto px_of = [&](int o) { return (o % RB) / PIXB; };
 
         float4 pv[RS::PRO];
-        {
+        Gd3Row gpv{};
+        (void)pv;
+        if constexpr (GD3) {
+            if (pw < 2) gpv = gd3_issue(gc, k0 < k1 && HN * k0 - 1 + pw >= 0, HN * k0 - 1 + pw);
+        } else {
             const unsigned base = (unsigned)((HN * k0 - 1) * RB);
 #pragma unroll
             for (int j = 0; j < RS::PRO; ++j) {
@@ -77,19 +107,25 @@
                 pv[j] = buf_load4(rs_hi, ok ? base + (unsigned)o : OOB);
             }
         }
-        float4 hv[WGR_DEPTH][4], lv[WGR_DEPTH];
+        float4 hv[WGR_DEPTH][GD3 ? 1 : 4], lv[WGR_DEPTH];
+        Gd3Row gv[WGR_DEPTH];
+        (void)hv; (void)gv;
         auto issue = [&](auto dc, int k) __attribute__((always_inline)) {
             constexpr int d = decltype(dc)::value;
             const bool ok = k < k1;
             const unsigned hb = (unsigned)((HN * k + 1) * RB) + pt * 16, lb = (unsigned)k * 4096u + pt * 16;
-#pragma unroll
-            for (int j = 0; j < 4; ++j) hv[d][j] = buf_load4(rs_hi, ok ? hb + j * 4096 : OOB);
+            if constexpr (GD3) gv[d] = gd3_issue(gc, ok, HN * k + 1 + pw);
+            else {
+#pragma unroll
+                for (int j = 0; j < 4; ++j) hv[d][j] = buf_load4(rs_hi, ok ? hb + j * 4096 : OOB);
+            }
             lv[d] = buf_load4(rs_lo, ok ? lb : OOB);
         };
         auto commit = [&](auto dc, int k) __attribute__((always_inline)) {
             constexpr int d = decltype(dc)::value;
-#pragma unroll
-            for (int j = 0; j < 4; ++j) {
+            if constexpr (GD3) put_row(gv[d], slot_of(k, pw + 1), true);
+#pragma unroll
+            for (int j = 0; j < (GD3 ? 0 : 4); ++j) {
                 const int o = j * 4096 + pt * 16;
                 put(ring + (slot_of(k, row_of(o) + 1) * PCOLS + px_of(o) + 1) * HP + chunk * 2, HPLANE, hv[d][j], sc_h);
                 if (BIAS == 2) { bias4.x += hv[d][j].x; bias4.y += hv[d][j].y; bias4.z += hv[d][j].z; bias4.w += hv[d][j].w; }
@@ -99,14 +135,17 @@
         };
         WGR_STAMP(1, 0);
         static_for<0, WGR_DEPTH>([&](auto dc) __attribute__((always_inline)) { issue(dc, k0 + decltype(dc)::value); });
-        sc_h = amax_scale(al_h).s;
+        if constexpr (!GD3) sc_h = amax_scale(al_h).s;
         sc_l = amax_scale(al_l).s;
         for (int e = pt; e < 2 * RING * 2 * 16; e += 256) {
             const int dw = e & 15, side = (e >> 4) & 1, row = (e >> 5) % RING, t = (e >> 5) / RING;
             ring[t * HPLANE + (row * PCOLS + side * (PCOLS - 1)) * HP + dw] = 0u;
         }
-#pragma unroll
-        for (int j = 0; j < RS::PRO; ++j) {
+        if constexpr (GD3) {
+            if (pw < 2) put_row(gpv, slot_of(k0, pw - 1), k0 == 0);
+        }
+#pragma unroll
+        for (int j = 0; j < (GD3 ? 0 : RS::PRO); ++j) {
             const int o = j * 4096 + pt * 16;
             put(ring + (slot_of(k0, row_of(o) - 1) * PCOLS + px_of(o) + 1) * HP + chunk * 2, HPLANE, pv[j], sc_h);
             if (BIAS == 2 && k0 == 0) { bias4.x += pv[j].x; bias4.y += pv[j].y; bias4.z += pv[j].z; bias4.w += pv[j].w; }
@@ -130,13 +169,31 @@
         WGR_STAMP(1, 63);
         if (BIAS != 0) {
             float *red = reinterpret_cast<float *>(ring);
+            if constexpr (GD3) {
+                const int ln = threadIdx.x & 63;
+                float4 mine = make_float4(0.f, 0.f, 0.f, 0.f);
+#pragma unroll
+                for (int g = 0; g < 4; ++g) {
+                    float4 t = gbias[g];
+#pragma unroll
+                    for (int o = 16; o > 0; o >>= 1) {
+                        t.x += __shfl_xor(t.x, o); t.y += __shfl_xor(t.y, o); t.z += __shfl_xor(t.z, o); t.w += __shfl_xor(t.w, o);
+                    }
+                    const int from = 32 * (ln & 1);
+                    const float4 u = make_float4(__shfl(t.x, from), __shfl(t.y, from), __shfl(t.z, from), __shfl(t.w, from));
+                    if (ln < 8 && (ln >> 1) == g) mine = make_float4(u.x * gc.inv_acc, u.y * gc.inv_acc, u.z * gc.inv_acc, u.w * gc.inv_acc);
+                }
+                bias4 = mine;
+            }
             *reinterpret_cast<float4 *>(red + pt * 4) = bias4;
             __builtin_amdgcn_fence(__ATOMIC_RELEASE, "workgroup");
         }
     } else {
         const int lane = threadIdx.x & 63, half = lane >> 5, rc = lane & 31;
         const int g16 = lane >> 4, q = (lane & 15) >> 2, pp = lane & 3;
-        const AmaxLoad al_h = amax_issue(amax_hi), al_l = amax_issue(amax_lo);
+        AmaxLoad al_h{};
+        if constexpr (!GD3) al_h = amax_issue(amax_hi);
+        const AmaxLoad al_l = amax_issue(amax_lo);
         int loff[2][2], hcol[2][2], hrow[2];
 #pragma unroll
         for (int b = 0; b < 2; ++b) {
@@ -198,7 +255,7 @@
             ARVAE_WGR_PRODUCT(0, 0)
 #undef ARVAE_WGR_PRODUCT
         };
-        const float inv = amax_scale(al_l).inv * amax_scale(al_h).inv;
+        const float inv = amax_scale(al_l).inv * (GD3 ? gc.in.inv : amax_scale(al_h).inv);
         WGR_STAMP(0, 0);
         __syncthreads();
         WGR_STAMP(0, 1);
```

After: 1.389 million. 0.982x the previous value.
